# EugenHotaj/zig_gpt2

Measured on AMD Instinct MI355X. Metric: tokens/sec GPT-2-124M greedy 1024-ctx, higher is better.
Workload: dtype bf16 weights, f32 activations/accumulate; 1 GPU; GPT-2 124M greedy decode, 1 prompt(s)/GPU x 1 GPU(s), 1-token prompts, 1024 decode steps per prompt (reference generate loop, src/main.zig:322-342); vocab=50257, context=1024, n_layer=12, n_heads=12, n_embed=768, prompts_per_gpu=1, global_prompts=1, kv_cache=f32, hip_graph=True, l2_prefetcher=on, parallelism=replicated weights, prompts sharded x1, RCCL broadcast at start-up only

## Files before the change

### zig_gpt2_amd/csrc/api_gpt.hip

```cpp
#include <stdio.h>
#include <stdlib.h>
#include <string.h>

#include <string>
#include <thread>
#include <vector>

#include "zg_runtime.h"

using namespace zg;

struct zg_layer {
    void *c_attn_w, *c_proj_w, *c_fc_w, *mlp_proj_w;
    bf16_t *c_attn_p, *c_proj_p, *c_fc_p, *mlp_proj_p;
    float *c_attn_c2, *c_attn_c3, *c_fc_c2, *c_fc_c3;
    float *ln_1_g, *ln_1_b, *c_attn_b, *c_proj_b, *ln_2_g, *ln_2_b, *c_fc_b, *mlp_proj_b;
    void *k_cache, *v_cache;
};

struct zg_gpt {
    zg_gpt_config cfg;
    size_t batch;
    unsigned flags;
    int wt;
    int kv_mode;
    size_t wbytes;
    char* arena;
    size_t arena_bytes, weight_region_bytes, state_bytes;
    size_t kv_region_bytes;
    void *wte, *wpe;
    float *ln_f_g, *ln_f_b;
    float *lm_c2, *lm_c3;
    std::vector<zg_layer> layers;
    StepCtrl* ctrl;
    float *x, *q, *h4, *part, *logits, *part_val;
    int *part_idx, *prompt, *prompt_len, *forced, *cur_token, *out_tokens;
    float* sk_ws;
    int* sk_cnt;
    int sk_tiles;
    float *pf_x, *pf_qkv, *pf_ws;
    size_t pf_ws_floats;
    unsigned* sk_flags;
    unsigned sk_epoch;
    bool sk_used;
    bf16_t *pf_a, *pf_h;
    bf16_t *xp, *hp, *ap;
    int* attn_cnt;
    unsigned* epoch;
    unsigned spin_limit;
    unsigned* fault;
    unsigned long long *sk_tag, *part_tag;
    size_t sk_tag_bytes, part_tag_bytes;
    size_t epochs_since_clear;
    bool tags_on;
    float* xst;
    bool st_on;
    bool pl_on;
    int max_splits, lm_grid;
    StepCtrl* h_ctrl;
    int* h_ints;
    std::vector<hipGraphExec_t> graphs;
    std::vector<hipGraphExec_t> graphs_k;
    std::vector<hipGraphExec_t> graphs_s, graphs_ks;
    int* sampled;
    float* samp_ws;
    SampleParams* samp;
    SampleParams* h_samp;
    bool gen_sampled;
    size_t graph_steps;
    hipStream_t graph_stream;
    size_t steps_enqueued;
    bool ln_folded;
    PfCtl* pf_ctl;
    PfJob* pf_jobs;
    int pf_njobs;
    bool pf_on;
    bool pf_ran;
    bool pf_stalled;
    int pf_strikes;
    int pf_sit_out;
    hipStream_t pf_stream;
    hipEvent_t pf_ev_main, pf_ev_side;
    hipStream_t stream;
    zg_gpt* parent;
    int n_children;
    char* wbase;
    size_t gen_pos, gen_n, gen_min_prompt, gen_since_sync;
    bool gen_open;
};

static inline hipStream_t gs(const zg_gpt* g) { return g->stream ? g->stream : ctx().stream; }
static inline zg_gpt* root(zg_gpt* g) { return g->parent ? g->parent : g; }

namespace {

struct Carver {
    size_t off = 0;
    size_t take(size_t bytes) {
        off = (off + 255) & ~(size_t)255;
        const size_t o = off;
        off += bytes;
        return o;
    }
};

void carve(zg_gpt* g, char* wbase, char* sbase) {
    const zg_gpt_config& c = g->cfg;
    const size_t E = c.n_embed, V = c.vocab_size, C = c.context_size, L = c.n_layer, B = g->batch;
    const size_t wb = g->wbytes, kvb = g->kv_mode == 1 ? 2 : g->kv_mode == 2 ? 3 : 4;
    Carver cv;
    char* base = wbase;
    auto P = [&](size_t bytes) -> char* {
        const size_t o = cv.take(bytes);
        return base ? base + o : nullptr;
    };
    g->wte = P(V * E * wb);
    g->wpe = P(C * E * wb);
    g->ln_f_g = (float*)P(E * 4);
    g->ln_f_b = (float*)P(E * 4);
    g->lm_c2 = (float*)P(V * 4);
    g->lm_c3 = (float*)P(V * 4);
    g->layers.resize(L);
    for (size_t l = 0; l < L; ++l) {
        zg_layer& y = g->layers[l];
        y.c_attn_w = P(3 * E * E * wb);
        y.c_proj_w = P(E * E * wb);
        y.c_fc_w = P(4 * E * E * wb);
        y.mlp_proj_w = P(4 * E * E * wb);
        y.ln_1_g = (float*)P(E * 4);
        y.ln_1_b = (float*)P(E * 4);
        y.c_attn_b = (float*)P(3 * E * 4);
        y.c_proj_b = (float*)P(E * 4);
        y.ln_2_g = (float*)P(E * 4);
        y.ln_2_b = (float*)P(E * 4);
        y.c_fc_b = (float*)P(4 * E * 4);
        y.mlp_proj_b = (float*)P(E * 4);
        y.c_attn_c2 = (float*)P(3 * E * 4);
        y.c_attn_c3 = (float*)P(3 * E * 4);
        y.c_fc_c2 = (float*)P(4 * E * 4);
        y.c_fc_c3 = (float*)P(4 * E * 4);
        y.c_attn_p = y.c_proj_p = y.c_fc_p = y.mlp_proj_p = nullptr;
        if (g->wt == WT_F32 && !(g->flags & ZG_GPT_NO_PREFILL)) {
            y.c_attn_p = (bf16_t*)P(3 * E * E * kSplit * 2);
            y.c_proj_p = (bf16_t*)P(E * E * kSplit * 2);
            y.c_fc_p = (bf16_t*)P(4 * E * E * kSplit * 2);
            y.mlp_proj_p = (bf16_t*)P(4 * E * E * kSplit * 2);
        }
    }
    g->weight_region_bytes = (cv.off + 255) & ~(size_t)255;
    cv = Carver{};
    base = sbase;
    for (size_t l = 0; l < L; ++l) {
        g->layers[l].k_cache = P(B * C * E * kvb);
        g->layers[l].v_cache = P(B * C * E * kvb);
    }
    g->ctrl = (StepCtrl*)P(sizeof(StepCtrl));
    g->kv_region_bytes = L ? (size_t)(reinterpret_cast<char*>(g->ctrl) - reinterpret_cast<char*>(g->layers[0].k_cache)) : 0;
    g->x = (float*)P(B * E * 4);
    g->q = (float*)P(B * E * 4);
    g->h4 = (float*)P(B * 4 * E * 4);
    g->part = (float*)P(B * c.n_heads * g->max_splits * kPartStride * 4);
    g->logits = (float*)P(B * V * 4);
    g->part_val = (float*)P(B * 4096 * 4);
    g->part_idx = (int*)P(B * 4096 * 4);
    g->prompt = (int*)P(B * C * 4);
    g->prompt_len = (int*)P(B * 4);
    g->forced = (int*)P(B * 4);
    g->cur_token = (int*)P(B * 4);
    g->out_tokens = (int*)P(B * C * 4);
    g->sampled = (int*)P(B * 4);
    g->samp = (SampleParams*)P(sizeof(SampleParams));
    g->samp_ws = (float*)P(sample_workspace_floats((int)B) * 4);
    g->xp = (bf16_t*)P(E * 48);
    g->hp = (bf16_t*)P(4 * E * 48);
    g->ap = (bf16_t*)P(E * 48);
    g->attn_cnt = (int*)P(8 * c.n_heads * 4);
    g->epoch = (unsigned*)P(256);
    g->xst = (float*)P(((E + 15) / 16) * 8 * 2 * 4);
    g->sk_tag_bytes = ((E + 15) / 16) * 4 * 128 * 8;
    g->part_tag_bytes = 8 * c.n_heads * g->max_splits * kPartStride * 8;
    g->sk_tag = (unsigned long long*)P(g->sk_tag_bytes);
    g->part_tag = (unsigned long long*)P(g->part_tag_bytes);
    g->sk_tiles = (int)((E + 15) / 16);
    g->sk_ws = (float*)P((size_t)g->sk_tiles * 4 * 128 * 4);
    g->sk_cnt = (int*)P((size_t)g->sk_tiles * 4 * 4);
    g->pf_njobs = (int)(2 + 5 * L);
    g->pf_ctl = (PfCtl*)P(sizeof(PfCtl));
    g->pf_jobs = (PfJob*)P((size_t)g->pf_njobs * sizeof(PfJob));
    g->pf_x = g->pf_qkv = g->pf_ws = nullptr;
    g->sk_flags = nullptr;
    g->sk_epoch = 0;
    g->sk_used = false;
    g->pf_a = g->pf_h = nullptr;
    g->pf_ws_floats = 0;
    if (!(g->flags & ZG_GPT_NO_PREFILL)) {
        g->pf_x = (float*)P(B * C * E * 4);
        g->pf_qkv = (float*)P(B * C * 3 * E * 4);
        g->pf_a = (bf16_t*)P(B * C * kSplit * E * 2);
        g->pf_h = (bf16_t*)P(B * C * kSplit * 4 * E * 2);
        g->pf_ws_floats = g->wt == WT_BF16 ? (size_t)(16u << 20) : std::max((size_t)(16u << 20), 3 * B * C * 4 * E);
        g->pf_ws = (float*)P(g->pf_ws_floats * 4);
        g->sk_flags = (unsigned*)P(2048);
    }
    g->state_bytes = (cv.off + 255) & ~(size_t)255;
}

int bucket_t_hi(const zg_gpt* g, size_t seq_len) {
    const size_t hi = ((seq_len + 63) / 64) * 64;
    return (int)(hi < g->cfg.context_size ? hi : g->cfg.context_size);
}

GemvArgs base_gemv(const zg_gpt* g, const void* W, const float* bias, size_t N, size_t K, int t_hi) {
    GemvArgs a{};
    a.t_hi = t_hi;
    a.dbg = ctx().dbg;
    a.zero = ctx().d_zero;
    a.W = W;
    a.bias = bias;
    a.N = (int)N;
    a.K = (int)K;
    a.M = (int)g->batch;
    a.eps = 1e-5f;
    a.ctrl = g->ctrl;
    a.n_heads = (int)g->cfg.n_heads;
    a.head_dim = 64;
    a.max_splits = g->max_splits;
    a.ctx = (int)g->cfg.context_size;
    a.kv_mode = g->kv_mode;
    a.kv_lo = g->batch * g->cfg.context_size * g->cfg.n_embed * 2;
    a.sk_ws = g->sk_ws;
    a.sk_cnt = g->sk_cnt;
    a.sk_tiles = g->sk_tiles;
    a.progress = g->pf_on ? &g->pf_ctl->progress : nullptr;
    return a;
}

EmbedArgs embed_args(const zg_gpt* g, int finish_only) {
    EmbedArgs e{};
    e.ctrl = g->ctrl;
    e.wte = g->wte;
    e.wpe = g->wpe;
    e.weight_type = g->wt;
    e.n_embed = (int)g->cfg.n_embed;
    e.batch = (int)g->batch;
    e.vocab = (int)g->cfg.vocab_size;
    e.prompt = g->prompt;
    e.prompt_stride = (int)g->cfg.context_size;
    e.prompt_len = g->prompt_len;
    e.forced = g->forced;
    e.cur_token = g->cur_token;
    e.out_tokens = g->out_tokens;
    e.out_stride = (int)g->cfg.context_size;
    e.part_val = g->part_val;
    e.part_idx = g->part_idx;
    e.part_stride = g->lm_grid;
    e.n_partials = g->lm_grid;
    e.x = g->x;
    e.pl_out = g->pl_on ? g->xp : nullptr;
    e.pl_g = g->layers[0].ln_1_g;
    e.epoch = (g->pl_on && g->tags_on && finish_only != 1 && finish_only != 2) ? g->epoch : nullptr;
    e.st_out = g->st_on ? g->xst : nullptr;
    e.finish_only = finish_only;
    e.progress = g->pf_on ? &g->pf_ctl->progress : nullptr;
    e.sampled = g->sampled;
    return e;
}

int emit_gemv(const zg_gpt* g, const GemvArgs& a, int grid, hipStream_t s, std::vector<PfJob>* rec, unsigned cls) {
    if (!rec) return launch_gemv(a, g->wt, grid, s);
    PfJob j{};
    j.cls = cls;
    const int rows = gemv_rows_per_wg(a, g->wt);
    if (rows > 0) {
        j.kind = PF_WEIGHTS;
        j.base = reinterpret_cast<const char*>(a.W);
        j.total_bytes = (size_t)a.N * a.K * g->wbytes;
        j.wg_bytes = (unsigned)((size_t)rows * a.K * g->wbytes);
        j.n_wg = (unsigned)grid;
        j.touch_bytes = j.wg_bytes;
        if (a.M == 1) {
            const bool lnk = a.prologue == PRO_LAYERNORM && a.ln_c2 != nullptr;
            const float* v[3] = {lnk ? a.ln_g : nullptr, lnk ? a.ln_c2 : a.bias, lnk ? a.ln_c3 : nullptr};
            const size_t n[3] = {(size_t)a.K * 4, (size_t)a.N * 4, (size_t)a.N * 4};
            for (int i = 0; i < 3; ++i) {
                j.aux[i] = reinterpret_cast<const char*>(v[i]);
                j.aux_bytes[i] = v[i] ? (unsigned)n[i] : 0u;
            }
        }
        const size_t cap = (size_t)16 << 20;
        if (j.total_bytes > cap) j.touch_bytes = (unsigned)(((size_t)j.wg_bytes * cap / j.total_bytes + 127) & ~(size_t)127);
    }
    rec->push_back(j);
    return ZG_OK;
}

int enqueue_lm_head(zg_gpt* g, hipStream_t s, std::vector<PfJob>* rec = nullptr) {
    const size_t E = g->cfg.n_embed, V = g->cfg.vocab_size;
    GemvArgs a = base_gemv(g, g->wte, nullptr, V, E, 0);
    a.prologue = PRO_LAYERNORM;
    a.x = g->x;
    a.x_stride = (int)E;
    a.ln_g = g->ln_f_g;
    a.ln_b = g->ln_f_b;
    a.ln_c2 = g->lm_c2;
    a.ln_c3 = g->lm_c3;
    a.epilogue = EPI_ARGMAX;
    a.logits = g->logits;
    a.logits_stride = (int)V;
    a.part_val = g->part_val;
    a.part_idx = g->part_idx;
    const int grid = gemv_plan(a, g->wt);
    ZG_REQUIRE(grid == g->lm_grid, ZG_ERR_ARG, "lm_head grid changed");
    return emit_gemv(g, a, grid, s, rec, 6);
}

struct StepProf {
    std::vector<hipEvent_t> ev;
    std::vector<int> cls;
    size_t n = 0;
};
inline int prof_mark(StepProf* p, int cls, hipStream_t s) {
    if (!p) return ZG_OK;
    if (p->n == p->ev.size()) {
        hipEvent_t e;
        ZG_HIP(hipEventCreate(&e));
        p->ev.push_back(e);
        p->cls.push_back(cls);
    }
    p->cls[p->n] = cls;
    ZG_HIP(hipEventRecord(p->ev[p->n++], s));
    return ZG_OK;
}

int ensure_ln_folded(zg_gpt* g, hipStream_t s) {
    zg_gpt* r = root(g);
    if (r->ln_folded) return ZG_OK;
    const int E = (int)g->cfg.n_embed;
    for (const zg_layer& y : g->layers) {
        ZG_TRY(launch_ln_fold(y.c_attn_w, g->wt, y.ln_1_g, y.ln_1_b, y.c_attn_b, 3 * E, E, y.c_attn_c2, y.c_attn_c3, s));
        ZG_TRY(launch_ln_fold(y.c_fc_w, g->wt, y.ln_2_g, y.ln_2_b, y.c_fc_b, 4 * E, E, y.c_fc_c2, y.c_fc_c3, s));
    }
    ZG_TRY(launch_ln_fold(g->wte, g->wt, g->ln_f_g, g->ln_f_b, nullptr, (int)g->cfg.vocab_size, E, g->lm_c2, g->lm_c3, s));
    if (r->n_children > 0 || g->parent) ZG_HIP(hipStreamSynchronize(s));
    r->ln_folded = true;
    return ZG_OK;
}

int env_int(const char* name, int dflt);

int enqueue_step(zg_gpt* g, bool with_logits, int t_hi, hipStream_t s, StepProf* prof = nullptr, int only = -1, size_t only_layer = 0,
                 std::vector<PfJob>* rec = nullptr, int salt = -1, bool with_sampler = false) {
    const size_t E = g->cfg.n_embed;
    auto launch_id = [&](size_t l, int k) { return (unsigned)(salt >= 0 ? 1 + (2 * salt + k) % 254 : 2 * (int)l + 1 + k); };
    ZG_TRY(prof_mark(prof, -1, s));
    if (rec) rec->push_back(PfJob{});
    else if (only < 0 || only == 0) {
        EmbedArgs e = embed_args(g, only == 0 ? 3 : 0);
        ZG_TRY(launch_embed_step(e, s));
    }
    ZG_TRY(prof_mark(prof, 0, s));
    for (size_t l = (only < 0 ? 0 : only_layer); l < (only < 0 ? g->cfg.n_layer : only_layer + 1); ++l) {
        const zg_layer& y = g->layers[l];
        if (only < 0 || only == 1) {
            GemvArgs a = base_gemv(g, y.c_attn_w, y.c_attn_b, 3 * E, E, t_hi);
            a.prologue = PRO_LAYERNORM;
            a.x = g->x;
            a.x_stride = (int)E;
            a.ln_g = y.ln_1_g;
            a.ln_b = y.ln_1_b;
            a.ln_c2 = y.c_attn_c2;
            a.ln_c3 = y.c_attn_c3;
            a.epilogue = EPI_QKV;
            a.pl_in = g->pl_on ? g->xp : nullptr;
            a.st_in = g->st_on ? g->xst : nullptr;
            a.q = g->q;
            a.k_cache = y.k_cache;
            a.v_cache = y.v_cache;
            const int grid = gemv_plan(a, g->wt);
            ZG_TRY(emit_gemv(g, a, grid, s, rec, 1));
            ZG_TRY(prof_mark(prof, 1, s));
        }
        if (only < 0 || only == 2) {
            AttnArgs a{};
            a.q = g->q;
            a.k = y.k_cache;
            a.v = y.v_cache;
            a.stride_b = (long)(g->cfg.context_size * E);
            a.stride_h = (long)(g->cfg.context_size * 64);
            a.stride_t = 64;
            a.kv_mode = g->kv_mode;
            a.kv_lo = g->batch * g->cfg.context_size * E * 2;
            a.n_heads = (int)g->cfg.n_heads;
            a.head_dim = 64;
            a.batch = (int)g->batch;
            a.ctrl = g->ctrl;
            a.t_hi = t_hi;
            a.max_splits = g->max_splits;
            a.part = g->part;
            a.progress = g->pf_on ? &g->pf_ctl->progress : nullptr;
            if (g->pl_on) {
                a.pl_out = g->ap;
                a.merge_cnt = g->attn_cnt;
                if (g->tags_on && 2 * l + 2 <= 255) {
                    a.epoch = g->epoch;
                    a.launch_id = launch_id(l, 0);
                    a.part_tag = g->part_tag;
                    a.fault = g->fault;
                    a.spin_limit = g->spin_limit;
                }
            }
            if (rec) {
                PfJob j{};
                j.kind = PF_KV;
                j.cls = 2;
                j.base = reinterpret_cast<const char*>(y.k_cache);
                j.base2 = reinterpret_cast<const char*>(y.v_cache);
                j.n_heads = (unsigned)g->cfg.n_heads;
                j.ctx = (unsigned)g->cfg.context_size;
                j.batch = (unsigned)g->batch;
                j.row_bytes = g->kv_mode ? 128u : 256u;
                rec->push_back(j);
            } else
                ZG_TRY(launch_attn_decode(a, s));
            ZG_TRY(prof_mark(prof, 2, s));
        }
        if (only < 0 || only == 3) {
            GemvArgs a = base_gemv(g, y.c_proj_w, y.c_proj_b, E, E, t_hi);
            a.prologue = PRO_ATTN_MERGE;
            a.part = g->part;
            a.epilogue = EPI_RESIDUAL;
            a.y = g->x;
            a.y_stride = (int)E;
            a.resid = g->x;
            a.resid_stride = (int)E;
            if (g->pl_on) {
                a.prologue = PRO_NONE;
                a.pl_in = g->ap;
                a.pl_out = g->xp;
                a.pl_g = y.ln_2_g;
                a.st_out = g->st_on ? g->xst : nullptr;
            }
            const int grid = gemv_plan(a, g->wt);
            ZG_TRY(emit_gemv(g, a, grid, s, rec, 3));
            ZG_TRY(prof_mark(prof, 3, s));
        }
        if (only < 0 || only == 4) {
            GemvArgs a = base_gemv(g, y.c_fc_w, y.c_fc_b, 4 * E, E, t_hi);
            a.prologue = PRO_LAYERNORM;
            a.x = g->x;
            a.x_stride = (int)E;
            a.ln_g = y.ln_2_g;
            a.ln_b = y.ln_2_b;
            a.ln_c2 = y.c_fc_c2;
            a.ln_c3 = y.c_fc_c3;
            a.epilogue = EPI_GELU;
            a.y = g->h4;
            a.y_stride = (int)(4 * E);
            if (g->pl_on) {
                a.st_in = g->st_on ? g->xst : nullptr;
                a.pl_in = g->xp;
                a.pl_out = g->hp;
                a.y = nullptr;
            }
            const int grid = gemv_plan(a, g->wt);
            ZG_TRY(emit_gemv(g, a, grid, s, rec, 4));
            ZG_TRY(prof_mark(prof, 4, s));
        }
        if (only < 0 || only == 5) {
            GemvArgs a = base_gemv(g, y.mlp_proj_w, y.mlp_proj_b, E, 4 * E, t_hi);
            a.prologue = PRO_NONE;
            a.x = g->h4;
            a.x_stride = (int)(4 * E);
            a.epilogue = EPI_RESIDUAL;
            a.y = g->x;
            a.y_stride = (int)E;
            a.resid = g->x;
            a.resid_stride = (int)E;
            if (g->pl_on) {
                if (g->tags_on && 2 * l + 2 <= 255) {
                    a.epoch = g->epoch;
                    a.launch_id = launch_id(l, 1);
                    a.sk_tag = g->sk_tag;
                    a.fault = g->fault;
                    a.spin_limit = g->spin_limit;
                }
                a.pl_in = g->hp;
                if (l + 1 < g->cfg.n_layer) {
                    a.pl_out = g->xp;
                    a.pl_g = g->layers[l + 1].ln_1_g;
                    a.st_out = g->st_on ? g->xst : nullptr;
                }
            }
            const int grid = gemv_plan(a, g->wt);
            ZG_TRY(emit_gemv(g, a, grid, s, rec, 5));
            ZG_TRY(prof_mark(prof, 5, s));
        }
    }
    if (with_logits && (only < 0 || only == 6)) {
        ZG_TRY(enqueue_lm_head(g, s, rec));
        ZG_TRY(prof_mark(prof, 6, s));
    }
    if (with_sampler && with_logits && only < 0 && !rec)
        ZG_TRY(launch_sample_step(g->logits, (int)g->batch, (int)g->cfg.vocab_size, g->samp, g->ctrl, g->part_val, g->lm_grid, g->lm_grid, g->samp_ws,
                                  g->sampled, s));
    return ZG_OK;
}

int enqueue_prefill(zg_gpt* g, size_t P, bool last_block_full, hipStream_t s) {
    const bool f32w = g->wt == WT_F32;
    const int np = f32w ? kWeightPlanes : (g->flags & ZG_GPT_PREFILL_2PLANE) ? 2 : kSplit;
    const size_t E = g->cfg.n_embed, L = g->cfg.n_layer, H = g->cfg.n_heads, C = g->cfg.context_size;
    const int B = (int)g->batch, M = (int)(g->batch * P), iE = (int)E;
    ZG_TRY(launch_embed_prefill(g->prompt, (int)C, B, (int)P, g->wte, g->wpe, g->wt, iE, g->pf_x, s));
    ZG_TRY(launch_ln_split(g->pf_x, M, iE, g->layers[0].ln_1_g, g->layers[0].ln_1_b, 1e-5f, g->pf_a, s));
    for (size_t l = 0; l < L; ++l) {
        const zg_layer& y = g->layers[l];
        PrefillQkv qa{(int)P, iE, (int)H, (int)C, g->kv_mode, y.k_cache, y.v_cache, g->batch * C * E * 2};
        if (!f32w && g->sk_flags != nullptr) {
            qa.sk_ws = g->pf_ws;
            qa.sk_ws_bytes = g->pf_ws_floats * 4;
            qa.sk_flags = g->sk_flags;
            qa.sk_flags_words = 512;
            qa.sk_epoch = ++g->sk_epoch;
            g->sk_used = true;
        }
        ZG_TRY(launch_prefill_gemm(g->pf_a, f32w ? y.c_attn_p : (const bf16_t*)y.c_attn_w, y.c_attn_b, g->pf_qkv, M, 3 * iE, iE, 3 * iE, PF_QKV,
                                   g->pf_ws, g->pf_ws_floats, nullptr, s, &qa, np));
        if (l + 1 == L && !last_block_full) break;
        ZG_TRY(launch_attn_prefill(g->pf_qkv, g->pf_a, B, (int)P, iE, (int)H, g->pf_ws, g->pf_ws_floats, g->kv_mode == 0 ? (const float*)y.k_cache : nullptr,
                                       g->kv_mode == 0 ? (const float*)y.v_cache : nullptr, (int)C, s));
        const PrefillLn ln2{y.ln_2_g, y.ln_2_b, 1e-5f, g->pf_a};
        ZG_TRY(launch_prefill_gemm(g->pf_a, f32w ? y.c_proj_p : (const bf16_t*)y.c_proj_w, y.c_proj_b, g->pf_x, M, iE, iE, iE, PF_RESID, g->pf_ws,
                                   g->pf_ws_floats, &ln2, s, nullptr, np));
        ZG_TRY(launch_prefill_gemm(g->pf_a, f32w ? y.c_fc_p : (const bf16_t*)y.c_fc_w, y.c_fc_b, g->pf_h, M, 4 * iE, iE, 0, PF_GELU_SPLIT, g->pf_ws,
                                   g->pf_ws_floats, nullptr, s, nullptr, np));
        const bool more = l + 1 < L;
        const PrefillLn ln1{more ? g->layers[l + 1].ln_1_g : nullptr, more ? g->layers[l + 1].ln_1_b : nullptr, 1e-5f, g->pf_a};
        ZG_TRY(launch_prefill_gemm(g->pf_h, f32w ? y.mlp_proj_p : (const bf16_t*)y.mlp_proj_w, y.mlp_proj_b, g->pf_x, M, iE, 4 * iE, iE, PF_RESID, g->pf_ws,
                                   g->pf_ws_floats, more ? &ln1 : nullptr, s, nullptr, np));
    }
    return ZG_OK;
}

int check_fault(zg_gpt* g) {
    unsigned sk = 0, tag = 0;
    if (g->sk_used) {
        g->sk_used = false;
        ZG_TRY(gemm_s4_fault(&sk));
    }
    if (g->tags_on) {
        volatile unsigned* f = g->fault;
        tag = *f;
        if (tag) *f = 0;
    }
    if (sk) {
        set_error("a half-tile hand-over of the whole-prompt c_attn GEMM timed out%s: results discarded", tag ? " (and a tagged hand-over of the decode step)" : "");
        return ZG_ERR_HIP;
    }
    if (tag) {
        set_error("a tagged hand-over of the decode step timed out (a workgroup waited %u polls for its writers): results discarded", g->spin_limit);
        return ZG_ERR_HIP;
    }
    return ZG_OK;
}

int note_steps(zg_gpt* g, size_t n, hipStream_t s) {
    if (!g->tags_on) return ZG_OK;
    g->epochs_since_clear += n;
    if (g->epochs_since_clear < ((size_t)1 << 23)) return ZG_OK;
    g->epochs_since_clear = n;
    ZG_HIP(hipMemsetAsync(g->sk_tag, 0, g->sk_tag_bytes, s));
    ZG_HIP(hipMemsetAsync(g->part_tag, 0, g->part_tag_bytes, s));
    return ZG_OK;
}

int env_int(const char* name, int dflt) {
    const char* e = getenv(name);
    return e ? atoi(e) : dflt;
}

int setup_prefetcher(zg_gpt* g) {
    g->pf_on = g->pf_ran = g->pf_stalled = false;
    g->pf_strikes = g->pf_sit_out = 0;
    g->pf_stream = nullptr;
    g->pf_ev_main = g->pf_ev_side = nullptr;
    const bool small = g->stream == nullptr && g->batch == 1 && 4 * g->cfg.n_embed * g->cfg.n_embed * g->wbytes <= ((size_t)6 << 20);
    const int want = env_int("ZGPT2_PREFETCH", small ? 1 : 0);
    if ((g->flags & ZG_GPT_NO_PREFETCH) || !want || gs(g) == nullptr) return ZG_OK;
    if (g->pf_njobs > 255) return ZG_OK;
    std::vector<PfJob> jobs;
    ZG_TRY(enqueue_step(g, true, (int)g->cfg.context_size, nullptr, nullptr, -1, 0, &jobs));
    ZG_REQUIRE((int)jobs.size() == g->pf_njobs, ZG_ERR_ARG, "prefetcher: %zu launches per step", jobs.size());
    ZG_HIP(hipMemcpy(g->pf_jobs, jobs.data(), jobs.size() * sizeof(PfJob), hipMemcpyHostToDevice));
    int least = 0, greatest = 0;
    ZG_HIP(hipDeviceGetStreamPriorityRange(&least, &greatest));
    ZG_HIP(hipStreamCreateWithPriority(&g->pf_stream, hipStreamNonBlocking, least));
    ZG_HIP(hipEventCreateWithFlags(&g->pf_ev_main, hipEventDisableTiming));
    ZG_HIP(hipEventCreateWithFlags(&g->pf_ev_side, hipEventDisableTiming));
    g->pf_on = true;
    return ZG_OK;
}

void drop_prefetcher(zg_gpt* g) {
    if (g->pf_stream) {
        (void)hipStreamSynchronize(g->pf_stream);
        (void)hipStreamDestroy(g->pf_stream);
    }
    if (g->pf_ev_main) (void)hipEventDestroy(g->pf_ev_main);
    if (g->pf_ev_side) (void)hipEventDestroy(g->pf_ev_side);
    g->pf_stream = nullptr;
    g->pf_ev_main = g->pf_ev_side = nullptr;
    g->pf_on = false;
}

int pf_start(zg_gpt* g, size_t last_T, hipStream_t s) {
    if (!g->pf_on || s == nullptr) return ZG_OK;
    if (g->pf_ran) {
        ZG_HIP(hipStreamSynchronize(g->pf_stream));
        unsigned why[8];
        ZG_HIP(hipMemcpy(why, g->pf_ctl->exit_reason, sizeof(why), hipMemcpyDeviceToHost));
        bool idle_exit = false;
        for (unsigned w : why) idle_exit |= w == 2u;
        g->pf_ran = false;
        if (idle_exit) {
            g->pf_stalled = true;
            ++g->pf_strikes;
            g->pf_sit_out = 8;
        }
    }
    if (g->pf_stalled) {
        if (g->pf_strikes >= 3 || g->pf_sit_out-- > 0) return ZG_OK;
        g->pf_stalled = false;
    }
    ZG_HIP(hipMemsetAsync(g->pf_ctl, 0, sizeof(PfCtl), g->pf_stream));
    ZG_HIP(hipEventRecord(g->pf_ev_side, g->pf_stream));
    ZG_HIP(hipStreamWaitEvent(s, g->pf_ev_side, 0));
    ZG_HIP(hipEventRecord(g->pf_ev_main, s));
    ZG_HIP(hipStreamWaitEvent(g->pf_stream, g->pf_ev_main, 0));
    PfArgs a{};
    a.ctl = g->pf_ctl;
    a.jobs = g->pf_jobs;
    a.njobs = g->pf_njobs;
    a.lead = 2;
    a.nsub = 12;
    a.max_T = (int)last_T;
    a.idle_limit = (unsigned)env_int("ZGPT2_PF_IDLE", 100000);
    a.sleep = 1;
    a.cls_mask = 0x3e;
    a.line_shift = 7;
    a.cap_bytes = 0;
    g->pf_ran = true;
    return launch_prefetcher(a, g->pf_stream);
}

int pf_stop(zg_gpt* g, hipStream_t s) {
    if (!g->pf_on || s == nullptr) return ZG_OK;
    ZG_HIP(hipMemsetD32Async(reinterpret_cast<hipDeviceptr_t>(&g->pf_ctl->progress), (int)PF_STOP, 1, s));
    return ZG_OK;
}

size_t prefill_min() { return 4; }

void drop_graphs(zg_gpt* g) {
    for (auto* v : {&g->graphs, &g->graphs_k, &g->graphs_s, &g->graphs_ks})
        for (auto& e : *v)
            if (e) {
                (void)hipGraphExecDestroy(e);
                e = nullptr;
            }
}

int capture_steps(zg_gpt* g, hipGraphExec_t* out, bool with_logits, int t_hi, size_t n_steps, hipStream_t cs, bool with_sampler = false) {
    hipGraph_t graph = nullptr;
    ZG_HIP(hipStreamBeginCapture(cs, hipStreamCaptureModeThreadLocal));
    int st = ZG_OK;
    for (size_t i = 0; i < n_steps && st == ZG_OK; ++i) st = enqueue_step(g, with_logits, t_hi, cs, nullptr, -1, 0, nullptr, -1, with_sampler);
    hipError_t e = hipStreamEndCapture(cs, &graph);
    if (st != ZG_OK) {
        if (graph) (void)hipGraphDestroy(graph);
        return st;
    }
    ZG_HIP(e);
    ZG_HIP(hipGraphInstantiate(out, graph, nullptr, nullptr, 0));
    ZG_HIP(hipGraphDestroy(graph));
    return ZG_OK;
}

int capture_bucket(zg_gpt* g, size_t idx, hipStream_t s) {
    const size_t seq_len = (idx / 2 + 1) * 64;
    const bool with_logits = idx & 1;
    if (g->graphs.size() <= idx) g->graphs.resize(idx + 1, nullptr);
    if (g->graphs[idx]) return ZG_OK;
    const int t_hi = bucket_t_hi(g, seq_len);
    return capture_steps(g, &g->graphs[idx], with_logits, t_hi, 1, s);
}

int capture_multi(zg_gpt* g, size_t b, hipStream_t s) {
    if (g->graphs_k.size() <= b) g->graphs_k.resize(b + 1, nullptr);
    if (g->graphs_k[b]) return ZG_OK;
    const int t_hi = bucket_t_hi(g, (b + 1) * 64);
    return capture_steps(g, &g->graphs_k[b], true, t_hi, g->graph_steps, s);
}

int capture_sampled(zg_gpt* g, size_t b, bool multi, hipStream_t s) {
    auto& v = multi ? g->graphs_ks : g->graphs_s;
    if (v.size() <= b) v.resize(b + 1, nullptr);
    if (v[b]) return ZG_OK;
    return capture_steps(g, &v[b], true, bucket_t_hi(g, (b + 1) * 64), multi ? g->graph_steps : 1, s, true);
}

int capture_all(zg_gpt* g, hipStream_t s) {
    if ((g->flags & ZG_GPT_NO_GRAPH) || s == nullptr) return ZG_OK;
    if (g->graph_stream != s) {
        drop_graphs(g);
        g->graph_stream = s;
    }
    const size_t n = ((g->cfg.context_size + 63) / 64) * 2;
    for (size_t idx = 0; idx < n; ++idx) ZG_TRY(capture_bucket(g, idx, s));
    if (g->graph_steps > 1)
        for (size_t b = 0; b < n / 2; ++b) ZG_TRY(capture_multi(g, b, s));
    if (g->flags & ZG_GPT_SAMPLED_GENERATE)
        for (size_t b = 0; b < n / 2; ++b) {
            ZG_TRY(capture_sampled(g, b, false, s));
            if (g->graph_steps > 1) ZG_TRY(capture_sampled(g, b, true, s));
        }
    return ZG_OK;
}

int run_step(zg_gpt* g, bool with_logits, size_t seq_len, hipStream_t s, bool with_sampler = false) {
    ZG_TRY(ensure_ln_folded(g, s));
    const int t_hi = bucket_t_hi(g, seq_len);
    with_sampler = with_sampler && with_logits;
    if ((g->flags & ZG_GPT_NO_GRAPH) || s == nullptr) return enqueue_step(g, with_logits, t_hi, s, nullptr, -1, 0, nullptr, -1, with_sampler);
    if (g->graph_stream != s) ZG_TRY(capture_all(g, s));
    if (with_sampler) {
        const size_t b = (seq_len + 63) / 64 - 1;
        ZG_TRY(capture_sampled(g, b, false, s));
        ZG_HIP(hipGraphLaunch(g->graphs_s[b], s));
        return ZG_OK;
    }
    const size_t idx = ((seq_len + 63) / 64 - 1) * 2 + (with_logits ? 1 : 0);
    ZG_TRY(capture_bucket(g, idx, s));
    ZG_HIP(hipGraphLaunch(g->graphs[idx], s));
    return ZG_OK;
}

int upload_f32(const float* src, size_t n, void* dst, bool as_bf16, hipStream_t s) {
    Ctx& c = ctx();
    const float* dsrc = src;
    if (!is_device_ptr(src)) {
        if (!as_bf16) {
            ZG_HIP(hipMemcpyAsync(dst, src, n * 4, hipMemcpyHostToDevice, s));
            ZG_HIP(hipStreamSynchronize(s));
            return ZG_OK;
        }
        const size_t cap = c.stage_cap / 4;
        ZG_REQUIRE(cap > 0, ZG_ERR_STAGING, "no staging arena");
        for (size_t o = 0; o < n; o += cap) {
            const size_t m = (n - o < cap) ? (n - o) : cap;
            ZG_HIP(hipMemcpyAsync(c.stage, src + o, m * 4, hipMemcpyHostToDevice, s));
            ZG_TRY(launch_f32_to_bf16(reinterpret_cast<const float*>(c.stage), reinterpret_cast<bf16_t*>(dst) + o, m, s));
            ZG_HIP(hipStreamSynchronize(s));
        }
        return ZG_OK;
    }
    if (as_bf16) ZG_TRY(launch_f32_to_bf16(dsrc, reinterpret_cast<bf16_t*>(dst), n, s));
    else ZG_HIP(hipMemcpyAsync(dst, dsrc, n * 4, hipMemcpyDeviceToDevice, s));
    ZG_HIP(hipStreamSynchronize(s));
    return ZG_OK;
}

}

extern "C" {

int zg_gpt_create(zg_gpt** out, const zg_gpt_config* config, size_t batch, unsigned flags) {
    return zg_gpt_create_ex(out, config, batch, flags, nullptr);
}

int zg_gpt_create_ex(zg_gpt** out, const zg_gpt_config* config, size_t batch, unsigned flags, const zg_gpt_options* opt) {
    ZG_TRY(require_init());
    ZG_REQUIRE(out && config, ZG_ERR_ARG, "zg_gpt_create: null argument");
    const zg_gpt_config& c = *config;
    zg_gpt* parent = opt ? opt->share_weights_with : nullptr;
    if (parent) {
        ZG_REQUIRE(parent->parent == nullptr, ZG_ERR_ARG, "zg_gpt_create_ex: share_weights_with must own its weights");
        ZG_REQUIRE(memcmp(&parent->cfg, config, sizeof(zg_gpt_config)) == 0, ZG_ERR_SHAPE, "zg_gpt_create_ex: a handle shares weights with one of the same config only");
        const unsigned same = ZG_GPT_WEIGHTS_F32 | ZG_GPT_NO_PREFILL;
        ZG_REQUIRE((parent->flags & same) == (flags & same), ZG_ERR_ARG, "zg_gpt_create_ex: weight type / prefill flags differ from the weight owner's");
    }
    ZG_REQUIRE(c.n_heads > 0 && c.n_embed % c.n_heads == 0 && c.n_embed / c.n_heads == 64, ZG_ERR_UNSUPPORTED,
               "head_dim %zu != 64 (GPT-2 family only)", c.n_heads ? c.n_embed / c.n_heads : (size_t)0);
    ZG_REQUIRE(c.n_embed % 8 == 0 && c.n_embed * 4 <= 8192, ZG_ERR_UNSUPPORTED, "n_embed %zu unsupported", c.n_embed);
    ZG_REQUIRE(batch >= 1 && batch <= 8, ZG_ERR_UNSUPPORTED, "batch %zu outside 1..8", batch);
    ZG_REQUIRE(c.vocab_size > 0 && c.context_size > 0 && c.n_layer > 0, ZG_ERR_ARG, "empty config");
    ZG_REQUIRE(!(flags & ZG_GPT_KV_F16) || !(flags & ZG_GPT_KV_B24), ZG_ERR_ARG, "ZG_GPT_KV_F16 and ZG_GPT_KV_B24 exclude each other");
    zg_gpt* g = new zg_gpt();
    g->cfg = c;
    g->batch = batch;
    g->flags = flags;
    g->wt = (flags & ZG_GPT_WEIGHTS_F32) ? WT_F32 : WT_BF16;
    g->wbytes = g->wt == WT_BF16 ? 2 : 4;
    g->kv_mode = (flags & ZG_GPT_KV_F16) ? 1 : (flags & ZG_GPT_KV_B24) ? 2 : 0;
    g->max_splits = (int)((c.context_size + kAttnChunk - 1) / kAttnChunk);
    g->graph_stream = nullptr;
    g->stream = nullptr;
    g->parent = parent;
    g->n_children = 0;
    g->gen_open = false;
    g->pf_stream = nullptr;
    g->pf_ev_main = g->pf_ev_side = nullptr;
    carve(g, nullptr, nullptr);
    g->arena_bytes = (parent ? 0 : g->weight_region_bytes) + g->state_bytes;
    hipError_t e = hipMalloc(reinterpret_cast<void**>(&g->arena), g->arena_bytes);
    if (e != hipSuccess) {
        delete g;
        return hip_fail(e, "hipMalloc(model arena)", __FILE__, __LINE__);
    }
    g->wbase = parent ? parent->wbase : g->arena;
    char* const sbase = parent ? g->arena : g->arena + g->weight_region_bytes;
    carve(g, g->wbase, sbase);
    (void)hipMemset(sbase, 0, g->state_bytes);
    if (opt && opt->own_stream) {
        int least = 0, greatest = 0;
        (void)hipDeviceGetStreamPriorityRange(&least, &greatest);
        const int pr = opt->stream_priority > 0 ? greatest : opt->stream_priority < 0 ? least : 0;
        e = hipStreamCreateWithPriority(&g->stream, hipStreamNonBlocking, pr);
        if (e != hipSuccess) {
            (void)hipFree(g->arena);
            delete g;
            return hip_fail(e, "hipStreamCreateWithPriority(handle stream)", __FILE__, __LINE__);
        }
    }
    {
        GemvArgs a = base_gemv(g, g->wte, nullptr, c.vocab_size, c.n_embed, 0);
        a.prologue = PRO_LAYERNORM;
        a.epilogue = EPI_ARGMAX;
        g->lm_grid = gemv_plan(a, g->wt);
    }
    {
        GemvArgs a = base_gemv(g, g->layers[0].mlp_proj_w, nullptr, c.n_embed, 4 * c.n_embed, 0);
        if (!gemv_supported(a, g->wt)) {
            if (g->stream) (void)hipStreamDestroy(g->stream);
            (void)hipFree(g->arena);
            delete g;
            set_error("batch %zu with n_embed %zu: %zu input rows of 4*n_embed floats do not fit the LDS (use a smaller batch)",
                      batch, c.n_embed, batch);
            return ZG_ERR_UNSUPPORTED;
        }
    }
    g->pl_on = false;
    if (g->wt == WT_BF16 && batch >= 2 && !(decode_paths_off() & 1)) {
        const zg_layer& y = g->layers[0];
        GemvArgs a1 = base_gemv(g, y.c_attn_w, y.c_attn_b, 3 * c.n_embed, c.n_embed, 0);
        a1.prologue = PRO_LAYERNORM;
        a1.ln_c2 = y.c_attn_c2;
        a1.ln_c3 = y.c_attn_c3;
        a1.epilogue = EPI_QKV;
        GemvArgs a4 = base_gemv(g, y.c_fc_w, y.c_fc_b, 4 * c.n_embed, c.n_embed, 0);
        a4.prologue = PRO_LAYERNORM;
        a4.ln_c2 = y.c_fc_c2;
        a4.ln_c3 = y.c_fc_c3;
        a4.epilogue = EPI_GELU;
        GemvArgs a5 = base_gemv(g, y.mlp_proj_w, y.mlp_proj_b, c.n_embed, 4 * c.n_embed, 0);
        a5.prologue = PRO_NONE;
        a5.epilogue = EPI_RESIDUAL;
        GemvArgs a3 = base_gemv(g, y.c_proj_w, y.c_proj_b, c.n_embed, c.n_embed, 0);
        a3.prologue = PRO_NONE;
        a3.epilogue = EPI_RESIDUAL;
        g->pl_on = c.n_embed % 32 == 0 && gemv_planes_ok(a1, g->wt) && gemv_planes_ok(a3, g->wt) && gemv_planes_ok(a4, g->wt) &&
                   gemv_planes_ok(a5, g->wt);
    }
    g->tags_on = g->pl_on && !(decode_paths_off() & 4);
    g->spin_limit = (unsigned)env_int("ZGPT2_TAG_SPIN_LIMIT", 1 << 20);
    g->st_on = false;
    if (g->pl_on && !(decode_paths_off() & 8) && c.n_embed % 16 == 0 && c.n_embed / 16 <= 128) {
        const zg_layer& y = g->layers[0];
        GemvArgs a1 = base_gemv(g, y.c_attn_w, y.c_attn_b, 3 * c.n_embed, c.n_embed, 0);
        a1.prologue = PRO_LAYERNORM;
        a1.x_stride = (int)c.n_embed;
        a1.ln_c2 = y.c_attn_c2;
        a1.ln_c3 = y.c_attn_c3;
        a1.epilogue = EPI_QKV;
        GemvArgs a4 = a1;
        a4.N = (int)(4 * c.n_embed);
        a4.epilogue = EPI_GELU;
        GemvArgs a3 = base_gemv(g, y.c_proj_w, y.c_proj_b, c.n_embed, c.n_embed, 0);
        a3.prologue = PRO_NONE;
        a3.epilogue = EPI_RESIDUAL;
        a3.resid_stride = (int)c.n_embed;
        GemvArgs a5 = base_gemv(g, y.mlp_proj_w, y.mlp_proj_b, c.n_embed, 4 * c.n_embed, 0);
        a5.prologue = PRO_NONE;
        a5.epilogue = EPI_RESIDUAL;
        a5.resid_stride = (int)c.n_embed;
        g->st_on = gemv_pl4_ok(a1, g->wt) && gemv_pl4_ok(a3, g->wt) && gemv_pl4_ok(a4, g->wt) && gemv_pl4_ok(a5, g->wt);
    }
    if (g->lm_grid > 4096) {
        if (g->stream) (void)hipStreamDestroy(g->stream);
        (void)hipFree(g->arena);
        delete g;
        set_error("lm_head grid %d exceeds the argmax partial buffer", g->lm_grid);
        return ZG_ERR_UNSUPPORTED;
    }
    g->h_ctrl = nullptr;
    g->h_ints = nullptr;
    hipError_t he = hipHostMalloc(reinterpret_cast<void**>(&g->h_ctrl), sizeof(StepCtrl) + 512, hipHostMallocDefault);
    if (he == hipSuccess)
        he = hipHostMalloc(reinterpret_cast<void**>(&g->h_ints), (batch * c.context_size + batch) * sizeof(int), hipHostMallocDefault);
    if (he != hipSuccess) {
        if (g->h_ctrl) (void)hipHostFree(g->h_ctrl);
        if (g->stream) (void)hipStreamDestroy(g->stream);
        (void)hipFree(g->arena);
        delete g;
        return hip_fail(he, "hipHostMalloc(control mirrors)", __FILE__, __LINE__);
    }
    static_assert(sizeof(StepCtrl) + sizeof(SampleParams) <= 256, "the fault word sits 256 bytes behind the control mirror");
    g->h_samp = reinterpret_cast<SampleParams*>(reinterpret_cast<char*>(g->h_ctrl) + 128);
    g->gen_sampled = false;
    g->fault = reinterpret_cast<unsigned*>(reinterpret_cast<char*>(g->h_ctrl) + 256);
    *g->fault = 0;
    g->steps_enqueued = 0;
    g->epochs_since_clear = 0;
    g->ln_folded = false;
    {
        const int k = env_int("ZGPT2_GRAPH_STEPS", 8);
        g->graph_steps = (k == 2 || k == 4 || k == 8 || k == 16 || k == 32 || k == 64) ? (size_t)k : 1;
    }
    {
        int st = setup_prefetcher(g);
        if (st == ZG_OK) st = capture_all(g, gs(g));
        if (st != ZG_OK) {
            drop_prefetcher(g);
            drop_graphs(g);
            (void)hipHostFree(g->h_ctrl);
            (void)hipHostFree(g->h_ints);
            if (g->stream) (void)hipStreamDestroy(g->stream);
            (void)hipFree(g->arena);
            delete g;
            return st;
        }
    }
    if (parent) ++parent->n_children;
    *out = g;
    return ZG_OK;
}

int zg_gpt_destroy(zg_gpt* g) {
    if (!g) return ZG_OK;
    ZG_REQUIRE(g->n_children == 0, ZG_ERR_ARG, "zg_gpt_destroy: %d handle(s) still borrow this one's weights (destroy them first)", g->n_children);
    (void)hipStreamSynchronize(gs(g));
    drop_prefetcher(g);
    drop_graphs(g);
    if (g->stream) (void)hipStreamDestroy(g->stream);
    if (g->parent) --g->parent->n_children;
    (void)hipFree(g->arena);
    (void)hipHostFree(g->h_ctrl);
    (void)hipHostFree(g->h_ints);
    delete g;
    return ZG_OK;
}

int zg_gpt_stream(zg_gpt* g, void** hip_stream_out) {
    ZG_TRY(require_init());
    ZG_REQUIRE(g && hip_stream_out, ZG_ERR_ARG, "zg_gpt_stream: null argument");
    *hip_stream_out = gs(g);
    return ZG_OK;
}

int zg_gpt_load_block_tensor(zg_gpt* g, size_t layer, int slot, const float* src, size_t len) {
    ZG_TRY(require_init());
    ZG_REQUIRE(g && src && layer < g->cfg.n_layer, ZG_ERR_ARG, "load_block_tensor: bad argument");
    ZG_REQUIRE(g->parent == nullptr, ZG_ERR_ARG, "load_block_tensor: this handle borrows its weights (load them into their owner)");
    const size_t E = g->cfg.n_embed;
    zg_layer& y = g->layers[layer];
    void* dst = nullptr;
    size_t n = 0;
    bool mat = false;
    switch (slot) {
        case ZG_LN_1_G: dst = y.ln_1_g; n = E; break;
        case ZG_LN_1_B: dst = y.ln_1_b; n = E; break;
        case ZG_C_ATTN_W: dst = y.c_attn_w; n = 3 * E * E; mat = true; break;
        case ZG_C_ATTN_B: dst = y.c_attn_b; n = 3 * E; break;
        case ZG_C_PROJ_W: dst = y.c_proj_w; n = E * E; mat = true; break;
        case ZG_C_PROJ_B: dst = y.c_proj_b; n = E; break;
        case ZG_LN_2_G: dst = y.ln_2_g; n = E; break;
        case ZG_LN_2_B: dst = y.ln_2_b; n = E; break;
        case ZG_C_FC_W: dst = y.c_fc_w; n = 4 * E * E; mat = true; break;
        case ZG_C_FC_B: dst = y.c_fc_b; n = 4 * E; break;
        case ZG_MLP_PROJ_W: dst = y.mlp_proj_w; n = 4 * E * E; mat = true; break;
        case ZG_MLP_PROJ_B: dst = y.mlp_proj_b; n = E; break;
        default: ZG_REQUIRE(false, ZG_ERR_ARG, "unknown block slot %d", slot);
    }
    ZG_REQUIRE(len == n, ZG_ERR_SHAPE, "block slot %d expects %zu elements, got %zu", slot, n, len);
    g->ln_folded = false;
    ZG_TRY(upload_f32(src, n, dst, mat && g->wt == WT_BF16, gs(g)));
    if (mat && g->wt == WT_F32 && y.c_attn_p) {
        bf16_t* pl = slot == ZG_C_ATTN_W ? y.c_attn_p : slot == ZG_C_PROJ_W ? y.c_proj_p : slot == ZG_C_FC_W ? y.c_fc_p : y.mlp_proj_p;
        ZG_REQUIRE(n <= (size_t)2147483647 / 3, ZG_ERR_SHAPE, "weight matrix of %zu elements", n);
        ZG_TRY(launch_split3(reinterpret_cast<const float*>(dst), 1, (int)n, pl, gs(g)));
        ZG_HIP(hipStreamSynchronize(gs(g)));
    }
    return ZG_OK;
}

int zg_gpt_load_tensor(zg_gpt* g, int slot, const float* src, size_t len) {
    ZG_TRY(require_init());
    ZG_REQUIRE(g && src, ZG_ERR_ARG, "load_tensor: bad argument");
    ZG_REQUIRE(g->parent == nullptr, ZG_ERR_ARG, "load_tensor: this handle borrows its weights (load them into their owner)");
    const size_t E = g->cfg.n_embed;
    void* dst = nullptr;
    size_t n = 0;
    bool mat = false;
    switch (slot) {
        case ZG_WTE: dst = g->wte; n = g->cfg.vocab_size * E; mat = true; break;
        case ZG_WPE: dst = g->wpe; n = g->cfg.context_size * E; mat = true; break;
        case ZG_LN_F_G: dst = g->ln_f_g; n = E; break;
        case ZG_LN_F_B: dst = g->ln_f_b; n = E; break;
        default: ZG_REQUIRE(false, ZG_ERR_ARG, "unknown slot %d", slot);
    }
    ZG_REQUIRE(len == n, ZG_ERR_SHAPE, "slot %d expects %zu elements, got %zu", slot, n, len);
    g->ln_folded = false;
    return upload_f32(src, n, dst, mat && g->wt == WT_BF16, gs(g));
}

int zg_gpt_weight_arena(zg_gpt* g, void** device_ptr, size_t* bytes) {
    ZG_REQUIRE(g && device_ptr && bytes, ZG_ERR_ARG, "weight_arena: null argument");
    if (!root(g)->ln_folded) {
// ... 337 lines not shown
        std::vector<std::thread> th;
        std::vector<int> res(begun, ZG_OK);
        std::vector<std::string> errs(begun);
        const int dev = ctx().device;
        for (size_t i = 0; i < begun; ++i)
            th.emplace_back([&, i]() {
                int r = hipSetDevice(dev) == hipSuccess ? ZG_OK : ZG_ERR_HIP;
                for (bool more = true; more && r == ZG_OK;) r = gen_pump(handles[i], &more);
                res[i] = r;
                if (r != ZG_OK) errs[i] = zg_last_error();
            });
        for (auto& t : th) t.join();
        for (size_t i = 0; i < begun && rs == ZG_OK; ++i)
            if (res[i] != ZG_OK) {
                rs = res[i];
                snprintf(msg, sizeof msg, "%s", errs[i].c_str());
            }
    } else {
        bool any = rs == ZG_OK;
        while (any && rs == ZG_OK) {
            any = false;
            for (size_t i = 0; i < begun && rs == ZG_OK; ++i) {
                bool more = false;
                if (handles[i]->gen_pos < handles[i]->gen_n) rs = gen_pump(handles[i], &more);
                any |= more;
            }
        }
        if (rs != ZG_OK) snprintf(msg, sizeof msg, "%s", zg_last_error());
    }
    int first_err = rs;
    for (size_t i = 0; i < begun; ++i) {
        const int e = gen_end(handles[i], rs);
        if (first_err == ZG_OK && e != ZG_OK) {
            first_err = e;
            snprintf(msg, sizeof msg, "%s", zg_last_error());
        }
    }
    if (first_err != ZG_OK) set_error("%s", msg);
    return first_err;
}

int zg_gpt_generate_fetch_many(zg_gpt* const* handles, size_t n_handles, size_t n_steps, size_t* out_tokens, size_t out_len) {
    ZG_TRY(require_init());
    ZG_REQUIRE(handles && n_handles >= 1 && out_tokens, ZG_ERR_ARG, "generate_fetch_many: null argument");
    size_t rows = 0;
    for (size_t i = 0; i < n_handles; ++i) {
        ZG_REQUIRE(handles[i] != nullptr, ZG_ERR_ARG, "generate_fetch_many: handle %zu is null", i);
        rows += handles[i]->batch;
    }
    ZG_REQUIRE(out_len >= rows * n_steps, ZG_ERR_SHAPE, "generate_fetch_many: out_tokens too short");
    size_t row = 0;
    int first_err = ZG_OK;
    char msg[512];
    for (size_t i = 0; i < n_handles; ++i) {
        const int e = zg_gpt_generate_fetch(handles[i], n_steps, out_tokens + row * n_steps, handles[i]->batch * n_steps);
        if (first_err == ZG_OK && e != ZG_OK) {
            first_err = e;
            snprintf(msg, sizeof msg, "%s", zg_last_error());
        }
        row += handles[i]->batch;
    }
    if (first_err != ZG_OK) set_error("%s", msg);
    return first_err;
}

int zg_gpt_generate_fetch(zg_gpt* g, size_t n_steps, size_t* out_tokens, size_t out_len) {
    ZG_TRY(require_init());
    ZG_REQUIRE(g && out_tokens, ZG_ERR_ARG, "generate_fetch: null argument");
    const size_t C = g->cfg.context_size, B = g->batch;
    ZG_REQUIRE(n_steps <= C && out_len >= B * n_steps, ZG_ERR_SHAPE, "generate_fetch: out_tokens too short");
    hipStream_t s = gs(g);
    ZG_HIP(hipMemcpyAsync(g->h_ints, g->out_tokens, B * C * sizeof(int), hipMemcpyDeviceToHost, s));
    ZG_HIP(hipStreamSynchronize(s));
    ZG_TRY(check_fault(g));
    for (size_t b = 0; b < B; ++b)
        for (size_t i = 0; i < n_steps; ++i) out_tokens[b * n_steps + i] = (size_t)g->h_ints[b * C + i];
    return ZG_OK;
}

int zg_gpt_generate_greedy(zg_gpt* g, const size_t* prompts, size_t prompt_stride, const size_t* prompt_lens,
                           size_t n_steps, size_t* out_tokens, size_t out_len) {
    ZG_REQUIRE(g && out_tokens && out_len >= g->batch * n_steps, ZG_ERR_SHAPE, "generate: out_tokens too short");
    ZG_TRY(zg_gpt_generate_enqueue(g, prompts, prompt_stride, prompt_lens, n_steps));
    return zg_gpt_generate_fetch(g, n_steps, out_tokens, out_len);
}

int zg_gpt_profile_step(zg_gpt* g, size_t seq_len, int iters, float* us_out, size_t n_out) {
    ZG_TRY(require_init());
    ZG_REQUIRE(g && us_out && n_out >= 8 && iters > 0, ZG_ERR_ARG, "profile_step: bad argument");
    ZG_REQUIRE(seq_len >= 1 && seq_len + (size_t)iters - 1 <= g->cfg.context_size, ZG_ERR_SHAPE,
               "profile_step: positions %zu..%zu outside the context", seq_len, seq_len + iters - 1);
    hipStream_t s = gs(g);
    ZG_HIP(hipStreamSynchronize(s));
    ZG_TRY(ensure_ln_folded(g, s));
    ZG_TRY(note_steps(g, (size_t)iters, s));
    for (size_t b = 0; b < g->batch; ++b) g->h_ints[b] = (int)(b % g->cfg.vocab_size);
    g->h_ctrl->step = (int)seq_len - 1;
    g->h_ctrl->seq_len = (int)seq_len;
    g->h_ctrl->mode = 1;
    g->h_ctrl->n_partials = g->lm_grid;
    ZG_HIP(hipMemcpyAsync(g->forced, g->h_ints, g->batch * sizeof(int), hipMemcpyHostToDevice, s));
    ZG_HIP(hipMemcpyAsync(g->ctrl, g->h_ctrl, sizeof(StepCtrl), hipMemcpyHostToDevice, s));
    static StepProf prof;
    double acc[8] = {0, 0, 0, 0, 0, 0, 0, 0};
    prof.n = 0;
    double null_us = 0.0;
    for (int it = 0; it < iters; ++it) {
        ZG_TRY(enqueue_step(g, true, bucket_t_hi(g, seq_len + it), s, &prof));
        ZG_TRY(launch_copy_f32(g->q, g->q + 4, 1, s));
        ZG_TRY(prof_mark(&prof, 8, s));
    }
    ZG_HIP(hipStreamSynchronize(s));
    for (size_t i = 1; i < prof.n; ++i) {
        if (prof.cls[i] < 0) continue;
        float ms = 0.0f;
        ZG_HIP(hipEventElapsedTime(&ms, prof.ev[i - 1], prof.ev[i]));
        if (prof.cls[i] == 8) {
            null_us += ms * 1000.0;
            continue;
        }
        acc[prof.cls[i]] += ms * 1000.0;
        acc[7] += ms * 1000.0;
    }
    for (int i = 0; i < 8; ++i) us_out[i] = (float)(acc[i] / iters);
    if (n_out >= 9) us_out[8] = (float)(null_us / iters);
    return check_fault(g);
}

int zg_gpt_time_kernel(zg_gpt* g, int which_and_options, int iters, float* avg_us, size_t* algorithmic_bytes) {
    ZG_TRY(require_init());
    const int which = which_and_options & 0xff;
    const bool cycle = (which_and_options & ZG_TIME_WALK_LAYERS) != 0;
    const size_t t_opt = (size_t)((unsigned)which_and_options >> 16);
    ZG_REQUIRE(g && avg_us && iters > 0 && which_and_options >= 0 && which <= 6, ZG_ERR_ARG, "time_kernel: bad argument (ZG_TIME_AT takes t < 32768)");
    hipStream_t s = gs(g);
    ZG_REQUIRE(s != nullptr, ZG_ERR_UNSUPPORTED, "time_kernel needs a capturable stream");
    const size_t E = g->cfg.n_embed, wb = g->wbytes;
    const size_t bytes_tab[7] = {0, 3 * E * E * wb, 0, E * E * wb, 4 * E * E * wb, 4 * E * E * wb, g->cfg.vocab_size * E * wb};
    size_t T = g->cfg.context_size / 2 > 0 ? g->cfg.context_size / 2 : 1;
    if (t_opt >= 1 && t_opt <= g->cfg.context_size) T = t_opt;
    ZG_HIP(hipStreamSynchronize(s));
    ZG_TRY(ensure_ln_folded(g, s));
    ZG_TRY(note_steps(g, (size_t)iters + 8, s));
    g->h_ctrl->step = (int)T - 1;
    g->h_ctrl->seq_len = (int)T;
    g->h_ctrl->mode = 1;
    g->h_ctrl->n_partials = g->lm_grid;
    ZG_HIP(hipMemcpyAsync(g->ctrl, g->h_ctrl, sizeof(StepCtrl), hipMemcpyHostToDevice, s));
    const int chain = 64;
    hipGraph_t graph = nullptr;
    hipGraphExec_t exec = nullptr;
    ZG_HIP(hipStreamBeginCapture(s, hipStreamCaptureModeThreadLocal));
    int st = ZG_OK;
    if (g->tags_on && which != 0) st = launch_epoch_bump(g->epoch, s);
    for (int i = 0; i < chain && st == ZG_OK; ++i)
        st = enqueue_step(g, true, bucket_t_hi(g, T), s, nullptr, which, cycle ? (size_t)i % g->cfg.n_layer : 0, nullptr, i);
    hipError_t ce = hipStreamEndCapture(s, &graph);
    if (st != ZG_OK) return st;
    ZG_HIP(ce);
    ZG_HIP(hipGraphInstantiate(&exec, graph, nullptr, nullptr, 0));
    hipEvent_t e0, e1;
    ZG_HIP(hipEventCreate(&e0));
    ZG_HIP(hipEventCreate(&e1));
    ZG_HIP(hipGraphLaunch(exec, s));
    ZG_HIP(hipStreamSynchronize(s));
    const int reps = (iters + chain - 1) / chain;
    ZG_HIP(hipEventRecord(e0, s));
    for (int r = 0; r < reps; ++r) ZG_HIP(hipGraphLaunch(exec, s));
    ZG_HIP(hipEventRecord(e1, s));
    ZG_HIP(hipEventSynchronize(e1));
    float ms = 0.0f;
    ZG_HIP(hipEventElapsedTime(&ms, e0, e1));
    (void)hipEventDestroy(e0);
    (void)hipEventDestroy(e1);
    (void)hipGraphExecDestroy(exec);
    (void)hipGraphDestroy(graph);
    *avg_us = ms * 1000.0f / (float)(reps * chain);
    if (algorithmic_bytes) *algorithmic_bytes = bytes_tab[which];
    return check_fault(g);
}

int zg_debug_prefetch_stats(zg_gpt* g, unsigned* out, size_t n_out) {
    ZG_TRY(require_init());
    ZG_REQUIRE(g && out && n_out >= 25, ZG_ERR_ARG, "prefetch_stats: need 25 words");
    memset(out, 0, n_out * sizeof(unsigned));
    out[0] = g->pf_on ? (g->pf_stalled ? 2u : 1u) : 0u;
    if (!g->pf_on) return ZG_OK;
    ZG_HIP(hipStreamSynchronize(gs(g)));
    ZG_HIP(hipStreamSynchronize(g->pf_stream));
    PfCtl h;
    ZG_HIP(hipMemcpy(&h, g->pf_ctl, sizeof(PfCtl), hipMemcpyDeviceToHost));
    for (int x = 0; x < 8; ++x) {
        out[1 + x] = h.ticket[x];
        out[9 + x] = h.exit_reason[x];
        out[17 + x] = h.jobs_done[x];
    }
    for (size_t i = 0; i < 256 && 25 + i < n_out; ++i) out[25 + i] = h.xcd_log[i];
    return ZG_OK;
}

#ifdef ZG_STAMPS
int zg_debug_stamps_begin(void) {
    ZG_TRY(require_init());
    Ctx& c = ctx();
    const size_t bytes = (16 + 10 * 4096) * sizeof(unsigned long long);
    if (!c.dbg) ZG_HIP(hipMalloc(reinterpret_cast<void**>(&c.dbg), bytes));
    ZG_HIP(hipMemset(c.dbg, 0, bytes));
    return ZG_OK;
}
int zg_debug_stamps_read(unsigned long long* out, size_t n_words) {
    ZG_TRY(require_init());
    ZG_HIP(hipDeviceSynchronize());
    ZG_HIP(hipMemcpy(out, ctx().dbg, n_words * sizeof(unsigned long long), hipMemcpyDeviceToHost));
    return ZG_OK;
}
#endif

}
```

### zig_gpt2_amd/csrc/attn.hip

```cpp
#include <stdlib.h>

#include "zg_kernels.h"
#include "zg_runtime.h"

namespace zg {

namespace {

constexpr float kNegBig = -1e30f;

template <typename KV>
__device__ __forceinline__ f32x4 load_kv4(const KV* p);
template <>
__device__ __forceinline__ f32x4 load_kv4<float>(const float* p) {
    return *reinterpret_cast<const f32x4*>(p);
}
template <>
__device__ __forceinline__ f32x4 load_kv4<_Float16>(const _Float16* p) {
    typedef __attribute__((ext_vector_type(4))) _Float16 h4;
    const h4 v = *reinterpret_cast<const h4*>(p);
    f32x4 r;
    r.x = (float)v.x; r.y = (float)v.y; r.z = (float)v.z; r.w = (float)v.w;
    return r;
}

__device__ __forceinline__ float row16_reduce_scatter(float (&s)[16], int lr) {
    float a8[8];
    {
        const bool hi = lr & 8;
#pragma unroll
        for (int j = 0; j < 8; ++j) {
            const float keep = hi ? s[j + 8] : s[j];
            const float send = hi ? s[j] : s[j + 8];
            a8[j] = keep + dpp_row_ror<8>(send);
        }
    }
    float a4[4];
    {
        const bool hi = lr & 4;
#pragma unroll
        for (int j = 0; j < 4; ++j) {
            const float keep = hi ? a8[j + 4] : a8[j];
            const float send = hi ? a8[j] : a8[j + 4];
            const float from_lo = dpp_row_ror<4>(send);
            const float from_hi = dpp_row_ror<12>(send);
            a4[j] = keep + (hi ? from_lo : from_hi);
        }
    }
    float a2[2];
    {
        const bool hi = lr & 2;
#pragma unroll
        for (int j = 0; j < 2; ++j) {
            const float keep = hi ? a4[j + 2] : a4[j];
            const float send = hi ? a4[j] : a4[j + 2];
            const float from_lo = dpp_row_ror<2>(send);
            const float from_hi = dpp_row_ror<14>(send);
            a2[j] = keep + (hi ? from_lo : from_hi);
        }
    }
    {
        const bool hi = lr & 1;
        const float keep = hi ? a2[1] : a2[0];
        const float send = hi ? a2[0] : a2[1];
        const float from_lo = dpp_row_ror<1>(send);
        const float from_hi = dpp_row_ror<15>(send);
        return keep + (hi ? from_lo : from_hi);
    }
}

__device__ __forceinline__ void publish_partial(const AttnArgs& a, int n_heads, int nsplit, int b, int h, int split, int lane, float o,
                                                float M, float l, unsigned tag) {
    float* part = a.part + (((size_t)b * n_heads + h) * a.max_splits + split) * kPartStride;
    if (a.pl_out == nullptr) {
        part[lane] = o;
        if (lane == 0) {
            part[64] = M;
            part[65] = l;
        }
        return;
    }
    float r = o, lsum = l;
    if (nsplit > 1 && a.part_tag) {
        typedef unsigned long long u64;
        auto pack = [&](float v) { return ((u64)tag << 32) | (u64)__float_as_uint(v); };
        u64* pt0 = a.part_tag + ((size_t)b * n_heads + h) * a.max_splits * kPartStride;
        const int last = nsplit - 1;
        if (split != last) {
            u64* pt = pt0 + split * kPartStride;
            __hip_atomic_store(pt + lane, pack(o), __ATOMIC_RELAXED, __HIP_MEMORY_SCOPE_AGENT);
            if (lane == 0) {
                __hip_atomic_store(pt + 64, pack(M), __ATOMIC_RELAXED, __HIP_MEMORY_SCOPE_AGENT);
                __hip_atomic_store(pt + 65, pack(l), __ATOMIC_RELAXED, __HIP_MEMORY_SCOPE_AGENT);
            }
            return;
        }
        float mx = M;
        r = 0.0f;
        lsum = 0.0f;
        constexpr int MAXS = 4;
        if (nsplit <= MAXS) {
            u64 vo[MAXS - 1], vm[MAXS - 1], vl[MAXS - 1];
            for (int spins = 0;; ++spins) {
                bool ok = true;
#pragma unroll
                for (int s = 0; s < MAXS - 1; ++s) {
                    const u64* ps = pt0 + min(s, last - 1) * kPartStride;
                    vo[s] = __hip_atomic_load(ps + lane, __ATOMIC_RELAXED, __HIP_MEMORY_SCOPE_AGENT);
                    vm[s] = __hip_atomic_load(ps + 64, __ATOMIC_RELAXED, __HIP_MEMORY_SCOPE_AGENT);
                    vl[s] = __hip_atomic_load(ps + 65, __ATOMIC_RELAXED, __HIP_MEMORY_SCOPE_AGENT);
                    ok = ok && (unsigned)(vo[s] >> 32) == tag && (unsigned)(vm[s] >> 32) == tag && (unsigned)(vl[s] >> 32) == tag;
                }
                if (__builtin_amdgcn_ballot_w64(!ok) == 0) break;
                if ((unsigned)spins >= a.spin_limit) {
                    if (lane == 0 && a.fault) __hip_atomic_store(a.fault, 1u, __ATOMIC_RELAXED, __HIP_MEMORY_SCOPE_AGENT);
                    break;
                }
                __builtin_amdgcn_s_sleep(1);
            }
            float ms[MAXS], ls[MAXS], os[MAXS];
#pragma unroll
            for (int s = 0; s < MAXS; ++s) {
                const bool polled = s < last && s < MAXS - 1;
                ms[s] = polled ? __uint_as_float((unsigned)vm[s < MAXS - 1 ? s : 0]) : s == last ? M : -1e30f;
                ls[s] = polled ? __uint_as_float((unsigned)vl[s < MAXS - 1 ? s : 0]) : l;
                os[s] = polled ? __uint_as_float((unsigned)vo[s < MAXS - 1 ? s : 0]) : o;
            }
            mx = fmaxf(fmaxf(ms[0], ms[1]), fmaxf(ms[2], ms[3]));
#pragma unroll
            for (int s = 0; s < MAXS; ++s) {
                const float w = __expf(ms[s] - mx);
                lsum = fmaf(w, ls[s], lsum);
                r = fmaf(w, os[s], r);
            }
        } else {
            float mrun = -1e30f;
            for (int s = 0; s <= last; ++s) {
                float m_s = M, o_s = o, l_s = l;
                if (s < last) {
                    const u64* ps = pt0 + s * kPartStride;
                    u64 vo, vm, vl;
                    for (int spins = 0;; ++spins) {
                        vo = __hip_atomic_load(ps + lane, __ATOMIC_RELAXED, __HIP_MEMORY_SCOPE_AGENT);
                        vm = __hip_atomic_load(ps + 64, __ATOMIC_RELAXED, __HIP_MEMORY_SCOPE_AGENT);
                        vl = __hip_atomic_load(ps + 65, __ATOMIC_RELAXED, __HIP_MEMORY_SCOPE_AGENT);
                        const bool ok = (unsigned)(vo >> 32) == tag && (unsigned)(vm >> 32) == tag && (unsigned)(vl >> 32) == tag;
                        if (__builtin_amdgcn_ballot_w64(!ok) == 0) break;
                        if ((unsigned)spins >= a.spin_limit) {
                            if (lane == 0 && a.fault) __hip_atomic_store(a.fault, 1u, __ATOMIC_RELAXED, __HIP_MEMORY_SCOPE_AGENT);
                            break;
                        }
                        __builtin_amdgcn_s_sleep(1);
                    }
                    m_s = __uint_as_float((unsigned)vm);
                    o_s = __uint_as_float((unsigned)vo);
                    l_s = __uint_as_float((unsigned)vl);
                }
                const float mnew = fmaxf(mrun, m_s);
                const float w0 = __expf(mrun - mnew), w1 = __expf(m_s - mnew);
                r = fmaf(w1, o_s, r * w0);
                lsum = fmaf(w1, l_s, lsum * w0);
                mrun = mnew;
            }
        }
    } else if (nsplit > 1) {
        typedef __attribute__((address_space(1))) unsigned gu32;
        gu32* gp = (gu32*)part;
        __hip_atomic_store(gp + lane, __float_as_uint(o), __ATOMIC_RELAXED, __HIP_MEMORY_SCOPE_AGENT);
        if (lane == 0) {
            __hip_atomic_store(gp + 64, __float_as_uint(M), __ATOMIC_RELAXED, __HIP_MEMORY_SCOPE_AGENT);
            __hip_atomic_store(gp + 65, __float_as_uint(l), __ATOMIC_RELAXED, __HIP_MEMORY_SCOPE_AGENT);
        }
        asm volatile("s_waitcnt vmcnt(0)" ::: "memory");
        int* cnt = a.merge_cnt + b * n_heads + h;
        int ticket = 0;
        if (lane == 0) ticket = __hip_atomic_fetch_add(cnt, 1, __ATOMIC_RELAXED, __HIP_MEMORY_SCOPE_AGENT);
        ticket = __builtin_amdgcn_readfirstlane(ticket);
        if (ticket != nsplit - 1) return;
        if (lane == 0) __hip_atomic_store(cnt, 0, __ATOMIC_RELAXED, __HIP_MEMORY_SCOPE_AGENT);
        const gu32* p0 = (const gu32*)(a.part + ((size_t)b * n_heads + h) * a.max_splits * kPartStride);
        constexpr int MAXS = 4;
        if (nsplit <= MAXS) {
            float ms[MAXS], ls[MAXS], os[MAXS];
#pragma unroll
            for (int s = 0; s < MAXS; ++s) {
                const gu32* ps = p0 + min(s, nsplit - 1) * kPartStride;
                ms[s] = __uint_as_float(__hip_atomic_load(ps + 64, __ATOMIC_RELAXED, __HIP_MEMORY_SCOPE_AGENT));
                ls[s] = __uint_as_float(__hip_atomic_load(ps + 65, __ATOMIC_RELAXED, __HIP_MEMORY_SCOPE_AGENT));
                os[s] = __uint_as_float(__hip_atomic_load(ps + lane, __ATOMIC_RELAXED, __HIP_MEMORY_SCOPE_AGENT));
            }
#pragma unroll
            for (int s = 0; s < MAXS; ++s)
                if (s >= nsplit) ms[s] = -1e30f;
            const float mx = fmaxf(fmaxf(ms[0], ms[1]), fmaxf(ms[2], ms[3]));
            r = 0.0f;
            lsum = 0.0f;
#pragma unroll
            for (int s = 0; s < MAXS; ++s) {
                const float w = __expf(ms[s] - mx);
                lsum = fmaf(w, ls[s], lsum);
                r = fmaf(w, os[s], r);
            }
        } else {
            float mx = -1e30f;
            for (int s = 0; s < nsplit; ++s)
                mx = fmaxf(mx, __uint_as_float(__hip_atomic_load(p0 + s * kPartStride + 64, __ATOMIC_RELAXED, __HIP_MEMORY_SCOPE_AGENT)));
            r = 0.0f;
            lsum = 0.0f;
            for (int s = 0; s < nsplit; ++s) {
                const gu32* ps = p0 + s * kPartStride;
                const float w = __expf(__uint_as_float(__hip_atomic_load(ps + 64, __ATOMIC_RELAXED, __HIP_MEMORY_SCOPE_AGENT)) - mx);
                lsum = fmaf(w, __uint_as_float(__hip_atomic_load(ps + 65, __ATOMIC_RELAXED, __HIP_MEMORY_SCOPE_AGENT)), lsum);
                r = fmaf(w, __uint_as_float(__hip_atomic_load(ps + lane, __ATOMIC_RELAXED, __HIP_MEMORY_SCOPE_AGENT)), r);
            }
        }
    }
    const float v = r * (1.0f / lsum);
    uint32_t hi, mid, lo;
    split3_pk(v, 0.0f, hi, mid, lo);
    const int k = h * 64 + lane;
    a.pl_out[plane_elem(0, b, k)] = (bf16_t)hi;
    a.pl_out[plane_elem(1, b, k)] = (bf16_t)mid;
    a.pl_out[plane_elem(2, b, k)] = (bf16_t)lo;
}

template <typename KV>
__global__ __launch_bounds__(256) void attn_decode_kernel(const float* __restrict__ qp, const void* __restrict__ kp,
                                                          const void* __restrict__ vp, unsigned sb, unsigned sh, unsigned st,
                                                          unsigned th, const int* __restrict__ cw, const unsigned* __restrict__ ew,
                                                          const AttnArgs a) {
    __shared__ __attribute__((aligned(16))) float s_o[4][64];
    __shared__ float s_m[4], s_l[4];
    const int h = blockIdx.x, split = blockIdx.y, b = blockIdx.z;
    const int t_hi = (int)(th & 0xfffffu), n_heads = (int)(th >> 20);
    const int Tc = cw[1];
    const unsigned epoch = ew[0];
    const int T = (st >> 31) ? Tc : t_hi;
    const size_t stride_t = st & 0x7fffffffu;
    const int chunk0 = split * kAttnChunk;
    if (chunk0 >= t_hi) return;

    const int lane = threadIdx.x & 63, wave = threadIdx.x >> 6;
    const int lr = lane & 15, g = lane >> 4;
    const int base = chunk0 + wave * 64;

    const KV* K = reinterpret_cast<const KV*>(kp) + (size_t)b * sb + (size_t)h * sh;
    const KV* V = reinterpret_cast<const KV*>(vp) + (size_t)b * sb + (size_t)h * sh;
    const f32x4 q4 = *reinterpret_cast<const f32x4*>(qp + ((size_t)b * n_heads + h) * 64 + lr * 4);
    const float alpha = 0.125f;

    float m_w = kNegBig, l_w = 0.0f;
    f32x4 o4 = {0.0f, 0.0f, 0.0f, 0.0f};
    if (base < t_hi) {
        f32x4 k4[16], v4[16];
#pragma unroll
        for (int i = 0; i < 16; ++i) {
            const int t = min(base + 4 * i + g, t_hi - 1);
            k4[i] = load_kv4<KV>(K + (size_t)t * stride_t + lr * 4);
            v4[i] = load_kv4<KV>(V + (size_t)t * stride_t + lr * 4);
        }
        ZG_PIN(a.progress); ZG_PIN(a.part); ZG_PIN(a.max_splits); ZG_PIN(a.pl_out); ZG_PIN(a.part_tag); ZG_PIN(a.launch_id); ZG_PIN(a.merge_cnt); ZG_PIN(a.fault); ZG_PIN(a.spin_limit);
        pf_count(a.progress);
        float s[16];
#pragma unroll
        for (int i = 0; i < 16; ++i)
            s[i] = fmaf(q4.x, k4[i].x, fmaf(q4.y, k4[i].y, fmaf(q4.z, k4[i].z, q4.w * k4[i].w)));
        float sc = row16_reduce_scatter(s, lr) * alpha;
        const int t_mine = base + 4 * lr + g;
        if (t_mine >= T) sc = kNegBig;
        m_w = wave_allmax(sc);
        const float p = (t_mine < T) ? __expf(sc - m_w) : 0.0f;
        l_w = wave_allsum(p);
#define ZG_PV(i)                                                                                                         \
    {                                                                                                                    \
        const float pi = __uint_as_float(__builtin_amdgcn_update_dpp(0u, __float_as_uint(p), 0x150 + (i), 0xF, 0xF, false)); \
        o4.x = fmaf(pi, v4[i].x, o4.x);                                                                                  \
        o4.y = fmaf(pi, v4[i].y, o4.y);                                                                                  \
        o4.z = fmaf(pi, v4[i].z, o4.z);                                                                                  \
        o4.w = fmaf(pi, v4[i].w, o4.w);                                                                                  \
    }
        ZG_PV(0) ZG_PV(1) ZG_PV(2) ZG_PV(3) ZG_PV(4) ZG_PV(5) ZG_PV(6) ZG_PV(7)
        ZG_PV(8) ZG_PV(9) ZG_PV(10) ZG_PV(11) ZG_PV(12) ZG_PV(13) ZG_PV(14) ZG_PV(15)
#undef ZG_PV
        o4.x += __shfl_xor(o4.x, 16, 64); o4.y += __shfl_xor(o4.y, 16, 64);
        o4.z += __shfl_xor(o4.z, 16, 64); o4.w += __shfl_xor(o4.w, 16, 64);
        o4.x += __shfl_xor(o4.x, 32, 64); o4.y += __shfl_xor(o4.y, 32, 64);
        o4.z += __shfl_xor(o4.z, 32, 64); o4.w += __shfl_xor(o4.w, 32, 64);
    }
    if (lane < 16) *reinterpret_cast<f32x4*>(&s_o[wave][lane * 4]) = o4;
    if (lane == 0) {
        s_m[wave] = m_w;
        s_l[wave] = l_w;
    }
    __syncthreads();
    if (wave == 0) {
        const float M = fmaxf(fmaxf(s_m[0], s_m[1]), fmaxf(s_m[2], s_m[3]));
        float o = 0.0f, l = 0.0f;
#pragma unroll
        for (int w = 0; w < 4; ++w) {
            const float sc = __expf(s_m[w] - M);
            o = fmaf(sc, s_o[w][lane], o);
            l = fmaf(sc, s_l[w], l);
        }
        publish_partial(a, n_heads, (t_hi + kAttnChunk - 1) / kAttnChunk, b, h, split, lane, o, M, l, (epoch << 8) | a.launch_id);
    }
}

typedef __attribute__((ext_vector_type(8))) _Float16 h8;

__device__ __forceinline__ float grp8_reduce_scatter(float (&s)[8], int c) {
    float a4[4];
    {
        const bool hi = c & 4;
#pragma unroll
        for (int j = 0; j < 4; ++j) {
            const float keep = hi ? s[j + 4] : s[j];
            const float send = hi ? s[j] : s[j + 4];
            const float from_lo = dpp_row_ror<4>(send);
            const float from_hi = dpp_row_ror<12>(send);
            a4[j] = keep + (hi ? from_lo : from_hi);
        }
    }
    float a2[2];
    {
        const bool hi = c & 2;
#pragma unroll
        for (int j = 0; j < 2; ++j) {
            const float keep = hi ? a4[j + 2] : a4[j];
            const float send = hi ? a4[j] : a4[j + 2];
            const float from_lo = dpp_row_ror<2>(send);
            const float from_hi = dpp_row_ror<14>(send);
            a2[j] = keep + (hi ? from_lo : from_hi);
        }
    }
    const bool hi = c & 1;
    const float keep = hi ? a2[1] : a2[0];
    const float send = hi ? a2[0] : a2[1];
    const float from_lo = dpp_row_ror<1>(send);
    const float from_hi = dpp_row_ror<15>(send);
    return keep + (hi ? from_lo : from_hi);
}

template <int MODE>
struct Row8;
template <>
struct Row8<1> {
    h8 v;
    __device__ __forceinline__ void load(const void* base, size_t, size_t elem) { v = *reinterpret_cast<const h8*>(reinterpret_cast<const _Float16*>(base) + elem); }
    __device__ __forceinline__ float at(int e) const { return (float)v[e]; }
};
template <>
struct Row8<2> {
    u32x4 hi;
    u32x2 lo;
    __device__ __forceinline__ void load(const void* base, size_t lo_off, size_t elem) {
        hi = *reinterpret_cast<const u32x4*>(reinterpret_cast<const uint16_t*>(base) + elem);
        lo = *reinterpret_cast<const u32x2*>(reinterpret_cast<const uint8_t*>(base) + lo_off + elem);
    }
    __device__ __forceinline__ float at(int e) const {
        const uint32_t sel = ((e & 1) ? 0x07060000u : 0x05040000u) | ((uint32_t)(e & 3) << 8) | 0x0cu;
        return __uint_as_float(__builtin_amdgcn_perm(hi[e >> 1], lo[e >> 2], sel));
    }
};

template <int MODE>
__global__ __launch_bounds__(256) void attn_decode_h8_kernel(const float* __restrict__ qp0, const void* __restrict__ kp,
                                                             const void* __restrict__ vp, unsigned sb, unsigned sh, unsigned st,
                                                             unsigned th, const int* __restrict__ cw, const unsigned* __restrict__ ew,
                                                             const AttnArgs a) {
    __shared__ __attribute__((aligned(16))) float s_o[4][64];
    __shared__ float s_m[4], s_l[4];
    const int h = blockIdx.x, split = blockIdx.y, b = blockIdx.z;
    const int t_hi = (int)(th & 0xfffffu), n_heads = (int)(th >> 20);
    const int Tc = cw[1];
    const unsigned epoch = ew[0];
    const int T = (st >> 31) ? Tc : t_hi;
    const size_t stride_t = st & 0x7fffffffu;
    const int chunk0 = split * kAttnChunk;
    if (chunk0 >= t_hi) return;

    const int lane = threadIdx.x & 63, wave = threadIdx.x >> 6;
    const int c = lane & 7, g8 = lane >> 3;
    const int base = chunk0 + wave * 64;
    const size_t head0 = (size_t)b * sb + (size_t)h * sh;
    const float* qp = qp0 + ((size_t)b * n_heads + h) * 64 + c * 8;
    const f32x4 qa = *reinterpret_cast<const f32x4*>(qp), qb = *reinterpret_cast<const f32x4*>(qp + 4);
    const float q[8] = {qa.x, qa.y, qa.z, qa.w, qb.x, qb.y, qb.z, qb.w};
    const float alpha = 0.125f;

    float m_w = kNegBig, l_w = 0.0f;
    float o[8] = {0.0f, 0.0f, 0.0f, 0.0f, 0.0f, 0.0f, 0.0f, 0.0f};
    if (base < t_hi) {
        Row8<MODE> k8[8], v8[8];
#pragma unroll
        for (int i = 0; i < 8; ++i) {
            const int t = min(base + 8 * i + g8, t_hi - 1);
            k8[i].load(kp, a.kv_lo, head0 + (size_t)t * stride_t + c * 8);
            v8[i].load(vp, a.kv_lo, head0 + (size_t)t * stride_t + c * 8);
        }
        ZG_PIN(a.progress); ZG_PIN(a.part); ZG_PIN(a.max_splits); ZG_PIN(a.pl_out); ZG_PIN(a.part_tag); ZG_PIN(a.launch_id); ZG_PIN(a.merge_cnt); ZG_PIN(a.fault); ZG_PIN(a.spin_limit);
        pf_count(a.progress);
        float s[8];
#pragma unroll
        for (int i = 0; i < 8; ++i) {
            float acc = 0.0f;
#pragma unroll
            for (int e = 0; e < 8; ++e) acc = fmaf(q[e], k8[i].at(e), acc);
            s[i] = acc;
        }
        float sc = grp8_reduce_scatter(s, c) * alpha;
        const int t_mine = base + 8 * c + g8;
        if (t_mine >= T) sc = kNegBig;
        m_w = wave_allmax(sc);
        const float p = (t_mine < T) ? __expf(sc - m_w) : 0.0f;
        l_w = wave_allsum(p);
        const bool up = lane & 8;
#define ZG_PV8(i)                                                                                                          \
    {                                                                                                                      \
        const float plo = __uint_as_float(__builtin_amdgcn_update_dpp(0u, __float_as_uint(p), 0x150 + (i), 0xF, 0xF, false));     \
        const float phi = __uint_as_float(__builtin_amdgcn_update_dpp(0u, __float_as_uint(p), 0x150 + 8 + (i), 0xF, 0xF, false)); \
        const float pi = up ? phi : plo;                                                                                   \
        _Pragma("unroll") for (int e = 0; e < 8; ++e) o[e] = fmaf(pi, v8[i].at(e), o[e]);                              \
    }
        ZG_PV8(0) ZG_PV8(1) ZG_PV8(2) ZG_PV8(3) ZG_PV8(4) ZG_PV8(5) ZG_PV8(6) ZG_PV8(7)
#undef ZG_PV8
#pragma unroll
        for (int e = 0; e < 8; ++e) {
            o[e] += dpp_row_ror<8>(o[e]);
            o[e] += __shfl_xor(o[e], 16, 64);
            o[e] += __shfl_xor(o[e], 32, 64);
        }
    }
    if (lane < 8) {
        *reinterpret_cast<f32x4*>(&s_o[wave][lane * 8]) = f32x4{o[0], o[1], o[2], o[3]};
        *reinterpret_cast<f32x4*>(&s_o[wave][lane * 8 + 4]) = f32x4{o[4], o[5], o[6], o[7]};
    }
    if (lane == 0) {
        s_m[wave] = m_w;
        s_l[wave] = l_w;
    }
    __syncthreads();
    if (wave == 0) {
        const float M = fmaxf(fmaxf(s_m[0], s_m[1]), fmaxf(s_m[2], s_m[3]));
        float ov = 0.0f, l = 0.0f;
#pragma unroll
        for (int w = 0; w < 4; ++w) {
            const float sc = __expf(s_m[w] - M);
            ov = fmaf(sc, s_o[w][lane], ov);
            l = fmaf(sc, s_l[w], l);
        }
        publish_partial(a, n_heads, (t_hi + kAttnChunk - 1) / kAttnChunk, b, h, split, lane, ov, M, l, (epoch << 8) | a.launch_id);
    }
}

__global__ __launch_bounds__(256) void attn_merge_kernel(const float* part, int n_heads, int max_splits,
                                                         int seq_len, float* out) {
    const int b = blockIdx.y;
    const int e = blockIdx.x * 256 + threadIdx.x;
// ... 135 lines not shown
```

### zig_gpt2_amd/csrc/gemv_internal.h

```cpp
#pragma once
#include <stdlib.h>

#include "zg_kernels.h"

#ifdef ZG_STAMPS
#define ZG_STAMP_DECL() unsigned long long zg_ts[8] = {0, 0, 0, 0, 0, 0, 0, 0}
#define ZG_STAMP(i) zg_ts[i] = __builtin_amdgcn_s_memtime()
#define ZG_STAMP_FLUSH()                                                                              \
    if (a.dbg && threadIdx.x == 0 && (blockIdx.x == 0 || blockIdx.x == gridDim.x - 1)) {             \
        const unsigned long long slot = atomicAdd(a.dbg, 1ull);                                       \
        unsigned long long* d = a.dbg + 16 + slot * 10;                                               \
        for (int i = 0; i < 8; ++i) d[i] = zg_ts[i];                                                  \
        d[8] = blockIdx.x;                                                                            \
        d[9] = __builtin_amdgcn_s_memtime();                                                          \
    }
#else
#define ZG_STAMP_DECL()
#define ZG_STAMP(i)
#define ZG_STAMP_FLUSH()
#endif

namespace zg {

namespace {
// ... 155 lines not shown
            ls[s] = ps[65];
            const float2 lo = *reinterpret_cast<const float2*>(ps + d0);
            const float2 hi = *reinterpret_cast<const float2*>(ps + d0 + 2);
            o[s][0] = lo.x; o[s][1] = lo.y; o[s][2] = hi.x; o[s][3] = hi.y;
        }
#pragma unroll
        for (int s = 0; s < MAXS; ++s)
            if (s >= nsplit) ms[s] = -1e30f;
        const float mx = fmaxf(fmaxf(ms[0], ms[1]), fmaxf(ms[2], ms[3]));
        float l = 0.0f;
        float r[4] = {0.0f, 0.0f, 0.0f, 0.0f};
#pragma unroll
        for (int s = 0; s < MAXS; ++s) {
            const float w = __expf(ms[s] - mx);
            l = fmaf(w, ls[s], l);
#pragma unroll
            for (int j = 0; j < 4; ++j) r[j] = fmaf(w, o[s][j], r[j]);
        }
        const float inv = 1.0f / l;
        return f32x4{r[0] * inv, r[1] * inv, r[2] * inv, r[3] * inv};
    }
    float mx = -1e30f;
    for (int s = 0; s < nsplit; ++s) mx = fmaxf(mx, p[s * kPartStride + 64]);
    float l = 0.0f;
    float r[4] = {0.0f, 0.0f, 0.0f, 0.0f};
    for (int s = 0; s < nsplit; ++s) {
        const float w = __expf(p[s * kPartStride + 64] - mx);
        l = fmaf(w, p[s * kPartStride + 65], l);
#pragma unroll
        for (int j = 0; j < 4; ++j) r[j] = fmaf(w, p[s * kPartStride + d0 + j], r[j]);
    }
    const float inv = 1.0f / l;
    return f32x4{r[0] * inv, r[1] * inv, r[2] * inv, r[3] * inv};
}

template <typename WT, int LPR, int CPL>
__device__ __forceinline__ void load_pass(Raw<WT> (&w)[CPL], const WT* W, int K, int nch, int row, int n_rows,
                                          int lr) {
    const WT* wp = W + (size_t)max(min(row, n_rows - 1), 0) * K;
#pragma unroll
    for (int i = 0; i < CPL; ++i) w[i] = load_raw(wp, min(lr + LPR * i, nch - 1));
}

template <int MT>
struct RowExtra {
    float bias;
    float resid[MT];
};
template <int MT>
__device__ __forceinline__ RowExtra<MT> load_extra(const GemvArgs& a, int epilogue, int M, int N, int r) {
    RowExtra<MT> e;
    const int rr = min(r, N - 1);
    e.bias = *(a.bias ? a.bias + rr : a.zero);
#pragma unroll
    for (int m = 0; m < MT; ++m)
        e.resid[m] = *((epilogue == EPI_RESIDUAL && m < M) ? a.resid + (size_t)m * a.resid_stride + rr : a.zero);
    return e;
}

template <int NJ>
__device__ __forceinline__ void ln_strip(const float* __restrict__ xin, const float* __restrict__ ln_g,
                                         const float* __restrict__ ln_b, f32x4* xw4, int nq, int K, float eps,
                                         int lane) {
    f32x4 v[NJ], g4[NJ], b4[NJ];
#pragma unroll
    for (int j = 0; j < NJ; ++j) {
        const int ic = min(lane + 64 * j, nq - 1);
        v[j] = reinterpret_cast<const f32x4*>(xin)[ic];
        g4[j] = reinterpret_cast<const f32x4*>(ln_g)[ic];
        b4[j] = reinterpret_cast<const f32x4*>(ln_b)[ic];
    }
#pragma unroll
    for (int j = 0; j < NJ; ++j)
        if (lane + 64 * j >= nq) v[j] = f32x4{0.0f, 0.0f, 0.0f, 0.0f};
    float t1 = 0.0f, t2 = 0.0f;
#pragma unroll
    for (int j = 0; j < NJ; ++j) {
        t1 += (v[j].x + v[j].y) + (v[j].z + v[j].w);
        t2 = fmaf(v[j].x, v[j].x, fmaf(v[j].y, v[j].y, fmaf(v[j].z, v[j].z, fmaf(v[j].w, v[j].w, t2))));
    }
    t1 = wave_allsum(t1);
    t2 = wave_allsum(t2);
    const float inv_k = 1.0f / (float)K;
    const float mean = t1 * inv_k;
    const float rstd = __builtin_amdgcn_rsqf(t2 * inv_k - mean * mean + eps);
#pragma unroll
    for (int j = 0; j < NJ; ++j) {
        const int i = lane + 64 * j;
        if (i < nq) {
            f32x4 o;
            o.x = fmaf((v[j].x - mean) * rstd, g4[j].x, b4[j].x);
            o.y = fmaf((v[j].y - mean) * rstd, g4[j].y, b4[j].y);
            o.z = fmaf((v[j].z - mean) * rstd, g4[j].z, b4[j].z);
            o.w = fmaf((v[j].w - mean) * rstd, g4[j].w, b4[j].w);
            xw4[i] = o;
        }
    }
}

typedef __attribute__((ext_vector_type(8))) __bf16 mf_bf16x8;
typedef __attribute__((ext_vector_type(4))) float mf_f32x4;

constexpr int kMfmaRows = 8;

__device__ __forceinline__ void store_split4(char* planes, int S, int m, int k, f32x4 v) {
    uint32_t h0, m0, l0, h1, m1, l1;
    split3_pk(v.x, v.y, h0, m0, l0);
    split3_pk(v.z, v.w, h1, m1, l1);
    const u32x2 h = {h0, h1}, md = {m0, m1}, l = {l0, l1};
    const size_t off = (size_t)m * S + (size_t)k * 2;
    const size_t plane = (size_t)kMfmaRows * S;
    *reinterpret_cast<u32x2*>(planes + off) = h;
    *reinterpret_cast<u32x2*>(planes + plane + off) = md;
    *reinterpret_cast<u32x2*>(planes + 2 * plane + off) = l;
}

inline int lm_wpt_steps(const GemvArgs& a) {
    const int off = decode_paths_off() & 32;
    if (off || a.epilogue != EPI_ARGMAX || a.prologue != PRO_LAYERNORM || a.M < 2 || a.M > kMfmaRows || a.K % 32 != 0) return 0;
    const int ns = a.K / 32;
    return (ns == 12 || ns == 24 || ns == 32) ? ns : 0;
}
inline int lm_wpt_tiles_per_wg() {
    constexpr int v = 8;
    return v >= 4 ? (v / 4) * 4 : 4;
}

inline int gemv_mfma_waves(const GemvArgs& a) { return a.epilogue == EPI_ARGMAX ? 4 : 16; }

inline size_t gemv_mfma_lds(int K, int nw, bool alias_partial = false, bool line = false, bool gpl = false) {
    const size_t planes = gpl ? 0 : (size_t)3 * kMfmaRows * (2 * K + 16);
    return planes + 64 * sizeof(float) + (alias_partial ? 0 : (size_t)2 * nw * 64 * 4 * sizeof(float)) + (line ? (size_t)nw * 2048 : 0);
}
inline bool gemv_mfma_line(int K, int nw, bool alias_partial, bool gpl = false) {
    const int off = decode_paths_off() & 16;
    return !off && !alias_partial && K % 64 == 0 && gemv_mfma_lds(K, nw, false, true, gpl) <= 160 * 1024;
}

inline bool gemv_mfma_alias(const GemvArgs& a) {
    return a.kslices <= 1 && a.epilogue != EPI_ARGMAX && a.rows_per_wave == 1 && gemv_mfma_lds(a.K, 16) > 160 * 1024;
}

inline int pl4_pairs(const GemvArgs& a) {
    const int off = decode_paths_off() & 2;
    if (off || a.pl_in == nullptr || a.epilogue == EPI_ARGMAX || a.rows_per_wave != 1) return 0;
    if (a.N > 0xffff || (a.prologue == PRO_LAYERNORM && a.x_stride != a.K) || (a.epilogue == EPI_RESIDUAL && a.resid_stride != a.N)) return 0;
    if (a.st_in != nullptr && a.K / 16 > 128) return 0;
    const int ksl = a.kslices > 1 ? a.kslices : 1;
    if (a.K % (64 * ksl) != 0) return 0;
    const int kp = (a.K / ksl / 64 + 3) / 4;
    return kp <= 5 ? kp : 0;
}

}

bool gemv_use_ksplit(const GemvArgs& a);
bool gemv_use_lnk(const GemvArgs& a);
int gemv_launch_ksplit(const GemvArgs& a, int weight_type, hipStream_t s);
int gemv_launch_lnk(const GemvArgs& a, int weight_type, hipStream_t s);
int gemv_launch_valu(const GemvArgs& a, int weight_type, int grid, hipStream_t s);
int gemv_launch_mfma16(const GemvArgs& a, int grid, hipStream_t s);
int gemv_launch_pl4(const GemvArgs& a, int pairs, int grid, hipStream_t s);
int gemv_launch_lm_wpt(const GemvArgs& a, int steps, int grid, hipStream_t s);

}
```

### zig_gpt2_amd/csrc/gemv_ksplit.hip

```cpp
#include "gemv_internal.h"

namespace zg {

namespace {

template <typename WT, int LPR, int CPL, int NP = 2>
__global__ __launch_bounds__(256) void gemv_ksplit_kernel(const void* __restrict__ Wv, const float* __restrict__ xin, int N,
                                                          int K, unsigned em, const float* __restrict__ part_in, int max_splits,
                                                          const float* __restrict__ bias, const float* __restrict__ resid,
                                                          const GemvArgs a) {
    const int epilogue = (int)(em & 0xffu), merge_splits = (int)((em >> 8) & 0xffu);
    const int has_bias = (int)((em >> 16) & 1u), has_resid = (int)((em >> 17) & 1u);
    ZG_STAMP_DECL();
    ZG_STAMP(0);
    constexpr int RPP = 64 / LPR, ROWS = NP * RPP;
    __shared__ float part[4][ROWS];
    const int tid = threadIdx.x, lane = tid & 63;
    const int wave = __builtin_amdgcn_readfirstlane(tid >> 6);
    const int lr = lane % LPR, rsub = lane / LPR;
    const int Kq = K >> 2, nchq = Kq >> 3;
    const WT* W = reinterpret_cast<const WT*>(Wv) + (size_t)wave * Kq;
    const int row0 = blockIdx.x * ROWS;
    Raw<WT> wq[NP][CPL];
#pragma unroll
    for (int p = 0; p < NP; ++p) {
        const WT* pr = W + (size_t)min(row0 + p * RPP + rsub, N - 1) * K;
#pragma unroll
        for (int i = 0; i < CPL; ++i) wq[p][i] = load_raw(pr, min(lr + LPR * i, nchq - 1));
    }
    W8 xr[CPL];
    if (merge_splits > 0) {
        constexpr int MAXS = 4;
        const int nsplit = merge_splits;
#pragma unroll
        for (int i = 0; i < CPL; ++i) {
            const int e0 = wave * Kq + min(lr + LPR * i, nchq - 1) * 8;
            const int h = e0 >> 6, d0 = e0 & 63;
            const float* p = part_in + ((size_t)h * max_splits) * kPartStride;
            float ms[MAXS], ls[MAXS];
            W8 o[MAXS];
#pragma unroll
            for (int sp = 0; sp < MAXS; ++sp) {
                const float* ps = p + min(sp, nsplit - 1) * kPartStride;
                ms[sp] = ps[64];
                ls[sp] = ps[65];
                const float2 a0 = *reinterpret_cast<const float2*>(ps + d0), a1 = *reinterpret_cast<const float2*>(ps + d0 + 2);
                const float2 a2 = *reinterpret_cast<const float2*>(ps + d0 + 4), a3 = *reinterpret_cast<const float2*>(ps + d0 + 6);
                o[sp].v[0] = a0.x; o[sp].v[1] = a0.y; o[sp].v[2] = a1.x; o[sp].v[3] = a1.y;
                o[sp].v[4] = a2.x; o[sp].v[5] = a2.y; o[sp].v[6] = a3.x; o[sp].v[7] = a3.y;
            }
#pragma unroll
            for (int sp = 0; sp < MAXS; ++sp)
                if (sp >= nsplit) ms[sp] = -1e30f;
            const float mx = fmaxf(fmaxf(ms[0], ms[1]), fmaxf(ms[2], ms[3]));
            float l = 0.0f;
            W8 r = zero_w8();
#pragma unroll
            for (int sp = 0; sp < MAXS; ++sp) {
                const float w = __expf(ms[sp] - mx);
                l = fmaf(w, ls[sp], l);
#pragma unroll
                for (int j = 0; j < 8; ++j) r.v[j] = fmaf(w, o[sp].v[j], r.v[j]);
            }
            const float inv = 1.0f / l;
#pragma unroll
            for (int j = 0; j < 8; ++j) xr[i].v[j] = r.v[j] * inv;
        }
    } else {
#pragma unroll
        for (int i = 0; i < CPL; ++i) xr[i] = load_x8(xin + (size_t)wave * Kq + (size_t)min(lr + LPR * i, nchq - 1) * 8);
    }
    float bias_n = 0.0f, resid_n = 0.0f;
    if (tid < ROWS) {
        const int n = min(row0 + tid, N - 1);
        bias_n = bias[n * has_bias];
        resid_n = resid[n * has_resid];
    }
    ZG_STAMP(1);
    ZG_PIN(a.y);
    ZG_PIN(a.progress);
    pf_count(a.progress);
    ZG_STAMP(2);
#pragma unroll
    for (int i = 0; i < CPL; ++i)
        if (lr + LPR * i >= nchq) xr[i] = zero_w8();
    auto dot = [&](const Raw<WT>(&w)[CPL]) {
        float p0 = 0.0f, p1 = 0.0f, p2 = 0.0f, p3 = 0.0f;
#pragma unroll
        for (int i = 0; i < CPL; ++i) {
            const W8 u = unpack(w[i]);
            p0 = fmaf(u.v[0], xr[i].v[0], p0); p1 = fmaf(u.v[1], xr[i].v[1], p1);
            p2 = fmaf(u.v[2], xr[i].v[2], p2); p3 = fmaf(u.v[3], xr[i].v[3], p3);
            p0 = fmaf(u.v[4], xr[i].v[4], p0); p1 = fmaf(u.v[5], xr[i].v[5], p1);
            p2 = fmaf(u.v[6], xr[i].v[6], p2); p3 = fmaf(u.v[7], xr[i].v[7], p3);
        }
        return group_allsum<LPR>((p0 + p1) + (p2 + p3));
    };
    float sp[NP];
#pragma unroll
    for (int p = 0; p < NP; ++p) sp[p] = dot(wq[p]);
    ZG_STAMP(3);
    if (lr == 0) {
#pragma unroll
        for (int p = 0; p < NP; ++p) part[wave][p * RPP + rsub] = sp[p];
    }
    __syncthreads();
    ZG_STAMP(4);
    if (tid < ROWS && row0 + tid < N) {
        const int n = row0 + tid;
        const float v = ((part[0][tid] + part[1][tid]) + (part[2][tid] + part[3][tid])) + bias_n;
        a.y[n] = epilogue == EPI_RESIDUAL ? v + resid_n : (epilogue == EPI_GELU ? gelu_ref(v) : v);
    }
    ZG_STAMP(5);
    ZG_STAMP(6);
    ZG_STAMP(7);
    ZG_STAMP_FLUSH();
}

template <typename WT>
int launch_ksplit(const GemvArgs& a, hipStream_t s) {
    const int nchq = a.K / 32;
    const int merge_splits = a.prologue == PRO_ATTN_MERGE ? (a.t_hi + kAttnChunk - 1) / kAttnChunk : 0;
    const unsigned has_resid = a.epilogue == EPI_RESIDUAL ? 1u : 0u;
    const unsigned em = (unsigned)a.epilogue | ((unsigned)merge_splits << 8) | ((a.bias ? 1u : 0u) << 16) | (has_resid << 17);
#define ZG_KS(LPR_, CPL_)                                                                                                \
    {                                                                                                                    \
        constexpr int rows = 2 * (64 / LPR_);                                                                            \
        note_kernel("gemv_ksplit_kernel<%s, %d, %d, 2>", sizeof(WT) == 2 ? "unsigned short" : "float", LPR_, CPL_);         \
        hipLaunchKernelGGL((gemv_ksplit_kernel<WT, LPR_, CPL_, 2>), dim3((a.N + rows - 1) / rows), dim3(256), 0, s, a.W,     \
                           a.x,                                                                                         \
                           a.N, a.K, em, a.part ? a.part : a.zero, a.max_splits, a.bias ? a.bias : a.zero,              \
                           has_resid ? a.resid : a.zero, a);                                                             \
        ZG_HIP(hipGetLastError());                                                                                       \
        return ZG_OK;                                                                                                    \
    }
    if (nchq <= 16 * 2) ZG_KS(16, 2)
    if (nchq <= 32 * 3) ZG_KS(32, 3)
    if (nchq <= 32 * 5) ZG_KS(32, 5)
    if (nchq <= 32 * 7) ZG_KS(32, 7)
    if (nchq <= 64 * 4) ZG_KS(64, 4)
#undef ZG_KS
    zg::set_error("gemv (K split): K=%d too large", a.K);
    return ZG_ERR_UNSUPPORTED;
}


template <typename WT, int LPR, int CPL, int NP = 2>
__global__ __launch_bounds__(256) void gemv_lnk_kernel(const void* __restrict__ Wv, const float* __restrict__ xin, unsigned ne, int K,
                                                       const float* __restrict__ ln_g, const float* __restrict__ c2,
                                                       const float* __restrict__ c3, const int* __restrict__ cw,
                                                       const GemvArgs a) {
    const int N = (int)(ne & 0xffffffu), epilogue = (int)(ne >> 24);
    ZG_STAMP_DECL();
    ZG_STAMP(0);
    constexpr int RPP = 64 / LPR, ROWS = NP * RPP;
    __shared__ float part[4][ROWS];
    __shared__ float stat[4][2];
    const int tid = threadIdx.x, lane = tid & 63;
    const int wave = __builtin_amdgcn_readfirstlane(tid >> 6);
    const int lr = lane % LPR, rsub = lane / LPR;
    int kbeg, nchq;
    if (sizeof(WT) == 2 && (K & 63) == 0 && ((K >> 6) & 3) != 0 && (((K >> 6) >> 2) + 1) * 8 <= LPR * CPL) {
        const int lines = K >> 6, base = lines >> 2, rem = lines & 3;
        kbeg = (wave * base + min(wave, rem)) * 64;
        nchq = (base + (wave < rem ? 1 : 0)) * 8;
    } else {
        kbeg = wave * (K >> 2);
        nchq = K >> 5;
    }
    const WT* W = reinterpret_cast<const WT*>(Wv) + kbeg;
    const int row0 = blockIdx.x * ROWS;
    Raw<WT> wq[NP][CPL];
#pragma unroll
    for (int p = 0; p < NP; ++p) {
        const WT* pr = W + (size_t)min(row0 + p * RPP + rsub, N - 1) * K;
#pragma unroll
        for (int i = 0; i < CPL; ++i) wq[p][i] = load_raw(pr, min(lr + LPR * i, nchq - 1));
    }
    W8 xr[CPL], gr[CPL];
#pragma unroll
    for (int i = 0; i < CPL; ++i) {
        const size_t off = (size_t)kbeg + (size_t)min(lr + LPR * i, nchq - 1) * 8;
        xr[i] = load_x8(xin + off);
        gr[i] = load_x8(ln_g + off);
    }
    float c2n = 0.0f, c3n = 0.0f;
    if (tid < ROWS) {
        const int n = min(row0 + tid, N - 1);
        c2n = c2[n];
        c3n = c3[n];
    }
    const int T = max(cw[1], 1);
    ZG_STAMP(1);
    {
        ZG_PIN(a.progress); ZG_PIN(a.y); ZG_PIN(a.y_stride); ZG_PIN(a.epilogue); ZG_PIN(__float_as_uint(a.eps));
        if (epilogue == EPI_QKV) {
            ZG_PIN(a.q); ZG_PIN(a.k_cache); ZG_PIN(a.v_cache); ZG_PIN(a.N); ZG_PIN(a.head_dim); ZG_PIN(a.n_heads); ZG_PIN(a.ctx); ZG_PIN(a.kv_mode); ZG_PIN(a.kv_lo);
        }
    }
    pf_count(a.progress);
    ZG_STAMP(2);
    float sx = 0.0f, sxx = 0.0f;
#pragma unroll
    for (int i = 0; i < CPL; ++i) {
        if (lr + LPR * i >= nchq) xr[i] = zero_w8();
#pragma unroll
        for (int j = 0; j < 8; ++j) {
            sx += xr[i].v[j];
            sxx = fmaf(xr[i].v[j], xr[i].v[j], sxx);
            xr[i].v[j] *= gr[i].v[j];
        }
    }
    sx = group_allsum<LPR>(sx);
    sxx = group_allsum<LPR>(sxx);
    auto dot = [&](const Raw<WT>(&w)[CPL]) {
        float p0 = 0.0f, p1 = 0.0f, p2 = 0.0f, p3 = 0.0f;
#pragma unroll
        for (int i = 0; i < CPL; ++i) {
            const W8 u = unpack(w[i]);
            p0 = fmaf(u.v[0], xr[i].v[0], p0); p1 = fmaf(u.v[1], xr[i].v[1], p1);
            p2 = fmaf(u.v[2], xr[i].v[2], p2); p3 = fmaf(u.v[3], xr[i].v[3], p3);
            p0 = fmaf(u.v[4], xr[i].v[4], p0); p1 = fmaf(u.v[5], xr[i].v[5], p1);
            p2 = fmaf(u.v[6], xr[i].v[6], p2); p3 = fmaf(u.v[7], xr[i].v[7], p3);
        }
        return group_allsum<LPR>((p0 + p1) + (p2 + p3));
    };
    float sp[NP];
#pragma unroll
    for (int p = 0; p < NP; ++p) sp[p] = dot(wq[p]);
    ZG_STAMP(3);
    if (lr == 0) {
#pragma unroll
        for (int p = 0; p < NP; ++p) part[wave][p * RPP + rsub] = sp[p];
    }
    if (lane == 0) {
        stat[wave][0] = sx;
        stat[wave][1] = sxx;
    }
    __syncthreads();
    ZG_STAMP(4);
    if (tid < ROWS && row0 + tid < N) {
        const int n = row0 + tid;
        const float inv_k = 1.0f / (float)K;
        const float mean = ((stat[0][0] + stat[1][0]) + (stat[2][0] + stat[3][0])) * inv_k;
        const float ex2 = ((stat[0][1] + stat[1][1]) + (stat[2][1] + stat[3][1])) * inv_k;
        const float rstd = __builtin_amdgcn_rsqf(ex2 - mean * mean + a.eps);
        const float S1 = (part[0][tid] + part[1][tid]) + (part[2][tid] + part[3][tid]);
        const float y = fmaf(rstd, fmaf(-mean, c2n, S1), c3n);
        Best nobest;
        epilogue_row(a, 0, n, y, 0.0f, 0.0f, T - 1, nobest);
    }
    ZG_STAMP(5);
    ZG_STAMP(6);
    ZG_STAMP(7);
    ZG_STAMP_FLUSH();
}

template <typename WT>
__global__ __launch_bounds__(256) void ln_fold_kernel(const void* __restrict__ Wv, const float* __restrict__ g,
                                                      const float* __restrict__ b, const float* __restrict__ bias, int N, int K,
                                                      float* __restrict__ c2, float* __restrict__ c3) {
    const int lane = threadIdx.x & 63, row = blockIdx.x * 4 + (threadIdx.x >> 6);
    if (row >= N) return;
    const WT* w = reinterpret_cast<const WT*>(Wv) + (size_t)row * K;
    float s2 = 0.0f, s3 = 0.0f;
    for (int k = lane; k < K; k += 64) {
        float wv;
        if constexpr (sizeof(WT) == 2) wv = __uint_as_float((uint32_t)w[k] << 16);
        else wv = w[k];
        s2 = fmaf(wv, g[k], s2);
        s3 = fmaf(wv, b[k], s3);
    }
    s2 = wave_allsum(s2);
    s3 = wave_allsum(s3);
    if (lane == 0) {
        c2[row] = s2;
        c3[row] = s3 + (bias ? bias[row] : 0.0f);
    }
}

template <typename WT>
int launch_lnk(const GemvArgs& a, hipStream_t s) {
    const int nchq = a.K / 32;
#define ZG_LK(LPR_, CPL_)                                                                                              \
    {                                                                                                                  \
        constexpr int rows = 4 * (64 / LPR_);                                                                          \
        note_kernel("gemv_lnk_kernel<%s, %d, %d, 4>", sizeof(WT) == 2 ? "unsigned short" : "float", LPR_, CPL_);       \
        hipLaunchKernelGGL((gemv_lnk_kernel<WT, LPR_, CPL_, 4>), dim3((a.N + rows - 1) / rows), dim3(256), 0, s, a.W, a.x, \
                           (unsigned)a.N | ((unsigned)a.epilogue << 24), a.K, a.ln_g, a.ln_c2, a.ln_c3,                 \
                           a.ctrl ? reinterpret_cast<const int*>(a.ctrl) : reinterpret_cast<const int*>(a.zero), a);   \
        ZG_HIP(hipGetLastError());                                                                                     \
        return ZG_OK;                                                                                                  \
    }
    if (nchq <= 16 * 2) ZG_LK(16, 2)
    if (nchq <= 32 * 2) ZG_LK(32, 2)
    if (nchq <= 32 * 3) ZG_LK(32, 3)
    if (nchq <= 64 * 2) ZG_LK(64, 2)
#undef ZG_LK
    zg::set_error("gemv (LayerNorm, K split): K=%d too large", a.K);
    return ZG_ERR_UNSUPPORTED;
}



}

bool gemv_use_ksplit(const GemvArgs& a) {
    if (a.M != 1) return false;
    if (a.epilogue != EPI_STORE && a.epilogue != EPI_RESIDUAL && a.epilogue != EPI_GELU) return false;
    if (a.prologue == PRO_ATTN_MERGE)
        return a.head_dim == 64 && a.t_hi > 0 && (a.t_hi + kAttnChunk - 1) / kAttnChunk <= 4 && a.K % 32 == 0 && a.K <= 1024;
    if (a.prologue != PRO_NONE) return false;
    return a.K >= 2048 && a.K % 32 == 0 && a.K / 32 <= 256;
}

bool gemv_use_lnk(const GemvArgs& a) {
    if (a.M != 1 || a.prologue != PRO_LAYERNORM || a.ln_c2 == nullptr || a.ln_c3 == nullptr) return false;
    if (a.epilogue != EPI_STORE && a.epilogue != EPI_GELU && a.epilogue != EPI_QKV) return false;
    return a.K % 32 == 0 && a.K / 32 <= 128 && a.N <= 16384;
}

int gemv_launch_ksplit(const GemvArgs& a, int weight_type, hipStream_t s) {
    return weight_type == WT_BF16 ? launch_ksplit<bf16_t>(a, s) : launch_ksplit<float>(a, s);
}
int gemv_launch_lnk(const GemvArgs& a, int weight_type, hipStream_t s) {
    return weight_type == WT_BF16 ? launch_lnk<bf16_t>(a, s) : launch_lnk<float>(a, s);
}

int launch_ln_fold(const void* W, int weight_type, const float* g, const float* b, const float* bias, int N, int K, float* c2,
                   float* c3, hipStream_t s) {
    if (weight_type == WT_BF16)
        hipLaunchKernelGGL((ln_fold_kernel<bf16_t>), dim3((N + 3) / 4), dim3(256), 0, s, W, g, b, bias, N, K, c2, c3);
    else
        hipLaunchKernelGGL((ln_fold_kernel<float>), dim3((N + 3) / 4), dim3(256), 0, s, W, g, b, bias, N, K, c2, c3);
    ZG_HIP(hipGetLastError());
    return ZG_OK;
}

}
```

### zig_gpt2_amd/csrc/zg_kernels.h

```cpp
#pragma once
#include "zg_common.h"

namespace zg {

struct StepCtrl {
    int step;
    int seq_len;
    int mode;
    int n_partials;
};

enum GemvPrologue { PRO_NONE = 0, PRO_LAYERNORM = 1, PRO_ATTN_MERGE = 2 };
enum GemvEpilogue { EPI_STORE = 0, EPI_RESIDUAL = 1, EPI_GELU = 2, EPI_QKV = 3, EPI_ARGMAX = 4 };
enum WeightType { WT_BF16 = 0, WT_F32 = 1 };

constexpr int kAttnChunk = 256;
constexpr int kPartStride = 64 + 2;

struct GemvArgs {
    const void* W;
    const float* bias;
    int N, K, M;
    int rows_per_wave;
    int waves_per_wg;
    int prologue, epilogue;
    const float* x;
    int x_stride;
    const float* ln_g;
    const float* ln_b;
    float eps;
    const float* ln_c2;
    const float* ln_c3;
    const float* part;
    int n_heads, head_dim, max_splits;
    const StepCtrl* ctrl;
    int t_hi;
    float* y;
    int y_stride;
    const float* resid;
    int resid_stride;
    float* q;
    void* k_cache;
    void* v_cache;
    int ctx;
    int kv_mode;
    size_t kv_lo;
    float* logits;
    int logits_stride;
    float* part_val;
    int* part_idx;
    float* sk_ws;
    int* sk_cnt;
    int sk_tiles;
    int kslices;
    const bf16_t* pl_in;
    bf16_t* pl_out;
    const float* pl_g;
    const unsigned* epoch;
    unsigned launch_id;
    unsigned long long* sk_tag;
    unsigned* fault;
    unsigned spin_limit;
    float* st_out;
    const float* st_in;
    const float* zero;
    unsigned long long* dbg;
    unsigned* progress;
};

bool gemv_supported(const GemvArgs& a, int weight_type);
bool gemv_planes_ok(const GemvArgs& a, int weight_type);
bool gemv_planes_producer_ok(const GemvArgs& a, int weight_type);
bool gemv_pl4_ok(const GemvArgs& a, int weight_type);
int gemv_plan(GemvArgs& a, int weight_type = WT_F32);
int gemv_kslices(const GemvArgs& a);
int gemv_rows_per_wg(const GemvArgs& a, int weight_type);
int launch_ln_fold(const void* W, int weight_type, const float* g, const float* b, const float* bias, int N, int K, float* c2,
                   float* c3, hipStream_t s);
int launch_gemv(const GemvArgs& a, int weight_type, int grid, hipStream_t s);

struct AttnArgs {
    const float* q;
    const void* k;
    const void* v;
    long stride_b, stride_h, stride_t;
    int kv_mode;
    size_t kv_lo;
    int n_heads, head_dim, batch;
    const StepCtrl* ctrl;
    int seq_len;
    int t_hi;
    int max_splits;
    float* part;
    unsigned* progress;
    bf16_t* pl_out;
    int* merge_cnt;
    const unsigned* epoch;
    unsigned launch_id;
    unsigned long long* part_tag;
    unsigned* fault;
    unsigned spin_limit;
};
int launch_attn_decode(const AttnArgs& a, hipStream_t s);
int launch_attn_any_dim(const float* q, const float* k, const float* v, long stride_b, long stride_h, long stride_t, int batch, int n_heads,
                        int head_dim, int seq_len, float* out, hipStream_t s);
int launch_attn_merge(const float* part, int batch, int n_heads, int head_dim, int max_splits,
                      int seq_len, float* out, hipStream_t s);

int launch_epoch_bump(unsigned* epoch, hipStream_t s);
int launch_layernorm(float* x, int rows, int n, const float* g, const float* b, float eps, hipStream_t s, unsigned* done_flag = nullptr,
                     unsigned done_seq = 0, bool* announced = nullptr, float* shadow = nullptr);
int launch_gelu(float* x, size_t n, hipStream_t s, unsigned* done_flag = nullptr, unsigned done_seq = 0, bool* announced = nullptr, float* shadow = nullptr);
int launch_softmax(float* x, size_t n, hipStream_t s, unsigned* done_flag = nullptr, unsigned done_seq = 0, bool* announced = nullptr);
int launch_done_flag(unsigned* flag, unsigned seq, hipStream_t s);
struct CopySegs {
    const void* src[4];
    void* dst[4];
    unsigned bytes[4];
    int n;
};
int launch_copy_out_done(const CopySegs& segs, unsigned* flag, unsigned seq, hipStream_t s);
int launch_copy2_f32(const float* a, float* da, const float* b, float* db, size_t n, hipStream_t s);
int launch_embedding(const float* w, size_t emb_dim, const size_t* idx, size_t n_idx, size_t n_rows,
                     float* out, int* d_oob_flag, hipStream_t s, unsigned* done_flag = nullptr, unsigned done_seq = 0, bool* announced = nullptr);
int launch_split_qkv(const float* in, size_t rows, size_t n_embed, size_t split_idx, float* out, hipStream_t s);
int launch_transpose(const float* in, size_t batch, size_t t, size_t n, size_t h, float* out, hipStream_t s);
int launch_copy_f32(const float* in, float* out, size_t n, hipStream_t s);
int launch_f32_to_bf16(const float* in, bf16_t* out, size_t n, hipStream_t s);
int launch_split3(const float* in, size_t rows, int K, bf16_t* out, hipStream_t s);
int launch_kv_clear_tail(void* base, int n_caches, size_t cache_stride, size_t plane_off, int row_bytes, int strips, int ctx, int from_row,
                         hipStream_t s);

int launch_gemm_bf16_nt(const bf16_t* A, const bf16_t* B, const float* bias, void* C, int M, int N, int K, int ldc,
                        bool gelu, bool out_bf16, hipStream_t s);
struct GemmPlanes {
    int lda, ldb;
    int kpp;
    int npairs;
    unsigned pa_bits, pb_bits;
    bool b_plane_major;
};
int launch_gemm_planes(const bf16_t* A, const bf16_t* B, const float* bias, void* C, int M, int N, const GemmPlanes& pl,
                       int ldc, bool gelu, bool out_bf16, hipStream_t s);
int launch_gemm_s4(const bf16_t* A, const bf16_t* B, const float* bias, void* C, int M, int N, const GemmPlanes& pl, int ldc,
                   bool gelu, bool out_bf16, int bn, hipStream_t s);
bool gemm_s4_args_ok(const GemmPlanes& pl, int ldc);
enum { S4_PLAIN = 0, S4_PARTIAL = 1, S4_QKV = 2, S4_SPLIT3 = 3 };
struct PrefillQkv;
int launch_gemm_s4_prefill(const bf16_t* A, const bf16_t* W, const float* bias, void* C, int M, int N, int K, int nplanes, int kind, int n_slices,
                           const PrefillQkv* qkv, hipStream_t s);
int gemm_s4_stamps(unsigned long long* out, size_t n_words);
int gemm_s4_fault(unsigned* out);
int gemm_debug_stamps(unsigned long long* out, size_t n_words);
unsigned long long gemm_mfma_launch_count();
void gemm_note_launch();

constexpr int kSplit = 3;
enum PrefillEpilogue { PF_F32 = 0, PF_RESID = 1, PF_GELU_SPLIT = 2, PF_PARTIAL = 3 , PF_QKV = 4 };
int launch_embed_prefill(const int* tokens, int token_stride, int B, int P, const void* wte, const void* wpe,
                         int weight_type, int E, float* x, hipStream_t s);
int launch_ln_split(const float* x, int M, int E, const float* g, const float* b, float eps, bf16_t* out, hipStream_t s);
struct PrefillQkv {
    int P, E, H, ctx, kv_mode;
    void* k_cache;
    void* v_cache;
    size_t kv_lo;
    void* sk_ws = nullptr;
    size_t sk_ws_bytes = 0;
    unsigned* sk_flags = nullptr;
    unsigned sk_flags_words = 0;
    unsigned sk_epoch = 0;
};
struct PrefillLn {
    const float* g;
    const float* b;
    float eps;
    bf16_t* out;
};
int launch_prefill_gemm(const bf16_t* A, const bf16_t* W, const float* bias, void* C, int M, int N, int K, int ldc, int epi,
                        float* ws, size_t ws_floats, const PrefillLn* ln, hipStream_t s, const PrefillQkv* qkv = nullptr,
                        int nsplit = kSplit);
constexpr int kWeightPlanes = 33;
void prefill_force_route(int kernel, int slices);
int launch_attn_prefill(const float* qkv, bf16_t* out, int B, int P, int E, int H, float* ws, size_t ws_floats, const float* k_cache_or_null,
                        const float* v_cache_or_null, int ctx, hipStream_t s, int force_tiles = 0);

int launch_sample(float* logits, int batch, int vocab, float temp, const float* u, const float* part_val, int n_part, int part_stride, float* seg_ws,
                  int* token_out, bool write_probs, hipStream_t s);
size_t sample_workspace_floats(int batch);

struct EmbedArgs {
    StepCtrl* ctrl;
    const float* part_val;
    const int* part_idx;
    int part_stride;
    int n_partials;
    const int* prompt;
    const int* prompt_len;
    int batch;
    int prompt_stride;
    const int* forced;
    const void* wte;
    const void* wpe;
    int weight_type;
    int n_embed, vocab;
    int* cur_token;
    int* out_tokens;
    int out_stride;
    float* x;
    bf16_t* pl_out;
    const float* pl_g;
    unsigned* epoch;
    float* st_out;
    int finish_only;
    unsigned* progress;
    const int* sampled;
};
int launch_embed_step(const EmbedArgs& a, hipStream_t s);
struct SampleParams {
    float inv_temp;
    unsigned pad;
    unsigned long long seed;
};
int launch_sample_step(float* logits, int batch, int vocab, const SampleParams* params, const StepCtrl* ctrl, const float* part_val, int n_part,
                       int part_stride, float* seg_ws, int* token_out, hipStream_t s);

int dist_broadcast(void* buf, size_t bytes, int root, hipStream_t s);

enum PfKind { PF_NONE = 0, PF_WEIGHTS = 1, PF_KV = 2 };
constexpr unsigned PF_STOP = 0xffffffffu;
struct PfJob {
    const char* base;
    const char* base2;
    size_t total_bytes;
    unsigned wg_bytes, n_wg;
    unsigned touch_bytes;
    unsigned kind;
    unsigned n_heads, ctx, batch, row_bytes;
    unsigned cls;
    unsigned pad;
    const char* aux[3];
    unsigned aux_bytes[3];
    unsigned pad2;
};
struct alignas(8) PfCtl {
    unsigned progress;
    unsigned base_xcd;
    unsigned sink_guard, sink;
    unsigned ticket[8];
    unsigned exit_reason[8];
    unsigned jobs_done[8];
    unsigned xcd_log[256];
};
struct PfArgs {
    PfCtl* ctl;
    const PfJob* jobs;
    int njobs;
    int lead;
    int nsub;
    int max_T;
    unsigned idle_limit;
    unsigned sleep;
    unsigned cls_mask;
    unsigned line_shift;
    unsigned cap_bytes;
};
int launch_prefetcher(const PfArgs& a, hipStream_t s);

__device__ __forceinline__ void pf_count(unsigned* progress) {
    if (progress != nullptr && (blockIdx.x | blockIdx.y | blockIdx.z | threadIdx.x) == 0) {
#ifdef ZG_STAMPS
        const unsigned old = __hip_atomic_fetch_add(progress, 1u, __ATOMIC_RELAXED, __HIP_MEMORY_SCOPE_AGENT);
        reinterpret_cast<PfCtl*>(progress)->xcd_log[old & 255u] = 0x100u | (__builtin_amdgcn_s_getreg((3 << 11) | 20) & 15u);
#else
        __hip_atomic_fetch_add(progress, 1u, __ATOMIC_RELAXED, __HIP_MEMORY_SCOPE_AGENT);
#endif
    }
}

}
```

Measured before the change: 4723 tokens/s.

## Fuse QKV layernorm-GEMV and attention decode into one kernel launch

Adds a fused kernel path in which the c_attn LayerNorm-GEMV and the attention decode for a layer run in a single launch. QKV outputs are published through epoch/launch-id tagged 64-bit slots that the attention part spin-waits on. The path is enabled by default for batch 1 and removes one kernel launch plus the boundary between the two kernels in every layer. In exchange it relies on spin-wait synchronisation with a fault fallback, adds tag memory that must be cleared periodically, and moves the attention code into a shared header.

```diff
diff --git a/zig_gpt2_amd/csrc/api_gpt.hip b/zig_gpt2_amd/csrc/api_gpt.hip
--- a/zig_gpt2_amd/csrc/api_gpt.hip
+++ b/zig_gpt2_amd/csrc/api_gpt.hip
@@ -53,6 +53,9 @@
     size_t sk_tag_bytes, part_tag_bytes;
     size_t epochs_since_clear;
     bool tags_on;
+    unsigned long long* qkv_tag;
+    size_t qkv_tag_bytes;
+    bool fused_on;
     float* xst;
     bool st_on;
     bool pl_on;
@@ -180,6 +183,8 @@
     g->sk_tag_bytes = ((E + 15) / 16) * 4 * 128 * 8;
     g->part_tag_bytes = 8 * c.n_heads * g->max_splits * kPartStride * 8;
     g->sk_tag = (unsigned long long*)P(g->sk_tag_bytes);
+    g->qkv_tag_bytes = 3 * E * 8;
+    g->qkv_tag = (unsigned long long*)P(g->qkv_tag_bytes);
     g->part_tag = (unsigned long long*)P(g->part_tag_bytes);
     g->sk_tiles = (int)((E + 15) / 16);
     g->sk_ws = (float*)P((size_t)g->sk_tiles * 4 * 128 * 4);
@@ -258,7 +263,7 @@
     e.x = g->x;
     e.pl_out = g->pl_on ? g->xp : nullptr;
     e.pl_g = g->layers[0].ln_1_g;
-    e.epoch = (g->pl_on && g->tags_on && finish_only != 1 && finish_only != 2) ? g->epoch : nullptr;
+    e.epoch = (((g->pl_on && g->tags_on) || g->fused_on) && finish_only != 1 && finish_only != 2) ? g->epoch : nullptr;
     e.st_out = g->st_on ? g->xst : nullptr;
     e.finish_only = finish_only;
     e.progress = g->pf_on ? &g->pf_ctl->progress : nullptr;
@@ -348,6 +353,47 @@
 
 int env_int(const char* name, int dflt);
 
+GemvArgs c_attn_args(const zg_gpt* g, const zg_layer& y, int t_hi) {
+    const size_t E = g->cfg.n_embed;
+    GemvArgs a = base_gemv(g, y.c_attn_w, y.c_attn_b, 3 * E, E, t_hi);
+    a.prologue = PRO_LAYERNORM;
+    a.x = g->x;
+    a.x_stride = (int)E;
+    a.ln_g = y.ln_1_g;
+    a.ln_b = y.ln_1_b;
+    a.ln_c2 = y.c_attn_c2;
+    a.ln_c3 = y.c_attn_c3;
+    a.epilogue = EPI_QKV;
+    a.pl_in = g->pl_on ? g->xp : nullptr;
+    a.st_in = g->st_on ? g->xst : nullptr;
+    a.q = g->q;
+    a.k_cache = y.k_cache;
+    a.v_cache = y.v_cache;
+    return a;
+}
+
+AttnArgs attn_args(const zg_gpt* g, const zg_layer& y, int t_hi) {
+    const size_t E = g->cfg.n_embed;
+    AttnArgs a{};
+    a.q = g->q;
+    a.k = y.k_cache;
+    a.v = y.v_cache;
+    a.stride_b = (long)(g->cfg.context_size * E);
+    a.stride_h = (long)(g->cfg.context_size * 64);
+    a.stride_t = 64;
+    a.kv_mode = g->kv_mode;
+    a.kv_lo = g->batch * g->cfg.context_size * E * 2;
+    a.n_heads = (int)g->cfg.n_heads;
+    a.head_dim = 64;
+    a.batch = (int)g->batch;
+    a.ctrl = g->ctrl;
+    a.t_hi = t_hi;
+    a.max_splits = g->max_splits;
+    a.part = g->part;
+    a.progress = g->pf_on ? &g->pf_ctl->progress : nullptr;
+    return a;
+}
+
 int enqueue_step(zg_gpt* g, bool with_logits, int t_hi, hipStream_t s, StepProf* prof = nullptr, int only = -1, size_t only_layer = 0,
                  std::vector<PfJob>* rec = nullptr, int salt = -1, bool with_sampler = false) {
     const size_t E = g->cfg.n_embed;
@@ -361,43 +407,25 @@
     ZG_TRY(prof_mark(prof, 0, s));
     for (size_t l = (only < 0 ? 0 : only_layer); l < (only < 0 ? g->cfg.n_layer : only_layer + 1); ++l) {
         const zg_layer& y = g->layers[l];
-        if (only < 0 || only == 1) {
-            GemvArgs a = base_gemv(g, y.c_attn_w, y.c_attn_b, 3 * E, E, t_hi);
-            a.prologue = PRO_LAYERNORM;
-            a.x = g->x;
-            a.x_stride = (int)E;
-            a.ln_g = y.ln_1_g;
-            a.ln_b = y.ln_1_b;
-            a.ln_c2 = y.c_attn_c2;
-            a.ln_c3 = y.c_attn_c3;
-            a.epilogue = EPI_QKV;
-            a.pl_in = g->pl_on ? g->xp : nullptr;
-            a.st_in = g->st_on ? g->xst : nullptr;
-            a.q = g->q;
-            a.k_cache = y.k_cache;
-            a.v_cache = y.v_cache;
+        const bool fused = g->fused_on && !rec && 2 * l + 2 <= 255;
+        if (fused && (only < 0 || only == 1)) {
+            GemvArgs a = c_attn_args(g, y, t_hi);
+            AttnArgs at = attn_args(g, y, t_hi);
+            at.launch_id = launch_id(l, 0);
+            at.fault = g->fault;
+            at.spin_limit = g->spin_limit;
+            ZG_TRY(launch_attn_qkv(a, g->wt, at, g->epoch, g->qkv_tag, s));
+            ZG_TRY(prof_mark(prof, 1, s));
+            ZG_TRY(prof_mark(prof, 2, s));
+        }
+        if (!fused && (only < 0 || only == 1)) {
+            GemvArgs a = c_attn_args(g, y, t_hi);
             const int grid = gemv_plan(a, g->wt);
             ZG_TRY(emit_gemv(g, a, grid, s, rec, 1));
             ZG_TRY(prof_mark(prof, 1, s));
         }
-        if (only < 0 || only == 2) {
-            AttnArgs a{};
-            a.q = g->q;
-            a.k = y.k_cache;
-            a.v = y.v_cache;
-            a.stride_b = (long)(g->cfg.context_size * E);
-            a.stride_h = (long)(g->cfg.context_size * 64);
-            a.stride_t = 64;
-            a.kv_mode = g->kv_mode;
-            a.kv_lo = g->batch * g->cfg.context_size * E * 2;
-            a.n_heads = (int)g->cfg.n_heads;
-            a.head_dim = 64;
-            a.batch = (int)g->batch;
-            a.ctrl = g->ctrl;
-            a.t_hi = t_hi;
-            a.max_splits = g->max_splits;
-            a.part = g->part;
-            a.progress = g->pf_on ? &g->pf_ctl->progress : nullptr;
+        if ((!fused && only < 0) || only == 2) {
+            AttnArgs a = attn_args(g, y, t_hi);
             if (g->pl_on) {
                 a.pl_out = g->ap;
                 a.merge_cnt = g->attn_cnt;
@@ -548,7 +576,7 @@
         g->sk_used = false;
         ZG_TRY(gemm_s4_fault(&sk));
     }
-    if (g->tags_on) {
+    if (g->tags_on || g->fused_on) {
         volatile unsigned* f = g->fault;
         tag = *f;
         if (tag) *f = 0;
@@ -565,12 +593,13 @@
 }
 
 int note_steps(zg_gpt* g, size_t n, hipStream_t s) {
-    if (!g->tags_on) return ZG_OK;
+    if (!g->tags_on && !g->fused_on) return ZG_OK;
     g->epochs_since_clear += n;
     if (g->epochs_since_clear < ((size_t)1 << 23)) return ZG_OK;
     g->epochs_since_clear = n;
     ZG_HIP(hipMemsetAsync(g->sk_tag, 0, g->sk_tag_bytes, s));
     ZG_HIP(hipMemsetAsync(g->part_tag, 0, g->part_tag_bytes, s));
+    ZG_HIP(hipMemsetAsync(g->qkv_tag, 0, g->qkv_tag_bytes, s));
     return ZG_OK;
 }
 
@@ -873,6 +902,8 @@
     }
     g->tags_on = g->pl_on && !(decode_paths_off() & 4);
     g->spin_limit = (unsigned)env_int("ZGPT2_TAG_SPIN_LIMIT", 1 << 20);
+    g->fused_on = batch == 1 && !(decode_paths_off() & 64) && c.n_layer <= 127 &&
+                  attn_qkv_ok(c_attn_args(g, g->layers[0], 0), attn_args(g, g->layers[0], (int)c.context_size));
     g->st_on = false;
     if (g->pl_on && !(decode_paths_off() & 8) && c.n_embed % 16 == 0 && c.n_embed / 16 <= 128) {
         const zg_layer& y = g->layers[0];
@@ -1516,7 +1547,7 @@
     hipGraphExec_t exec = nullptr;
     ZG_HIP(hipStreamBeginCapture(s, hipStreamCaptureModeThreadLocal));
     int st = ZG_OK;
-    if (g->tags_on && which != 0) st = launch_epoch_bump(g->epoch, s);
+    if ((g->tags_on || g->fused_on) && which != 0) st = launch_epoch_bump(g->epoch, s);
     for (int i = 0; i < chain && st == ZG_OK; ++i)
         st = enqueue_step(g, true, bucket_t_hi(g, T), s, nullptr, which, cycle ? (size_t)i % g->cfg.n_layer : 0, nullptr, i);
     hipError_t ce = hipStreamEndCapture(s, &graph);
diff --git a/zig_gpt2_amd/csrc/attn.hip b/zig_gpt2_amd/csrc/attn.hip
--- a/zig_gpt2_amd/csrc/attn.hip
+++ b/zig_gpt2_amd/csrc/attn.hip
@@ -1,309 +1,18 @@
 #include <stdlib.h>
 
-#include "zg_kernels.h"
+#include "attn_decode.h"
 #include "zg_runtime.h"
 
 namespace zg {
 
 namespace {
-
-constexpr float kNegBig = -1e30f;
-
-template <typename KV>
-__device__ __forceinline__ f32x4 load_kv4(const KV* p);
-template <>
-__device__ __forceinline__ f32x4 load_kv4<float>(const float* p) {
-    return *reinterpret_cast<const f32x4*>(p);
-}
-template <>
-__device__ __forceinline__ f32x4 load_kv4<_Float16>(const _Float16* p) {
-    typedef __attribute__((ext_vector_type(4))) _Float16 h4;
-    const h4 v = *reinterpret_cast<const h4*>(p);
-    f32x4 r;
-    r.x = (float)v.x; r.y = (float)v.y; r.z = (float)v.z; r.w = (float)v.w;
-    return r;
-}
-
-__device__ __forceinline__ float row16_reduce_scatter(float (&s)[16], int lr) {
-    float a8[8];
-    {
-        const bool hi = lr & 8;
-#pragma unroll
-        for (int j = 0; j < 8; ++j) {
-            const float keep = hi ? s[j + 8] : s[j];
-            const float send = hi ? s[j] : s[j + 8];
-            a8[j] = keep + dpp_row_ror<8>(send);
-        }
-    }
-    float a4[4];
-    {
-        const bool hi = lr & 4;
-#pragma unroll
-        for (int j = 0; j < 4; ++j) {
-            const float keep = hi ? a8[j + 4] : a8[j];
-            const float send = hi ? a8[j] : a8[j + 4];
-            const float from_lo = dpp_row_ror<4>(send);
-            const float from_hi = dpp_row_ror<12>(send);
-            a4[j] = keep + (hi ? from_lo : from_hi);
-        }
-    }
-    float a2[2];
-    {
-        const bool hi = lr & 2;
-#pragma unroll
-        for (int j = 0; j < 2; ++j) {
-            const float keep = hi ? a4[j + 2] : a4[j];
-            const float send = hi ? a4[j] : a4[j + 2];
-            const float from_lo = dpp_row_ror<2>(send);
-            const float from_hi = dpp_row_ror<14>(send);
-            a2[j] = keep + (hi ? from_lo : from_hi);
-        }
-    }
-    {
-        const bool hi = lr & 1;
-        const float keep = hi ? a2[1] : a2[0];
-        const float send = hi ? a2[0] : a2[1];
-        const float from_lo = dpp_row_ror<1>(send);
-        const float from_hi = dpp_row_ror<15>(send);
-        return keep + (hi ? from_lo : from_hi);
-    }
-}
-
-__device__ __forceinline__ void publish_partial(const AttnArgs& a, int n_heads, int nsplit, int b, int h, int split, int lane, float o,
-                                                float M, float l, unsigned tag) {
-    float* part = a.part + (((size_t)b * n_heads + h) * a.max_splits + split) * kPartStride;
-    if (a.pl_out == nullptr) {
-        part[lane] = o;
-        if (lane == 0) {
-            part[64] = M;
-            part[65] = l;
-        }
-        return;
-    }
-    float r = o, lsum = l;
-    if (nsplit > 1 && a.part_tag) {
-        typedef unsigned long long u64;
-        auto pack = [&](float v) { return ((u64)tag << 32) | (u64)__float_as_uint(v); };
-        u64* pt0 = a.part_tag + ((size_t)b * n_heads + h) * a.max_splits * kPartStride;
-        const int last = nsplit - 1;
-        if (split != last) {
-            u64* pt = pt0 + split * kPartStride;
-            __hip_atomic_store(pt + lane, pack(o), __ATOMIC_RELAXED, __HIP_MEMORY_SCOPE_AGENT);
-            if (lane == 0) {
-                __hip_atomic_store(pt + 64, pack(M), __ATOMIC_RELAXED, __HIP_MEMORY_SCOPE_AGENT);
-                __hip_atomic_store(pt + 65, pack(l), __ATOMIC_RELAXED, __HIP_MEMORY_SCOPE_AGENT);
-            }
-            return;
-        }
-        float mx = M;
-        r = 0.0f;
-        lsum = 0.0f;
-        constexpr int MAXS = 4;
-        if (nsplit <= MAXS) {
-            u64 vo[MAXS - 1], vm[MAXS - 1], vl[MAXS - 1];
-            for (int spins = 0;; ++spins) {
-                bool ok = true;
-#pragma unroll
-                for (int s = 0; s < MAXS - 1; ++s) {
-                    const u64* ps = pt0 + min(s, last - 1) * kPartStride;
-                    vo[s] = __hip_atomic_load(ps + lane, __ATOMIC_RELAXED, __HIP_MEMORY_SCOPE_AGENT);
-                    vm[s] = __hip_atomic_load(ps + 64, __ATOMIC_RELAXED, __HIP_MEMORY_SCOPE_AGENT);
-                    vl[s] = __hip_atomic_load(ps + 65, __ATOMIC_RELAXED, __HIP_MEMORY_SCOPE_AGENT);
-                    ok = ok && (unsigned)(vo[s] >> 32) == tag && (unsigned)(vm[s] >> 32) == tag && (unsigned)(vl[s] >> 32) == tag;
-                }
-                if (__builtin_amdgcn_ballot_w64(!ok) == 0) break;
-                if ((unsigned)spins >= a.spin_limit) {
-                    if (lane == 0 && a.fault) __hip_atomic_store(a.fault, 1u, __ATOMIC_RELAXED, __HIP_MEMORY_SCOPE_AGENT);
-                    break;
-                }
-                __builtin_amdgcn_s_sleep(1);
-            }
-            float ms[MAXS], ls[MAXS], os[MAXS];
-#pragma unroll
-            for (int s = 0; s < MAXS; ++s) {
-                const bool polled = s < last && s < MAXS - 1;
-                ms[s] = polled ? __uint_as_float((unsigned)vm[s < MAXS - 1 ? s : 0]) : s == last ? M : -1e30f;
-                ls[s] = polled ? __uint_as_float((unsigned)vl[s < MAXS - 1 ? s : 0]) : l;
-                os[s] = polled ? __uint_as_float((unsigned)vo[s < MAXS - 1 ? s : 0]) : o;
-            }
-            mx = fmaxf(fmaxf(ms[0], ms[1]), fmaxf(ms[2], ms[3]));
-#pragma unroll
-            for (int s = 0; s < MAXS; ++s) {
-                const float w = __expf(ms[s] - mx);
-                lsum = fmaf(w, ls[s], lsum);
-                r = fmaf(w, os[s], r);
-            }
-        } else {
-            float mrun = -1e30f;
-            for (int s = 0; s <= last; ++s) {
-                float m_s = M, o_s = o, l_s = l;
-                if (s < last) {
-                    const u64* ps = pt0 + s * kPartStride;
-                    u64 vo, vm, vl;
-                    for (int spins = 0;; ++spins) {
-                        vo = __hip_atomic_load(ps + lane, __ATOMIC_RELAXED, __HIP_MEMORY_SCOPE_AGENT);
-                        vm = __hip_atomic_load(ps + 64, __ATOMIC_RELAXED, __HIP_MEMORY_SCOPE_AGENT);
-                        vl = __hip_atomic_load(ps + 65, __ATOMIC_RELAXED, __HIP_MEMORY_SCOPE_AGENT);
-                        const bool ok = (unsigned)(vo >> 32) == tag && (unsigned)(vm >> 32) == tag && (unsigned)(vl >> 32) == tag;
-                        if (__builtin_amdgcn_ballot_w64(!ok) == 0) break;
-                        if ((unsigned)spins >= a.spin_limit) {
-                            if (lane == 0 && a.fault) __hip_atomic_store(a.fault, 1u, __ATOMIC_RELAXED, __HIP_MEMORY_SCOPE_AGENT);
-                            break;
-                        }
-                        __builtin_amdgcn_s_sleep(1);
-                    }
-                    m_s = __uint_as_float((unsigned)vm);
-                    o_s = __uint_as_float((unsigned)vo);
-                    l_s = __uint_as_float((unsigned)vl);
-                }
-                const float mnew = fmaxf(mrun, m_s);
-                const float w0 = __expf(mrun - mnew), w1 = __expf(m_s - mnew);
-                r = fmaf(w1, o_s, r * w0);
-                lsum = fmaf(w1, l_s, lsum * w0);
-                mrun = mnew;
-            }
-        }
-    } else if (nsplit > 1) {
-        typedef __attribute__((address_space(1))) unsigned gu32;
-        gu32* gp = (gu32*)part;
-        __hip_atomic_store(gp + lane, __float_as_uint(o), __ATOMIC_RELAXED, __HIP_MEMORY_SCOPE_AGENT);
-        if (lane == 0) {
-            __hip_atomic_store(gp + 64, __float_as_uint(M), __ATOMIC_RELAXED, __HIP_MEMORY_SCOPE_AGENT);
-            __hip_atomic_store(gp + 65, __float_as_uint(l), __ATOMIC_RELAXED, __HIP_MEMORY_SCOPE_AGENT);
-        }
-        asm volatile("s_waitcnt vmcnt(0)" ::: "memory");
-        int* cnt = a.merge_cnt + b * n_heads + h;
-        int ticket = 0;
-        if (lane == 0) ticket = __hip_atomic_fetch_add(cnt, 1, __ATOMIC_RELAXED, __HIP_MEMORY_SCOPE_AGENT);
-        ticket = __builtin_amdgcn_readfirstlane(ticket);
-        if (ticket != nsplit - 1) return;
-        if (lane == 0) __hip_atomic_store(cnt, 0, __ATOMIC_RELAXED, __HIP_MEMORY_SCOPE_AGENT);
-        const gu32* p0 = (const gu32*)(a.part + ((size_t)b * n_heads + h) * a.max_splits * kPartStride);
-        constexpr int MAXS = 4;
-        if (nsplit <= MAXS) {
-            float ms[MAXS], ls[MAXS], os[MAXS];
-#pragma unroll
-            for (int s = 0; s < MAXS; ++s) {
-                const gu32* ps = p0 + min(s, nsplit - 1) * kPartStride;
-                ms[s] = __uint_as_float(__hip_atomic_load(ps + 64, __ATOMIC_RELAXED, __HIP_MEMORY_SCOPE_AGENT));
-                ls[s] = __uint_as_float(__hip_atomic_load(ps + 65, __ATOMIC_RELAXED, __HIP_MEMORY_SCOPE_AGENT));
-                os[s] = __uint_as_float(__hip_atomic_load(ps + lane, __ATOMIC_RELAXED, __HIP_MEMORY_SCOPE_AGENT));
-            }
-#pragma unroll
-            for (int s = 0; s < MAXS; ++s)
-                if (s >= nsplit) ms[s] = -1e30f;
-            const float mx = fmaxf(fmaxf(ms[0], ms[1]), fmaxf(ms[2], ms[3]));
-            r = 0.0f;
-            lsum = 0.0f;
-#pragma unroll
-            for (int s = 0; s < MAXS; ++s) {
-                const float w = __expf(ms[s] - mx);
-                lsum = fmaf(w, ls[s], lsum);
-                r = fmaf(w, os[s], r);
-            }
-        } else {
-            float mx = -1e30f;
-            for (int s = 0; s < nsplit; ++s)
-                mx = fmaxf(mx, __uint_as_float(__hip_atomic_load(p0 + s * kPartStride + 64, __ATOMIC_RELAXED, __HIP_MEMORY_SCOPE_AGENT)));
-            r = 0.0f;
-            lsum = 0.0f;
-            for (int s = 0; s < nsplit; ++s) {
-                const gu32* ps = p0 + s * kPartStride;
-                const float w = __expf(__uint_as_float(__hip_atomic_load(ps + 64, __ATOMIC_RELAXED, __HIP_MEMORY_SCOPE_AGENT)) - mx);
-                lsum = fmaf(w, __uint_as_float(__hip_atomic_load(ps + 65, __ATOMIC_RELAXED, __HIP_MEMORY_SCOPE_AGENT)), lsum);
-                r = fmaf(w, __uint_as_float(__hip_atomic_load(ps + lane, __ATOMIC_RELAXED, __HIP_MEMORY_SCOPE_AGENT)), r);
-            }
-        }
-    }
-    const float v = r * (1.0f / lsum);
-    uint32_t hi, mid, lo;
-    split3_pk(v, 0.0f, hi, mid, lo);
-    const int k = h * 64 + lane;
-    a.pl_out[plane_elem(0, b, k)] = (bf16_t)hi;
-    a.pl_out[plane_elem(1, b, k)] = (bf16_t)mid;
-    a.pl_out[plane_elem(2, b, k)] = (bf16_t)lo;
-}
 
 template <typename KV>
 __global__ __launch_bounds__(256) void attn_decode_kernel(const float* __restrict__ qp, const void* __restrict__ kp,
                                                           const void* __restrict__ vp, unsigned sb, unsigned sh, unsigned st,
                                                           unsigned th, const int* __restrict__ cw, const unsigned* __restrict__ ew,
                                                           const AttnArgs a) {
-    __shared__ __attribute__((aligned(16))) float s_o[4][64];
-    __shared__ float s_m[4], s_l[4];
-    const int h = blockIdx.x, split = blockIdx.y, b = blockIdx.z;
-    const int t_hi = (int)(th & 0xfffffu), n_heads = (int)(th >> 20);
-    const int Tc = cw[1];
-    const unsigned epoch = ew[0];
-    const int T = (st >> 31) ? Tc : t_hi;
-    const size_t stride_t = st & 0x7fffffffu;
-    const int chunk0 = split * kAttnChunk;
-    if (chunk0 >= t_hi) return;
-
-    const int lane = threadIdx.x & 63, wave = threadIdx.x >> 6;
-    const int lr = lane & 15, g = lane >> 4;
-    const int base = chunk0 + wave * 64;
-
-    const KV* K = reinterpret_cast<const KV*>(kp) + (size_t)b * sb + (size_t)h * sh;
-    const KV* V = reinterpret_cast<const KV*>(vp) + (size_t)b * sb + (size_t)h * sh;
-    const f32x4 q4 = *reinterpret_cast<const f32x4*>(qp + ((size_t)b * n_heads + h) * 64 + lr * 4);
-    const float alpha = 0.125f;
-
-    float m_w = kNegBig, l_w = 0.0f;
-    f32x4 o4 = {0.0f, 0.0f, 0.0f, 0.0f};
-    if (base < t_hi) {
-        f32x4 k4[16], v4[16];
-#pragma unroll
-        for (int i = 0; i < 16; ++i) {
-            const int t = min(base + 4 * i + g, t_hi - 1);
-            k4[i] = load_kv4<KV>(K + (size_t)t * stride_t + lr * 4);
-            v4[i] = load_kv4<KV>(V + (size_t)t * stride_t + lr * 4);
-        }
-        ZG_PIN(a.progress); ZG_PIN(a.part); ZG_PIN(a.max_splits); ZG_PIN(a.pl_out); ZG_PIN(a.part_tag); ZG_PIN(a.launch_id); ZG_PIN(a.merge_cnt); ZG_PIN(a.fault); ZG_PIN(a.spin_limit);
-        pf_count(a.progress);
-        float s[16];
-#pragma unroll
-        for (int i = 0; i < 16; ++i)
-            s[i] = fmaf(q4.x, k4[i].x, fmaf(q4.y, k4[i].y, fmaf(q4.z, k4[i].z, q4.w * k4[i].w)));
-        float sc = row16_reduce_scatter(s, lr) * alpha;
-        const int t_mine = base + 4 * lr + g;
-        if (t_mine >= T) sc = kNegBig;
-        m_w = wave_allmax(sc);
-        const float p = (t_mine < T) ? __expf(sc - m_w) : 0.0f;
-        l_w = wave_allsum(p);
-#define ZG_PV(i)                                                                                                         \
-    {                                                                                                                    \
-        const float pi = __uint_as_float(__builtin_amdgcn_update_dpp(0u, __float_as_uint(p), 0x150 + (i), 0xF, 0xF, false)); \
-        o4.x = fmaf(pi, v4[i].x, o4.x);                                                                                  \
-        o4.y = fmaf(pi, v4[i].y, o4.y);                                                                                  \
-        o4.z = fmaf(pi, v4[i].z, o4.z);                                                                                  \
-        o4.w = fmaf(pi, v4[i].w, o4.w);                                                                                  \
-    }
-        ZG_PV(0) ZG_PV(1) ZG_PV(2) ZG_PV(3) ZG_PV(4) ZG_PV(5) ZG_PV(6) ZG_PV(7)
-        ZG_PV(8) ZG_PV(9) ZG_PV(10) ZG_PV(11) ZG_PV(12) ZG_PV(13) ZG_PV(14) ZG_PV(15)
-#undef ZG_PV
-        o4.x += __shfl_xor(o4.x, 16, 64); o4.y += __shfl_xor(o4.y, 16, 64);
-        o4.z += __shfl_xor(o4.z, 16, 64); o4.w += __shfl_xor(o4.w, 16, 64);
-        o4.x += __shfl_xor(o4.x, 32, 64); o4.y += __shfl_xor(o4.y, 32, 64);
-        o4.z += __shfl_xor(o4.z, 32, 64); o4.w += __shfl_xor(o4.w, 32, 64);
-    }
-    if (lane < 16) *reinterpret_cast<f32x4*>(&s_o[wave][lane * 4]) = o4;
-    if (lane == 0) {
-        s_m[wave] = m_w;
-        s_l[wave] = l_w;
-    }
-    __syncthreads();
-    if (wave == 0) {
-        const float M = fmaxf(fmaxf(s_m[0], s_m[1]), fmaxf(s_m[2], s_m[3]));
-        float o = 0.0f, l = 0.0f;
-#pragma unroll
-        for (int w = 0; w < 4; ++w) {
-            const float sc = __expf(s_m[w] - M);
-            o = fmaf(sc, s_o[w][lane], o);
-            l = fmaf(sc, s_l[w], l);
-        }
-        publish_partial(a, n_heads, (t_hi + kAttnChunk - 1) / kAttnChunk, b, h, split, lane, o, M, l, (epoch << 8) | a.launch_id);
-    }
+    attn_decode_body<KV, false>((int)blockIdx.x, (int)blockIdx.y, (int)blockIdx.z, qp, kp, vp, sb, sh, st, th, cw, ew, a, nullptr);
 }
 
 typedef __attribute__((ext_vector_type(8))) _Float16 h8;
diff --git a/zig_gpt2_amd/csrc/attn_decode.h b/zig_gpt2_amd/csrc/attn_decode.h
--- /dev/null
+++ b/zig_gpt2_amd/csrc/attn_decode.h
@@ -0,0 +1,354 @@
+#pragma once
+#include "zg_kernels.h"
+
+namespace zg {
+
+namespace {
+
+constexpr float kNegBig = -1e30f;
+
+template <typename KV>
+__device__ __forceinline__ f32x4 load_kv4(const KV* p);
+template <>
+__device__ __forceinline__ f32x4 load_kv4<float>(const float* p) {
+    return *reinterpret_cast<const f32x4*>(p);
+}
+template <>
+__device__ __forceinline__ f32x4 load_kv4<_Float16>(const _Float16* p) {
+    typedef __attribute__((ext_vector_type(4))) _Float16 h4;
+    const h4 v = *reinterpret_cast<const h4*>(p);
+    f32x4 r;
+    r.x = (float)v.x; r.y = (float)v.y; r.z = (float)v.z; r.w = (float)v.w;
+    return r;
+}
+
+__device__ __forceinline__ float row16_reduce_scatter(float (&s)[16], int lr) {
+    float a8[8];
+    {
+        const bool hi = lr & 8;
+#pragma unroll
+        for (int j = 0; j < 8; ++j) {
+            const float keep = hi ? s[j + 8] : s[j];
+            const float send = hi ? s[j] : s[j + 8];
+            a8[j] = keep + dpp_row_ror<8>(send);
+        }
+    }
+    float a4[4];
+    {
+        const bool hi = lr & 4;
+#pragma unroll
+        for (int j = 0; j < 4; ++j) {
+            const float keep = hi ? a8[j + 4] : a8[j];
+            const float send = hi ? a8[j] : a8[j + 4];
+            const float from_lo = dpp_row_ror<4>(send);
+            const float from_hi = dpp_row_ror<12>(send);
+            a4[j] = keep + (hi ? from_lo : from_hi);
+        }
+    }
+    float a2[2];
+    {
+        const bool hi = lr & 2;
+#pragma unroll
+        for (int j = 0; j < 2; ++j) {
+            const float keep = hi ? a4[j + 2] : a4[j];
+            const float send = hi ? a4[j] : a4[j + 2];
+            const float from_lo = dpp_row_ror<2>(send);
+            const float from_hi = dpp_row_ror<14>(send);
+            a2[j] = keep + (hi ? from_lo : from_hi);
+        }
+    }
+    {
+        const bool hi = lr & 1;
+        const float keep = hi ? a2[1] : a2[0];
+        const float send = hi ? a2[0] : a2[1];
+        const float from_lo = dpp_row_ror<1>(send);
+        const float from_hi = dpp_row_ror<15>(send);
+        return keep + (hi ? from_lo : from_hi);
+    }
+}
+
+__device__ __forceinline__ void publish_partial(const AttnArgs& a, int n_heads, int nsplit, int b, int h, int split, int lane, float o,
+                                                float M, float l, unsigned tag) {
+    float* part = a.part + (((size_t)b * n_heads + h) * a.max_splits + split) * kPartStride;
+    if (a.pl_out == nullptr) {
+        part[lane] = o;
+        if (lane == 0) {
+            part[64] = M;
+            part[65] = l;
+        }
+        return;
+    }
+    float r = o, lsum = l;
+    if (nsplit > 1 && a.part_tag) {
+        typedef unsigned long long u64;
+        auto pack = [&](float v) { return ((u64)tag << 32) | (u64)__float_as_uint(v); };
+        u64* pt0 = a.part_tag + ((size_t)b * n_heads + h) * a.max_splits * kPartStride;
+        const int last = nsplit - 1;
+        if (split != last) {
+            u64* pt = pt0 + split * kPartStride;
+            __hip_atomic_store(pt + lane, pack(o), __ATOMIC_RELAXED, __HIP_MEMORY_SCOPE_AGENT);
+            if (lane == 0) {
+                __hip_atomic_store(pt + 64, pack(M), __ATOMIC_RELAXED, __HIP_MEMORY_SCOPE_AGENT);
+                __hip_atomic_store(pt + 65, pack(l), __ATOMIC_RELAXED, __HIP_MEMORY_SCOPE_AGENT);
+            }
+            return;
+        }
+        float mx = M;
+        r = 0.0f;
+        lsum = 0.0f;
+        constexpr int MAXS = 4;
+        if (nsplit <= MAXS) {
+            u64 vo[MAXS - 1], vm[MAXS - 1], vl[MAXS - 1];
+            for (int spins = 0;; ++spins) {
+                bool ok = true;
+#pragma unroll
+                for (int s = 0; s < MAXS - 1; ++s) {
+                    const u64* ps = pt0 + min(s, last - 1) * kPartStride;
+                    vo[s] = __hip_atomic_load(ps + lane, __ATOMIC_RELAXED, __HIP_MEMORY_SCOPE_AGENT);
+                    vm[s] = __hip_atomic_load(ps + 64, __ATOMIC_RELAXED, __HIP_MEMORY_SCOPE_AGENT);
+                    vl[s] = __hip_atomic_load(ps + 65, __ATOMIC_RELAXED, __HIP_MEMORY_SCOPE_AGENT);
+                    ok = ok && (unsigned)(vo[s] >> 32) == tag && (unsigned)(vm[s] >> 32) == tag && (unsigned)(vl[s] >> 32) == tag;
+                }
+                if (__builtin_amdgcn_ballot_w64(!ok) == 0) break;
+                if ((unsigned)spins >= a.spin_limit) {
+                    if (lane == 0 && a.fault) __hip_atomic_store(a.fault, 1u, __ATOMIC_RELAXED, __HIP_MEMORY_SCOPE_AGENT);
+                    break;
+                }
+                __builtin_amdgcn_s_sleep(1);
+            }
+            float ms[MAXS], ls[MAXS], os[MAXS];
+#pragma unroll
+            for (int s = 0; s < MAXS; ++s) {
+                const bool polled = s < last && s < MAXS - 1;
+                ms[s] = polled ? __uint_as_float((unsigned)vm[s < MAXS - 1 ? s : 0]) : s == last ? M : -1e30f;
+                ls[s] = polled ? __uint_as_float((unsigned)vl[s < MAXS - 1 ? s : 0]) : l;
+                os[s] = polled ? __uint_as_float((unsigned)vo[s < MAXS - 1 ? s : 0]) : o;
+            }
+            mx = fmaxf(fmaxf(ms[0], ms[1]), fmaxf(ms[2], ms[3]));
+#pragma unroll
+            for (int s = 0; s < MAXS; ++s) {
+                const float w = __expf(ms[s] - mx);
+                lsum = fmaf(w, ls[s], lsum);
+                r = fmaf(w, os[s], r);
+            }
+        } else {
+            float mrun = -1e30f;
+            for (int s = 0; s <= last; ++s) {
+                float m_s = M, o_s = o, l_s = l;
+                if (s < last) {
+                    const u64* ps = pt0 + s * kPartStride;
+                    u64 vo, vm, vl;
+                    for (int spins = 0;; ++spins) {
+                        vo = __hip_atomic_load(ps + lane, __ATOMIC_RELAXED, __HIP_MEMORY_SCOPE_AGENT);
+                        vm = __hip_atomic_load(ps + 64, __ATOMIC_RELAXED, __HIP_MEMORY_SCOPE_AGENT);
+                        vl = __hip_atomic_load(ps + 65, __ATOMIC_RELAXED, __HIP_MEMORY_SCOPE_AGENT);
+                        const bool ok = (unsigned)(vo >> 32) == tag && (unsigned)(vm >> 32) == tag && (unsigned)(vl >> 32) == tag;
+                        if (__builtin_amdgcn_ballot_w64(!ok) == 0) break;
+                        if ((unsigned)spins >= a.spin_limit) {
+                            if (lane == 0 && a.fault) __hip_atomic_store(a.fault, 1u, __ATOMIC_RELAXED, __HIP_MEMORY_SCOPE_AGENT);
+                            break;
+                        }
+                        __builtin_amdgcn_s_sleep(1);
+                    }
+                    m_s = __uint_as_float((unsigned)vm);
+                    o_s = __uint_as_float((unsigned)vo);
+                    l_s = __uint_as_float((unsigned)vl);
+                }
+                const float mnew = fmaxf(mrun, m_s);
+                const float w0 = __expf(mrun - mnew), w1 = __expf(m_s - mnew);
+                r = fmaf(w1, o_s, r * w0);
+                lsum = fmaf(w1, l_s, lsum * w0);
+                mrun = mnew;
+            }
+        }
+    } else if (nsplit > 1) {
+        typedef __attribute__((address_space(1))) unsigned gu32;
+        gu32* gp = (gu32*)part;
+        __hip_atomic_store(gp + lane, __float_as_uint(o), __ATOMIC_RELAXED, __HIP_MEMORY_SCOPE_AGENT);
+        if (lane == 0) {
+            __hip_atomic_store(gp + 64, __float_as_uint(M), __ATOMIC_RELAXED, __HIP_MEMORY_SCOPE_AGENT);
+            __hip_atomic_store(gp + 65, __float_as_uint(l), __ATOMIC_RELAXED, __HIP_MEMORY_SCOPE_AGENT);
+        }
+        asm volatile("s_waitcnt vmcnt(0)" ::: "memory");
+        int* cnt = a.merge_cnt + b * n_heads + h;
+        int ticket = 0;
+        if (lane == 0) ticket = __hip_atomic_fetch_add(cnt, 1, __ATOMIC_RELAXED, __HIP_MEMORY_SCOPE_AGENT);
+        ticket = __builtin_amdgcn_readfirstlane(ticket);
+        if (ticket != nsplit - 1) return;
+        if (lane == 0) __hip_atomic_store(cnt, 0, __ATOMIC_RELAXED, __HIP_MEMORY_SCOPE_AGENT);
+        const gu32* p0 = (const gu32*)(a.part + ((size_t)b * n_heads + h) * a.max_splits * kPartStride);
+        constexpr int MAXS = 4;
+        if (nsplit <= MAXS) {
+            float ms[MAXS], ls[MAXS], os[MAXS];
+#pragma unroll
+            for (int s = 0; s < MAXS; ++s) {
+                const gu32* ps = p0 + min(s, nsplit - 1) * kPartStride;
+                ms[s] = __uint_as_float(__hip_atomic_load(ps + 64, __ATOMIC_RELAXED, __HIP_MEMORY_SCOPE_AGENT));
+                ls[s] = __uint_as_float(__hip_atomic_load(ps + 65, __ATOMIC_RELAXED, __HIP_MEMORY_SCOPE_AGENT));
+                os[s] = __uint_as_float(__hip_atomic_load(ps + lane, __ATOMIC_RELAXED, __HIP_MEMORY_SCOPE_AGENT));
+            }
+#pragma unroll
+            for (int s = 0; s < MAXS; ++s)
+                if (s >= nsplit) ms[s] = -1e30f;
+            const float mx = fmaxf(fmaxf(ms[0], ms[1]), fmaxf(ms[2], ms[3]));
+            r = 0.0f;
+            lsum = 0.0f;
+#pragma unroll
+            for (int s = 0; s < MAXS; ++s) {
+                const float w = __expf(ms[s] - mx);
+                lsum = fmaf(w, ls[s], lsum);
+                r = fmaf(w, os[s], r);
+            }
+        } else {
+            float mx = -1e30f;
+            for (int s = 0; s < nsplit; ++s)
+                mx = fmaxf(mx, __uint_as_float(__hip_atomic_load(p0 + s * kPartStride + 64, __ATOMIC_RELAXED, __HIP_MEMORY_SCOPE_AGENT)));
+            r = 0.0f;
+            lsum = 0.0f;
+            for (int s = 0; s < nsplit; ++s) {
+                const gu32* ps = p0 + s * kPartStride;
+                const float w = __expf(__uint_as_float(__hip_atomic_load(ps + 64, __ATOMIC_RELAXED, __HIP_MEMORY_SCOPE_AGENT)) - mx);
+                lsum = fmaf(w, __uint_as_float(__hip_atomic_load(ps + 65, __ATOMIC_RELAXED, __HIP_MEMORY_SCOPE_AGENT)), lsum);
+                r = fmaf(w, __uint_as_float(__hip_atomic_load(ps + lane, __ATOMIC_RELAXED, __HIP_MEMORY_SCOPE_AGENT)), r);
+            }
+        }
+    }
+    const float v = r * (1.0f / lsum);
+    uint32_t hi, mid, lo;
+    split3_pk(v, 0.0f, hi, mid, lo);
+    const int k = h * 64 + lane;
+    a.pl_out[plane_elem(0, b, k)] = (bf16_t)hi;
+    a.pl_out[plane_elem(1, b, k)] = (bf16_t)mid;
+    a.pl_out[plane_elem(2, b, k)] = (bf16_t)lo;
+}
+
+template <typename KV, bool FUSED>
+__device__ __forceinline__ void attn_decode_body(int h, int split, int b, const float* __restrict__ qp, const void* __restrict__ kp,
+                                                 const void* __restrict__ vp, unsigned sb, unsigned sh, unsigned st, unsigned th,
+                                                 const int* __restrict__ cw, const unsigned* __restrict__ ew, const AttnArgs& a,
+                                                 const unsigned long long* __restrict__ qkv_tag) {
+    __shared__ __attribute__((aligned(16))) float s_o[4][64];
+    __shared__ float s_m[4], s_l[4];
+    const int t_hi = (int)(th & 0xfffffu), n_heads = (int)(th >> 20);
+    const int Tc = cw[1];
+    const unsigned epoch = ew[0];
+    const int T = (st >> 31) ? Tc : t_hi;
+    const size_t stride_t = st & 0x7fffffffu;
+    const int chunk0 = split * kAttnChunk;
+    if (chunk0 >= t_hi) return;
+
+    const int lane = threadIdx.x & 63, wave = threadIdx.x >> 6;
+    const int lr = lane & 15, g = lane >> 4;
+    const int base = chunk0 + wave * 64;
+
+    const KV* K = reinterpret_cast<const KV*>(kp) + (size_t)b * sb + (size_t)h * sh;
+    const KV* V = reinterpret_cast<const KV*>(vp) + (size_t)b * sb + (size_t)h * sh;
+    f32x4 q4 = {0.0f, 0.0f, 0.0f, 0.0f};
+    if (!FUSED) q4 = *reinterpret_cast<const f32x4*>(qp + ((size_t)b * n_heads + h) * 64 + lr * 4);
+    const float alpha = 0.125f;
+
+    float m_w = kNegBig, l_w = 0.0f;
+    f32x4 o4 = {0.0f, 0.0f, 0.0f, 0.0f};
+    if (base < t_hi) {
+        f32x4 k4[16], v4[16];
+#pragma unroll
+        for (int i = 0; i < 16; ++i) {
+            const int t = min(base + 4 * i + g, t_hi - 1);
+            k4[i] = load_kv4<KV>(K + (size_t)t * stride_t + lr * 4);
+            v4[i] = load_kv4<KV>(V + (size_t)t * stride_t + lr * 4);
+        }
+        ZG_PIN(a.progress); ZG_PIN(a.part); ZG_PIN(a.max_splits); ZG_PIN(a.pl_out); ZG_PIN(a.part_tag); ZG_PIN(a.launch_id); ZG_PIN(a.merge_cnt); ZG_PIN(a.fault); ZG_PIN(a.spin_limit);
+        pf_count(a.progress);
+        if (FUSED) {
+            typedef unsigned long long u64;
+            const int E = n_heads * 64;
+            const unsigned tag = (epoch << 8) | a.launch_id;
+            const int rel = __builtin_amdgcn_readfirstlane(T - 1 - base);
+            const bool holder = (unsigned)rel < 64u;
+            const u64* wq = qkv_tag + h * 64 + lr * 4;
+            u64 wv[12];
+            for (unsigned spins = 0;; ++spins) {
+                bool ok = true;
+#pragma unroll
+                for (int j = 0; j < 4; ++j) {
+                    wv[j] = __hip_atomic_load(wq + j, __ATOMIC_RELAXED, __HIP_MEMORY_SCOPE_AGENT);
+                    ok = ok && (unsigned)(wv[j] >> 32) == tag;
+                }
+                if (holder) {
+#pragma unroll
+                    for (int j = 0; j < 4; ++j) {
+                        wv[4 + j] = __hip_atomic_load(wq + E + j, __ATOMIC_RELAXED, __HIP_MEMORY_SCOPE_AGENT);
+                        wv[8 + j] = __hip_atomic_load(wq + 2 * E + j, __ATOMIC_RELAXED, __HIP_MEMORY_SCOPE_AGENT);
+                        ok = ok && (unsigned)(wv[4 + j] >> 32) == tag && (unsigned)(wv[8 + j] >> 32) == tag;
+                    }
+                }
+                if (__builtin_amdgcn_ballot_w64(!ok) == 0) break;
+                if (spins >= a.spin_limit) {
+                    if (lane == 0 && a.fault) __hip_atomic_store(a.fault, 1u, __ATOMIC_RELAXED, __HIP_MEMORY_SCOPE_AGENT);
+                    break;
+                }
+                __builtin_amdgcn_s_sleep(1);
+            }
+            q4 = f32x4{__uint_as_float((unsigned)wv[0]), __uint_as_float((unsigned)wv[1]), __uint_as_float((unsigned)wv[2]),
+                       __uint_as_float((unsigned)wv[3])};
+            if (holder && g == (rel & 3)) {
+                const f32x4 kn = {__uint_as_float((unsigned)wv[4]), __uint_as_float((unsigned)wv[5]), __uint_as_float((unsigned)wv[6]),
+                                  __uint_as_float((unsigned)wv[7])};
+                const f32x4 vn = {__uint_as_float((unsigned)wv[8]), __uint_as_float((unsigned)wv[9]), __uint_as_float((unsigned)wv[10]),
+                                  __uint_as_float((unsigned)wv[11])};
+                switch (rel >> 2) {
+#define ZG_NEW_ROW(i) case i: k4[i] = kn; v4[i] = vn; break;
+                    ZG_NEW_ROW(0) ZG_NEW_ROW(1) ZG_NEW_ROW(2) ZG_NEW_ROW(3) ZG_NEW_ROW(4) ZG_NEW_ROW(5) ZG_NEW_ROW(6) ZG_NEW_ROW(7)
+                    ZG_NEW_ROW(8) ZG_NEW_ROW(9) ZG_NEW_ROW(10) ZG_NEW_ROW(11) ZG_NEW_ROW(12) ZG_NEW_ROW(13) ZG_NEW_ROW(14) ZG_NEW_ROW(15)
+#undef ZG_NEW_ROW
+                }
+            }
+        }
+        float s[16];
+#pragma unroll
+        for (int i = 0; i < 16; ++i)
+            s[i] = fmaf(q4.x, k4[i].x, fmaf(q4.y, k4[i].y, fmaf(q4.z, k4[i].z, q4.w * k4[i].w)));
+        float sc = row16_reduce_scatter(s, lr) * alpha;
+        const int t_mine = base + 4 * lr + g;
+        if (t_mine >= T) sc = kNegBig;
+        m_w = wave_allmax(sc);
+        const float p = (t_mine < T) ? __expf(sc - m_w) : 0.0f;
+        l_w = wave_allsum(p);
+#define ZG_PV(i)                                                                                                         \
+    {                                                                                                                    \
+        const float pi = __uint_as_float(__builtin_amdgcn_update_dpp(0u, __float_as_uint(p), 0x150 + (i), 0xF, 0xF, false)); \
+        o4.x = fmaf(pi, v4[i].x, o4.x);                                                                                  \
+        o4.y = fmaf(pi, v4[i].y, o4.y);                                                                                  \
+        o4.z = fmaf(pi, v4[i].z, o4.z);                                                                                  \
+        o4.w = fmaf(pi, v4[i].w, o4.w);                                                                                  \
+    }
+        ZG_PV(0) ZG_PV(1) ZG_PV(2) ZG_PV(3) ZG_PV(4) ZG_PV(5) ZG_PV(6) ZG_PV(7)
+        ZG_PV(8) ZG_PV(9) ZG_PV(10) ZG_PV(11) ZG_PV(12) ZG_PV(13) ZG_PV(14) ZG_PV(15)
+#undef ZG_PV
+        o4.x += __shfl_xor(o4.x, 16, 64); o4.y += __shfl_xor(o4.y, 16, 64);
+        o4.z += __shfl_xor(o4.z, 16, 64); o4.w += __shfl_xor(o4.w, 16, 64);
+        o4.x += __shfl_xor(o4.x, 32, 64); o4.y += __shfl_xor(o4.y, 32, 64);
+        o4.z += __shfl_xor(o4.z, 32, 64); o4.w += __shfl_xor(o4.w, 32, 64);
+    }
+    if (lane < 16) *reinterpret_cast<f32x4*>(&s_o[wave][lane * 4]) = o4;
+    if (lane == 0) {
+        s_m[wave] = m_w;
+        s_l[wave] = l_w;
+    }
+    __syncthreads();
+    if (wave == 0) {
+        const float M = fmaxf(fmaxf(s_m[0], s_m[1]), fmaxf(s_m[2], s_m[3]));
+        float o = 0.0f, l = 0.0f;
+#pragma unroll
+        for (int w = 0; w < 4; ++w) {
+            const float sc = __expf(s_m[w] - M);
+            o = fmaf(sc, s_o[w][lane], o);
+            l = fmaf(sc, s_l[w], l);
+        }
+        publish_partial(a, n_heads, (t_hi + kAttnChunk - 1) / kAttnChunk, b, h, split, lane, o, M, l, (epoch << 8) | a.launch_id);
+    }
+}
+
+}
+
+}
diff --git a/zig_gpt2_amd/csrc/attn_qkv.hip b/zig_gpt2_amd/csrc/attn_qkv.hip
--- /dev/null
+++ b/zig_gpt2_amd/csrc/attn_qkv.hip
@@ -0,0 +1,83 @@
+#include "attn_decode.h"
+#include "gemv_internal.h"
+
+namespace zg {
+
+namespace {
+
+struct QkvAttnArgs {
+    AttnArgs at;
+    unsigned sb, sh, st, th;
+    const unsigned* ew;
+    unsigned long long* qkv_tag;
+    unsigned a0;
+};
+
+template <typename WT, int LPR, int CPL>
+__global__ __launch_bounds__(256) void attn_qkv_kernel(const void* __restrict__ Wv, const float* __restrict__ xin, unsigned ne, unsigned kg,
+                                                       const float* __restrict__ ln_g, const float* __restrict__ c2,
+                                                       const float* __restrict__ c3, const int* __restrict__ cw, const GemvArgs a,
+                                                       const QkvAttnArgs f) {
+    const unsigned blk = blockIdx.x;
+    if (blk < (kg >> 16)) {
+        gemv_lnk_body<WT, LPR, CPL, 4, true>((int)blk, Wv, xin, ne, (int)(kg & 0xffffu), ln_g, c2, c3, cw, a, 2u, f.qkv_tag, f.ew,
+                                             f.at.launch_id);
+        return;
+    }
+    if (blk < f.a0) return;
+    const unsigned r = blk - f.a0, H = f.th >> 20;
+    attn_decode_body<float, true>((int)(r % H), (int)(r / H), 0, nullptr, f.at.k, f.at.v, f.sb, f.sh, f.st, f.th, cw, f.ew, f.at, f.qkv_tag);
+}
+
+}
+
+bool attn_qkv_ok(const GemvArgs& g, const AttnArgs& at) {
+    return gemv_use_lnk(g) && g.epilogue == EPI_QKV && g.M == 1 && g.K <= 0xffff && at.batch == 1 && at.kv_mode == 0 && at.head_dim == 64 &&
+           at.stride_t == 64 && at.ctrl != nullptr && at.pl_out == nullptr && at.part_tag == nullptr && g.head_dim == 64 &&
+           g.N == 3 * at.n_heads * 64;
+}
+
+int launch_attn_qkv(const GemvArgs& g, int weight_type, const AttnArgs& at, const unsigned* epoch, unsigned long long* qkv_tag, hipStream_t s) {
+    ZG_REQUIRE(attn_qkv_ok(g, at) && epoch != nullptr && qkv_tag != nullptr && at.launch_id >= 1 && at.launch_id <= 255, ZG_ERR_ARG,
+               "fused c_attn + attention: unsupported arguments");
+    ZG_REQUIRE(at.t_hi >= 1 && at.t_hi < (1 << 20) && at.n_heads < (1 << 12), ZG_ERR_UNSUPPORTED, "fused attention: t_hi %d / heads %d", at.t_hi,
+               at.n_heads);
+    const int splits = (at.t_hi + kAttnChunk - 1) / kAttnChunk;
+    ZG_REQUIRE(splits <= at.max_splits, ZG_ERR_ARG, "fused attention: t_hi %d needs %d splits > %d", at.t_hi, splits, at.max_splits);
+    ZG_REQUIRE(at.stride_b >= 0 && at.stride_h >= 0 && at.stride_h < (1ll << 32), ZG_ERR_UNSUPPORTED, "fused attention: strides beyond 32 bits");
+    QkvAttnArgs f{};
+    f.at = at;
+    f.sb = (unsigned)at.stride_b;
+    f.sh = (unsigned)at.stride_h;
+    f.st = (unsigned)at.stride_t | 0x80000000u;
+    f.th = (unsigned)at.t_hi | ((unsigned)at.n_heads << 20);
+    f.ew = epoch;
+    f.qkv_tag = qkv_tag;
+    const int* cw = reinterpret_cast<const int*>(g.ctrl);
+    const int nchq = g.K / 32;
+#define ZG_QA(LPR_, CPL_)                                                                                                          \
+    {                                                                                                                              \
+        constexpr int rows = 4 * (64 / LPR_);                                                                                      \
+        const unsigned G = (unsigned)((g.N + rows - 1) / rows);                                                                    \
+        f.a0 = (G + 7u) & ~7u;                                                                                                     \
+        const unsigned grid = f.a0 + (unsigned)(at.n_heads * splits);                                                              \
+        note_kernel("attn_qkv_kernel<%s, %d, %d>", weight_type == WT_BF16 ? "unsigned short" : "float", LPR_, CPL_);               \
+        if (weight_type == WT_BF16)                                                                                                \
+            hipLaunchKernelGGL((attn_qkv_kernel<bf16_t, LPR_, CPL_>), dim3(grid), dim3(256), 0, s, g.W, g.x,                       \
+                               (unsigned)g.N | ((unsigned)g.epilogue << 24), (unsigned)g.K | (G << 16), g.ln_g, g.ln_c2, g.ln_c3, cw, g, f); \
+        else                                                                                                                       \
+            hipLaunchKernelGGL((attn_qkv_kernel<float, LPR_, CPL_>), dim3(grid), dim3(256), 0, s, g.W, g.x,                        \
+                               (unsigned)g.N | ((unsigned)g.epilogue << 24), (unsigned)g.K | (G << 16), g.ln_g, g.ln_c2, g.ln_c3, cw, g, f); \
+        ZG_HIP(hipGetLastError());                                                                                                 \
+        return ZG_OK;                                                                                                              \
+    }
+    if (nchq <= 16 * 2) ZG_QA(16, 2)
+    if (nchq <= 32 * 2) ZG_QA(32, 2)
+    if (nchq <= 32 * 3) ZG_QA(32, 3)
+    if (nchq <= 64 * 2) ZG_QA(64, 2)
+#undef ZG_QA
+    zg::set_error("fused c_attn + attention: K=%d too large", g.K);
+    return ZG_ERR_UNSUPPORTED;
+}
+
+}
diff --git a/zig_gpt2_amd/csrc/gemv_internal.h b/zig_gpt2_amd/csrc/gemv_internal.h
--- a/zig_gpt2_amd/csrc/gemv_internal.h
+++ b/zig_gpt2_amd/csrc/gemv_internal.h
@@ -331,6 +331,123 @@
     return kp <= 5 ? kp : 0;
 }
 
+template <typename WT, int LPR, int CPL, int NP, bool TAGGED>
+__device__ __forceinline__ void gemv_lnk_body(int blk, const void* __restrict__ Wv, const float* __restrict__ xin, unsigned ne, int K,
+                                              const float* __restrict__ ln_g, const float* __restrict__ c2, const float* __restrict__ c3,
+                                              const int* __restrict__ cw, const GemvArgs& a, unsigned pf_inc,
+                                              unsigned long long* __restrict__ tagw, const unsigned* __restrict__ ew, unsigned launch_id) {
+    const int N = (int)(ne & 0xffffffu), epilogue = (int)(ne >> 24);
+    ZG_STAMP_DECL();
+    ZG_STAMP(0);
+    constexpr int RPP = 64 / LPR, ROWS = NP * RPP;
+    __shared__ float part[4][ROWS];
+    __shared__ float stat[4][2];
+    const int tid = threadIdx.x, lane = tid & 63;
+    const int wave = __builtin_amdgcn_readfirstlane(tid >> 6);
+    const int lr = lane % LPR, rsub = lane / LPR;
+    int kbeg, nchq;
+    if (sizeof(WT) == 2 && (K & 63) == 0 && ((K >> 6) & 3) != 0 && (((K >> 6) >> 2) + 1) * 8 <= LPR * CPL) {
+        const int lines = K >> 6, base = lines >> 2, rem = lines & 3;
+        kbeg = (wave * base + min(wave, rem)) * 64;
+        nchq = (base + (wave < rem ? 1 : 0)) * 8;
+    } else {
+        kbeg = wave * (K >> 2);
+        nchq = K >> 5;
+    }
+    const WT* W = reinterpret_cast<const WT*>(Wv) + kbeg;
+    const int row0 = blk * ROWS;
+    Raw<WT> wq[NP][CPL];
+#pragma unroll
+    for (int p = 0; p < NP; ++p) {
+        const WT* pr = W + (size_t)min(row0 + p * RPP + rsub, N - 1) * K;
+#pragma unroll
+        for (int i = 0; i < CPL; ++i) wq[p][i] = load_raw(pr, min(lr + LPR * i, nchq - 1));
+    }
+    W8 xr[CPL], gr[CPL];
+#pragma unroll
+    for (int i = 0; i < CPL; ++i) {
+        const size_t off = (size_t)kbeg + (size_t)min(lr + LPR * i, nchq - 1) * 8;
+        xr[i] = load_x8(xin + off);
+        gr[i] = load_x8(ln_g + off);
+    }
+    float c2n = 0.0f, c3n = 0.0f;
+    if (tid < ROWS) {
+        const int n = min(row0 + tid, N - 1);
+        c2n = c2[n];
+        c3n = c3[n];
+    }
+    const int T = max(cw[1], 1);
+    const unsigned epoch = TAGGED ? ew[0] : 0u;
+    ZG_STAMP(1);
+    {
+        ZG_PIN(a.progress); ZG_PIN(a.y); ZG_PIN(a.y_stride); ZG_PIN(a.epilogue); ZG_PIN(__float_as_uint(a.eps));
+        if (epilogue == EPI_QKV) {
+            ZG_PIN(a.q); ZG_PIN(a.k_cache); ZG_PIN(a.v_cache); ZG_PIN(a.N); ZG_PIN(a.head_dim); ZG_PIN(a.n_heads); ZG_PIN(a.ctx); ZG_PIN(a.kv_mode); ZG_PIN(a.kv_lo);
+        }
+    }
+    if (TAGGED) { ZG_PIN(tagw); ZG_PIN(launch_id); }
+    pf_count(a.progress, pf_inc);
+    ZG_STAMP(2);
+    float sx = 0.0f, sxx = 0.0f;
+#pragma unroll
+    for (int i = 0; i < CPL; ++i) {
+        if (lr + LPR * i >= nchq) xr[i] = zero_w8();
+#pragma unroll
+        for (int j = 0; j < 8; ++j) {
+            sx += xr[i].v[j];
+            sxx = fmaf(xr[i].v[j], xr[i].v[j], sxx);
+            xr[i].v[j] *= gr[i].v[j];
+        }
+    }
+    sx = group_allsum<LPR>(sx);
+    sxx = group_allsum<LPR>(sxx);
+    auto dot = [&](const Raw<WT>(&w)[CPL]) {
+        float p0 = 0.0f, p1 = 0.0f, p2 = 0.0f, p3 = 0.0f;
+#pragma unroll
+        for (int i = 0; i < CPL; ++i) {
+            const W8 u = unpack(w[i]);
+            p0 = fmaf(u.v[0], xr[i].v[0], p0); p1 = fmaf(u.v[1], xr[i].v[1], p1);
+            p2 = fmaf(u.v[2], xr[i].v[2], p2); p3 = fmaf(u.v[3], xr[i].v[3], p3);
+            p0 = fmaf(u.v[4], xr[i].v[4], p0); p1 = fmaf(u.v[5], xr[i].v[5], p1);
+            p2 = fmaf(u.v[6], xr[i].v[6], p2); p3 = fmaf(u.v[7], xr[i].v[7], p3);
+        }
+        return group_allsum<LPR>((p0 + p1) + (p2 + p3));
+    };
+    float sp[NP];
+#pragma unroll
+    for (int p = 0; p < NP; ++p) sp[p] = dot(wq[p]);
+    ZG_STAMP(3);
+    if (lr == 0) {
+#pragma unroll
+        for (int p = 0; p < NP; ++p) part[wave][p * RPP + rsub] = sp[p];
+    }
+    if (lane == 0) {
+        stat[wave][0] = sx;
+        stat[wave][1] = sxx;
+    }
+    __syncthreads();
+    ZG_STAMP(4);
+    if (tid < ROWS && row0 + tid < N) {
+        const int n = row0 + tid;
+        const float inv_k = 1.0f / (float)K;
+        const float mean = ((stat[0][0] + stat[1][0]) + (stat[2][0] + stat[3][0])) * inv_k;
+        const float msq = mean * mean;
+        const float var = fmaf(((stat[0][1] + stat[1][1]) + (stat[2][1] + stat[3][1])), inv_k, -msq);
+        const float rstd = __builtin_amdgcn_rsqf(var + a.eps);
+        const float S1 = (part[0][tid] + part[1][tid]) + (part[2][tid] + part[3][tid]);
+        const float y = fmaf(rstd, fmaf(-mean, c2n, S1), c3n);
+        Best nobest;
+        const float v = epilogue_row(a, 0, n, y, 0.0f, 0.0f, T - 1, nobest);
+        if (TAGGED)
+            __hip_atomic_store(tagw + n, ((unsigned long long)((epoch << 8) | launch_id) << 32) | __float_as_uint(v), __ATOMIC_RELAXED,
+                               __HIP_MEMORY_SCOPE_AGENT);
+    }
+    ZG_STAMP(5);
+    ZG_STAMP(6);
+    ZG_STAMP(7);
+    ZG_STAMP_FLUSH();
+}
+
 }
 
 bool gemv_use_ksplit(const GemvArgs& a);
diff --git a/zig_gpt2_amd/csrc/gemv_ksplit.hip b/zig_gpt2_amd/csrc/gemv_ksplit.hip
--- a/zig_gpt2_amd/csrc/gemv_ksplit.hip
+++ b/zig_gpt2_amd/csrc/gemv_ksplit.hip
@@ -150,110 +150,7 @@
                                                        const float* __restrict__ ln_g, const float* __restrict__ c2,
                                                        const float* __restrict__ c3, const int* __restrict__ cw,
                                                        const GemvArgs a) {
-    const int N = (int)(ne & 0xffffffu), epilogue = (int)(ne >> 24);
-    ZG_STAMP_DECL();
-    ZG_STAMP(0);
-    constexpr int RPP = 64 / LPR, ROWS = NP * RPP;
-    __shared__ float part[4][ROWS];
-    __shared__ float stat[4][2];
-    const int tid = threadIdx.x, lane = tid & 63;
-    const int wave = __builtin_amdgcn_readfirstlane(tid >> 6);
-    const int lr = lane % LPR, rsub = lane / LPR;
-    int kbeg, nchq;
-    if (sizeof(WT) == 2 && (K & 63) == 0 && ((K >> 6) & 3) != 0 && (((K >> 6) >> 2) + 1) * 8 <= LPR * CPL) {
-        const int lines = K >> 6, base = lines >> 2, rem = lines & 3;
-        kbeg = (wave * base + min(wave, rem)) * 64;
-        nchq = (base + (wave < rem ? 1 : 0)) * 8;
-    } else {
-        kbeg = wave * (K >> 2);
-        nchq = K >> 5;
-    }
-    const WT* W = reinterpret_cast<const WT*>(Wv) + kbeg;
-    const int row0 = blockIdx.x * ROWS;
-    Raw<WT> wq[NP][CPL];
-#pragma unroll
-    for (int p = 0; p < NP; ++p) {
-        const WT* pr = W + (size_t)min(row0 + p * RPP + rsub, N - 1) * K;
-#pragma unroll
-        for (int i = 0; i < CPL; ++i) wq[p][i] = load_raw(pr, min(lr + LPR * i, nchq - 1));
-    }
-    W8 xr[CPL], gr[CPL];
-#pragma unroll
-    for (int i = 0; i < CPL; ++i) {
-        const size_t off = (size_t)kbeg + (size_t)min(lr + LPR * i, nchq - 1) * 8;
-        xr[i] = load_x8(xin + off);
-        gr[i] = load_x8(ln_g + off);
-    }
-    float c2n = 0.0f, c3n = 0.0f;
-    if (tid < ROWS) {
-        const int n = min(row0 + tid, N - 1);
-        c2n = c2[n];
-        c3n = c3[n];
-    }
-    const int T = max(cw[1], 1);
-    ZG_STAMP(1);
-    {
-        ZG_PIN(a.progress); ZG_PIN(a.y); ZG_PIN(a.y_stride); ZG_PIN(a.epilogue); ZG_PIN(__float_as_uint(a.eps));
-        if (epilogue == EPI_QKV) {
-            ZG_PIN(a.q); ZG_PIN(a.k_cache); ZG_PIN(a.v_cache); ZG_PIN(a.N); ZG_PIN(a.head_dim); ZG_PIN(a.n_heads); ZG_PIN(a.ctx); ZG_PIN(a.kv_mode); ZG_PIN(a.kv_lo);
-        }
-    }
-    pf_count(a.progress);
-    ZG_STAMP(2);
-    float sx = 0.0f, sxx = 0.0f;
-#pragma unroll
-    for (int i = 0; i < CPL; ++i) {
-        if (lr + LPR * i >= nchq) xr[i] = zero_w8();
-#pragma unroll
-        for (int j = 0; j < 8; ++j) {
-            sx += xr[i].v[j];
-            sxx = fmaf(xr[i].v[j], xr[i].v[j], sxx);
-            xr[i].v[j] *= gr[i].v[j];
-        }
-    }
-    sx = group_allsum<LPR>(sx);
-    sxx = group_allsum<LPR>(sxx);
-    auto dot = [&](const Raw<WT>(&w)[CPL]) {
-        float p0 = 0.0f, p1 = 0.0f, p2 = 0.0f, p3 = 0.0f;
-#pragma unroll
-        for (int i = 0; i < CPL; ++i) {
-            const W8 u = unpack(w[i]);
-            p0 = fmaf(u.v[0], xr[i].v[0], p0); p1 = fmaf(u.v[1], xr[i].v[1], p1);
-            p2 = fmaf(u.v[2], xr[i].v[2], p2); p3 = fmaf(u.v[3], xr[i].v[3], p3);
-            p0 = fmaf(u.v[4], xr[i].v[4], p0); p1 = fmaf(u.v[5], xr[i].v[5], p1);
-            p2 = fmaf(u.v[6], xr[i].v[6], p2); p3 = fmaf(u.v[7], xr[i].v[7], p3);
-        }
-        return group_allsum<LPR>((p0 + p1) + (p2 + p3));
-    };
-    float sp[NP];
-#pragma unroll
-    for (int p = 0; p < NP; ++p) sp[p] = dot(wq[p]);
-    ZG_STAMP(3);
-    if (lr == 0) {
-#pragma unroll
-        for (int p = 0; p < NP; ++p) part[wave][p * RPP + rsub] = sp[p];
-    }
-    if (lane == 0) {
-        stat[wave][0] = sx;
-        stat[wave][1] = sxx;
-    }
-    __syncthreads();
-    ZG_STAMP(4);
-    if (tid < ROWS && row0 + tid < N) {
-        const int n = row0 + tid;
-        const float inv_k = 1.0f / (float)K;
-        const float mean = ((stat[0][0] + stat[1][0]) + (stat[2][0] + stat[3][0])) * inv_k;
-        const float ex2 = ((stat[0][1] + stat[1][1]) + (stat[2][1] + stat[3][1])) * inv_k;
-        const float rstd = __builtin_amdgcn_rsqf(ex2 - mean * mean + a.eps);
-        const float S1 = (part[0][tid] + part[1][tid]) + (part[2][tid] + part[3][tid]);
-        const float y = fmaf(rstd, fmaf(-mean, c2n, S1), c3n);
-        Best nobest;
-        epilogue_row(a, 0, n, y, 0.0f, 0.0f, T - 1, nobest);
-    }
-    ZG_STAMP(5);
-    ZG_STAMP(6);
-    ZG_STAMP(7);
-    ZG_STAMP_FLUSH();
+    gemv_lnk_body<WT, LPR, CPL, NP, false>((int)blockIdx.x, Wv, xin, ne, K, ln_g, c2, c3, cw, a, 1u, nullptr, nullptr, 0u);
 }
 
 template <typename WT>
diff --git a/zig_gpt2_amd/csrc/zg_kernels.h b/zig_gpt2_amd/csrc/zg_kernels.h
--- a/zig_gpt2_amd/csrc/zg_kernels.h
+++ b/zig_gpt2_amd/csrc/zg_kernels.h
@@ -102,6 +102,8 @@
     unsigned spin_limit;
 };
 int launch_attn_decode(const AttnArgs& a, hipStream_t s);
+bool attn_qkv_ok(const GemvArgs& g, const AttnArgs& at);
+int launch_attn_qkv(const GemvArgs& g, int weight_type, const AttnArgs& at, const unsigned* epoch, unsigned long long* qkv_tag, hipStream_t s);
 int launch_attn_any_dim(const float* q, const float* k, const float* v, long stride_b, long stride_h, long stride_t, int batch, int n_heads,
                         int head_dim, int seq_len, float* out, hipStream_t s);
 int launch_attn_merge(const float* part, int batch, int n_heads, int head_dim, int max_splits,
@@ -267,13 +269,13 @@
 };
 int launch_prefetcher(const PfArgs& a, hipStream_t s);
 
-__device__ __forceinline__ void pf_count(unsigned* progress) {
+__device__ __forceinline__ void pf_count(unsigned* progress, unsigned n = 1u) {
     if (progress != nullptr && (blockIdx.x | blockIdx.y | blockIdx.z | threadIdx.x) == 0) {
 #ifdef ZG_STAMPS
-        const unsigned old = __hip_atomic_fetch_add(progress, 1u, __ATOMIC_RELAXED, __HIP_MEMORY_SCOPE_AGENT);
+        const unsigned old = __hip_atomic_fetch_add(progress, n, __ATOMIC_RELAXED, __HIP_MEMORY_SCOPE_AGENT);
         reinterpret_cast<PfCtl*>(progress)->xcd_log[old & 255u] = 0x100u | (__builtin_amdgcn_s_getreg((3 << 11) | 20) & 15u);
 #else
-        __hip_atomic_fetch_add(progress, 1u, __ATOMIC_RELAXED, __HIP_MEMORY_SCOPE_AGENT);
+        __hip_atomic_fetch_add(progress, n, __ATOMIC_RELAXED, __HIP_MEMORY_SCOPE_AGENT);
 #endif
     }
 }
```

New measurement: 5035 tokens/s, median of 6. 6.6% higher.
